# roysubhankar/dwt-domain-adaptation

Measured on NVIDIA H100. Metric: ResNet-50-DWT images/sec fwd+bwd, higher is better.
Workload: dtype f32

## Files before the change

### dwt-domain-adaptation_b200/dwt_b200/_native.py

```python
from __future__ import annotations

import ctypes
import os
import threading

import torch

_HERE = os.path.dirname(os.path.abspath(__file__))
LIB_PATH = os.environ.get("DWT_B200_LIB") or os.path.join(_HERE, "lib", "libdwt_b200.so")

ABI_VERSION = 6
MAX_DOMAINS = 4
MAX_GROUP_SIZE = 64
MODE_TRAIN, MODE_EVAL = 0, 1
EPI_NONE, EPI_AFFINE, EPI_RELU, EPI_RESIDUAL = 0, 1, 2, 4
LAYOUT_NHWC = 0x100
STATUS_NOT_PD, STATUS_BAD_LABEL = 1, 2
KIND_WHITEN, KIND_BN = 0, 1

_c_float_p = ctypes.c_void_p
_PtrArray = ctypes.c_void_p * MAX_DOMAINS


class TailSite(ctypes.Structure):
    _fields_ = [("x", ctypes.c_void_p), ("eps", ctypes.c_float), ("momentum", ctypes.c_float),
                ("update_running", ctypes.c_int), ("running_mean", ctypes.POINTER(ctypes.c_void_p)),
                ("running_cov", ctypes.POINTER(ctypes.c_void_p)), ("gamma", ctypes.c_void_p), ("beta", ctypes.c_void_p),
                ("save_mean", ctypes.c_void_p), ("save_w", ctypes.c_void_p), ("dx", ctypes.c_void_p),
                ("dgamma", ctypes.c_void_p), ("dbeta", ctypes.c_void_p)]

_SIGNATURES = {
    "dwt_abi_version": (ctypes.c_int, []),
    "dwt_last_error": (ctypes.c_char_p, []),
    "dwt_workspace_bytes": (ctypes.c_size_t, [ctypes.c_int64, ctypes.c_int64, ctypes.c_int64, ctypes.c_int, ctypes.c_int]),
    "dwt_whiten_fwd": (ctypes.c_int, [_c_float_p, _c_float_p, ctypes.c_int64, ctypes.c_int64, ctypes.c_int64,
                                      ctypes.c_int, ctypes.c_int, ctypes.c_int, ctypes.c_float, ctypes.c_float,
                                      ctypes.c_int, ctypes.POINTER(ctypes.c_void_p), ctypes.POINTER(ctypes.c_void_p),
                                      _c_float_p, _c_float_p, _c_float_p, ctypes.c_void_p, ctypes.c_int, _c_float_p,
                                      _c_float_p, ctypes.c_void_p, ctypes.c_size_t, ctypes.c_void_p]),
    "dwt_whiten_bwd": (ctypes.c_int, [_c_float_p, _c_float_p, _c_float_p, _c_float_p, ctypes.c_int64, ctypes.c_int64,
                                      ctypes.c_int64, ctypes.c_int, ctypes.c_int, ctypes.c_int, ctypes.c_float,
                                      _c_float_p, _c_float_p, _c_float_p, _c_float_p, ctypes.c_void_p, _c_float_p,
                                      ctypes.c_int, _c_float_p, _c_float_p, ctypes.c_void_p, ctypes.c_size_t,
                                      ctypes.c_void_p]),
    "dwt_bn_fwd": (ctypes.c_int, [_c_float_p, _c_float_p, ctypes.c_int64, ctypes.c_int64, ctypes.c_int64,
                                  ctypes.c_int, ctypes.c_int, ctypes.c_float, ctypes.c_float, ctypes.c_int,
                                  ctypes.POINTER(ctypes.c_void_p), ctypes.POINTER(ctypes.c_void_p), _c_float_p,
                                  _c_float_p, _c_float_p, ctypes.c_void_p, ctypes.c_int, _c_float_p, _c_float_p,
                                  ctypes.c_void_p, ctypes.c_size_t, ctypes.c_void_p]),
    "dwt_bn_bwd": (ctypes.c_int, [_c_float_p, _c_float_p, _c_float_p, _c_float_p, ctypes.c_int64, ctypes.c_int64, ctypes.c_int64,
                                  ctypes.c_int, ctypes.c_int, _c_float_p, _c_float_p, _c_float_p, _c_float_p,
                                  ctypes.c_void_p, _c_float_p, ctypes.c_int, _c_float_p, _c_float_p, ctypes.c_void_p,
                                  ctypes.c_size_t, ctypes.c_void_p]),
    "dwt_tail2_fwd": (ctypes.c_int, [ctypes.c_int, ctypes.POINTER(TailSite), _c_float_p, ctypes.c_void_p, ctypes.c_int64,
                                     ctypes.c_int64, ctypes.c_int64, ctypes.c_int, ctypes.c_int, ctypes.c_void_p,
                                     ctypes.c_size_t, ctypes.c_void_p]),
    "dwt_tail2_bwd": (ctypes.c_int, [ctypes.c_int, ctypes.POINTER(TailSite), _c_float_p, _c_float_p, ctypes.c_void_p,
                                     _c_float_p, ctypes.c_int64, ctypes.c_int64, ctypes.c_int64, ctypes.c_int, ctypes.c_int,
                                     ctypes.c_void_p, ctypes.c_size_t, ctypes.c_void_p]),
    "dwt_mec_fwd_bwd": (ctypes.c_int, [_c_float_p, _c_float_p, ctypes.c_int64, ctypes.c_int64, _c_float_p,
                                       _c_float_p, _c_float_p, ctypes.c_void_p]),
    "dwt_head_loss_fwd_bwd": (ctypes.c_int, [_c_float_p, ctypes.c_void_p, ctypes.c_int64, ctypes.c_int64, ctypes.c_float,
                                             _c_float_p, _c_float_p, ctypes.c_void_p, ctypes.c_void_p]),
    "dwt_augment_pair": (ctypes.c_int, [ctypes.c_void_p, ctypes.c_int64, ctypes.c_int, ctypes.c_int, ctypes.c_int,
                                        ctypes.c_void_p, ctypes.c_void_p, ctypes.c_void_p, _c_float_p,
                                        ctypes.POINTER(ctypes.c_float), ctypes.POINTER(ctypes.c_float), _c_float_p,
                                        _c_float_p, ctypes.c_int, ctypes.c_void_p]),
    "dwt_maxpool_fwd": (ctypes.c_int, [_c_float_p, _c_float_p, ctypes.c_void_p, ctypes.c_int64, ctypes.c_int64, ctypes.c_int64,
                                       ctypes.c_int64, ctypes.c_int, ctypes.c_int, ctypes.c_int, ctypes.c_void_p]),
    "dwt_maxpool_bwd": (ctypes.c_int, [_c_float_p, ctypes.c_void_p, _c_float_p, ctypes.c_int64, ctypes.c_int64, ctypes.c_int64,
                                       ctypes.c_int64, ctypes.c_int, ctypes.c_int, ctypes.c_int, ctypes.c_void_p]),
    "dwt_launch_count": (ctypes.c_int64, []),
    "dwt_profile_begin": (None, []),
    "dwt_profile_end": (ctypes.c_int, [ctypes.c_void_p, ctypes.c_int]),
}


class ProfileEntry(ctypes.Structure):
    _fields_ = [("name", ctypes.c_char * 48), ("launches", ctypes.c_int64), ("ms", ctypes.c_double),
                ("bytes", ctypes.c_double)]


def profile_begin():
    lib().dwt_profile_begin()


def profile_end():
    cap = 1024
    buf = (ProfileEntry * cap)()
    k = lib().dwt_profile_end(ctypes.cast(buf, ctypes.c_void_p), cap)
    return {buf[i].name.decode(): dict(launches=buf[i].launches, ms=buf[i].ms, bytes=buf[i].bytes) for i in range(k)}


def by_family(prof):
    out = {}
    for name, v in prof.items():
        f = out.setdefault(name.split("|")[0], dict(launches=0, ms=0.0, bytes=0.0))
        for k in f:
            f[k] += v[k]
    return out


def launch_count() -> int:
    return int(lib().dwt_launch_count())
EXPORTS = tuple(_SIGNATURES)

_lib = None
_lock = threading.Lock()


class NativeError(RuntimeError):
    pass


def lib() -> ctypes.CDLL:
    global _lib
    if _lib is None:
        with _lock:
            if _lib is None:
                if not os.path.exists(LIB_PATH):
                    raise NativeError(
                        f"{LIB_PATH} is missing: build it with `python {os.path.join(_HERE, 'build.py')}` "
                        "(dwt_b200 has no CPU or PyTorch fallback)")
                handle = ctypes.CDLL(LIB_PATH)
                for name, (res, args) in _SIGNATURES.items():
                    fn = getattr(handle, name)
                    fn.restype, fn.argtypes = res, args
                if handle.dwt_abi_version() != ABI_VERSION:
                    raise NativeError("libdwt_b200.so ABI version mismatch; rebuild it")
                _lib = handle
    return _lib


def channels_last_supported(channels: int, group_size: int) -> bool:
    if group_size not in (1, 2, 4) or channels % 4:
        return False
    c4 = channels // 4
    return c4 & (c4 - 1) == 0


def check(rc: int) -> None:
    if rc != 0:
        raise NativeError(f"libdwt_b200 error {rc}: {lib().dwt_last_error().decode()}")


def ptr(t):
    return None if t is None else ctypes.c_void_p(t.data_ptr())


def ptr_array(tensors):
    arr = _PtrArray()
    for i, t in enumerate(tensors):
        arr[i] = None if t is None else t.data_ptr()
    return ctypes.cast(arr, ctypes.POINTER(ctypes.c_void_p))


def require_cuda(*tensors, any_dtype=False) -> torch.device:
    dev = None
    for t in tensors:
        if t is None:
            continue
        if not t.is_cuda:
            raise NativeError("dwt_b200 runs on CUDA tensors only (no CPU fallback); got a tensor on " + str(t.device))
        if t.dtype != torch.float32 and not any_dtype:
            raise NativeError("dwt_b200 computes in float32; got " + str(t.dtype))
        if dev is None:
            dev = t.device
        elif t.device != dev:
            raise NativeError(f"tensors on different devices: {dev} vs {t.device}")
    return dev


def stream_ptr(device) -> ctypes.c_void_p:
    return ctypes.c_void_p(torch.cuda.current_stream(device).cuda_stream)


_workspaces: dict = {}


def workspace(device, n, c, hw, gs, nd):
    need = lib().dwt_workspace_bytes(n, c, hw, gs, nd)
    if need == 0:
        raise NativeError(f"invalid geometry for workspace: C={c} group_size={gs} domains={nd}")
    key = (device.index, torch.cuda.current_stream(device).cuda_stream)
    buf = _workspaces.get(key)
    if buf is None or buf.numel() < need:
        buf = torch.zeros(max(need, 8 << 20), dtype=torch.uint8, device=device)
        _workspaces[key] = buf
    return buf


def status(device=None) -> int:
    device = torch.device("cuda", torch.cuda.current_device()) if device is None else device
    buf = _workspaces.get((device.index, torch.cuda.current_stream(device).cuda_stream))
    return 0 if buf is None else int(buf[:4].view(torch.int32).item())


def status_all(device=None) -> int:
    device = torch.device("cuda", torch.cuda.current_device()) if device is None else device
    torch.cuda.synchronize(device)
    st = 0
    for (idx, _), buf in _workspaces.items():
        if idx == device.index:
            st |= int(buf[:4].view(torch.int32).item())
    return st


def status_ptr(device):
    return ctypes.c_void_p(workspace(device, 1, 4, 1, 1, 1).data_ptr())


def clear_status(device=None) -> None:
    device = torch.device("cuda", torch.cuda.current_device()) if device is None else device
    buf = _workspaces.get((device.index, torch.cuda.current_stream(device).cuda_stream))
    if buf is not None:
        buf[:4].zero_()


class NotPositiveDefiniteError(torch.linalg.LinAlgError):
    """What the reference's torch.cholesky raises at utils/whitening.py:53, raised late: the kernels never sync the
    host, so the failure is seen at the next poll (raise_on_status) or explicit check_status() call."""


_poll = {"every": 0, "count": 0}


def raise_on_status(every: int = 1) -> None:
    _poll["every"], _poll["count"] = max(0, int(every)), 0


def check_status(device=None) -> None:
    st = status(device)
    if st == 0:
        return
    clear_status(device)
    if st & STATUS_NOT_PD:
        raise NotPositiveDefiniteError(
            "cholesky: a whitening covariance was not positive definite (status word bit 0; the reference raises "
            "from torch.cholesky, utils/whitening.py:53); the affected group's output is NaN and its running-"
            "statistics update was skipped")
    if st & STATUS_BAD_LABEL:
        raise IndexError("head loss: a label was outside [0, num_classes) and is not ignore_index=-100 "
                         "(F.nll_loss asserts here); the row was dropped")
    raise NativeError(f"unknown status bits {st:#x}")


def poll_status(device) -> None:
    if _poll["every"]:
        _poll["count"] += 1
        if _poll["count"] >= _poll["every"]:
            _poll["count"] = 0
            check_status(device)
```

### dwt-domain-adaptation_b200/dwt_b200/csrc/api.cu

```cuda
#include <stdarg.h>
#include <stdio.h>
#include <stdlib.h>

#include <atomic>
#include <mutex>
#include <string>
#include <vector>
#include <string.h>

#include "norm_launch.h"

namespace {

thread_local char g_err[512] = "";

int fail(int code, const char* fmt, ...) {
  va_list ap;
  va_start(ap, fmt);
  vsnprintf(g_err, sizeof(g_err), fmt, ap);
  va_end(ap);
  return code;
}

int check_launch(const char* what) {
  cudaError_t e = cudaPeekAtLastError();
  if (e != cudaSuccess) {
    cudaGetLastError();
    return fail(DWT_E_LAUNCH, "%s: %s", what, cudaGetErrorString(e));
  }
  return DWT_OK;
}

int sm_count() {
  static int n = 0;
  if (n == 0) {
    int dev = 0;
    if (cudaGetDevice(&dev) != cudaSuccess ||
        cudaDeviceGetAttribute(&n, cudaDevAttrMultiProcessorCount, dev) != cudaSuccess || n <= 0)
      n = 132;
  }
  return n;
}

std::atomic<int64_t> g_launches{0};
std::mutex g_prof_mu;
bool g_prof_on = false;
struct ProfRec { char name[48]; cudaEvent_t a, b; double bytes; };
std::vector<ProfRec> g_prof;
std::vector<cudaEvent_t> g_event_pool;

cudaEvent_t take_event() {
  if (!g_event_pool.empty()) { cudaEvent_t e = g_event_pool.back(); g_event_pool.pop_back(); return e; }
  cudaEvent_t e = nullptr;
  cudaEventCreate(&e);
  return e;
}

struct Launch {
  cudaStream_t st; ProfRec rec; bool on;
  Launch(const char* family, const dwt::Geom* gm, double bytes, cudaStream_t s) : st(s), on(false) {
    rec.a = rec.b = nullptr; rec.bytes = bytes;
    if (gm) snprintf(rec.name, sizeof(rec.name), "%s|%d|%d|%d|%d|%d", family, gm->C, gm->HW, gm->GS, gm->D, gm->N);
    else snprintf(rec.name, sizeof(rec.name), "%s", family);
    g_launches.fetch_add(1, std::memory_order_relaxed);
    std::lock_guard<std::mutex> lk(g_prof_mu);
    if (g_prof_on && g_prof.size() < (1u << 18)) {
      on = true; rec.a = take_event(); rec.b = take_event();
      cudaEventRecord(rec.a, st);
    }
  }
  ~Launch() {
    if (!on) return;
    cudaEventRecord(rec.b, st);
    std::lock_guard<std::mutex> lk(g_prof_mu);
    g_prof.push_back(rec);
  }
};

std::once_flag g_tiled_once;
int g_tiled_rc = 0;
int ensure_tiled() {
  std::call_once(g_tiled_once, [] { g_tiled_rc = dwt::tiled_init(); });
  return g_tiled_rc;
}

std::once_flag g_tc_once;
int g_tc_rc = 0;
int ensure_tc() {
  std::call_once(g_tc_once, [] { g_tc_rc = dwt::tc_init(); });
  return g_tc_rc;
}

int tc_chunks(const dwt::Geom& g) {
  const int problems = dwt::tc_superblocks(g) * g.D;
  int n = 2 * sm_count() / problems;
  const int64_t tiles = (int64_t)g.N * ((g.HW + 31) / 32);
  if (n > tiles) n = (int)tiles;
  return n < 1 ? 1 : n;
}

int tc_apply_ctas(const dwt::Geom& g, int per_sm, int tile_px) {
  const int problems = dwt::tc_superblocks(g) * g.D;
  int n = per_sm * sm_count() / problems;
  const int64_t tiles = (int64_t)g.N * ((g.HW + tile_px - 1) / tile_px);
  if (n > tiles) n = (int)tiles;
  return n < 1 ? 1 : n;
}

int env_int(const char* name, int dflt) {
  const char* v = getenv(name);
  return (v && *v) ? atoi(v) : dflt;
}

struct ClPlan { int nred, new_, S, gridy, gz_red, gz_ew; };
ClPlan cl_plan(const dwt::Geom& g, int slots_red, int slots_ew, int unroll_red, int unroll_ew) {
  static const int seq_mb = env_int("DWT_CL_SEQ_MB", 1 << 30);
  const int C4 = g.C / 4, CW = C4 < 256 ? C4 : 256, rpi = 256 / CW, gridy = C4 / CW;
  const long long rows = (long long)g.N * g.HW;
  const double mbytes = 4.0 * (double)g.D * (double)rows * (double)g.C / 1048576.0;
  const bool seq = g.D > 1 && mbytes >= (double)seq_mb;
  ClPlan p;
  p.gridy = gridy;
  p.gz_red = p.gz_ew = seq ? 1 : g.D;
  auto shape = [&](int slots, int unroll, int gz) {
    long long by_work = rows / ((long long)rpi * unroll * 2);
    if (by_work < 1) by_work = 1;
    int cap = slots * sm_count() / (gridy * gz);
    if (cap < 1) cap = 1;
    return (int)(by_work < cap ? by_work : cap);
  };
  p.nred = shape(slots_red, unroll_red, p.gz_red);
  p.new_ = shape(slots_ew, unroll_ew, p.gz_ew);
  p.S = p.nred < 8 ? p.nred : 8;
  return p;
}

inline size_t align_up(size_t v, size_t a) { return (v + a - 1) / a * a; }

enum KernelKind { K_STATS, K_APPLY, K_BWD_REDUCE, K_BWD_APPLY };

int slots_per_sm(KernelKind k, int GS) {
  if (GS > 4) return 2;
  return ((k == K_STATS || k == K_APPLY) && GS < 4) ? 4 : 3;
}

int chunk_cap(int GS, int G, int D) {
  (void)GS;
  const int target = 16 * sm_count();
  int cap = (target + G * D - 1) / (G * D);
  return cap < 1 ? 1 : cap;
}

struct Workspace {
  int* status;
  int* counters;
  int* dom_counter;
  int* dom_counter2;
  float* partial;
  float* save_cov;
  float* coef;
  float* dgb_part;
  float* gram;
  float* shift;
  float* red;
  int* bad;
  size_t bytes;
};

constexpr size_t kMaxGroups = 65536;
constexpr size_t kOffCounters = 256;
constexpr size_t kOffDom1 = kOffCounters + sizeof(int) * DWT_MAX_DOMAINS * kMaxGroups;
constexpr size_t kOffDom2 = kOffDom1 + sizeof(int) * kMaxGroups;
constexpr size_t kOffScratch = kOffDom2 + sizeof(int) * kMaxGroups;

Workspace carve(void* base, int64_t C, int GS, int D, size_t start = kOffScratch) {
  const int G = (int)(C / GS);
  const int cap = chunk_cap(GS, G, D);
  size_t off = start;
  auto take = [&](size_t nbytes) { size_t o = off; off = align_up(off + nbytes, 256); return o; };
  char* b = static_cast<char*>(base);
  Workspace w;
  w.status = reinterpret_cast<int*>(b);
  w.counters = reinterpret_cast<int*>(b + kOffCounters);
  w.dom_counter = reinterpret_cast<int*>(b + kOffDom1);
  w.dom_counter2 = reinterpret_cast<int*>(b + kOffDom2);
  size_t partial_floats = (size_t)D * G * cap * (GS * GS + GS);
  if (GS >= 8 && 64 % GS == 0) {
    const size_t tc = ((size_t)2 * sm_count() + (size_t)((C + 63) / 64) * D) * (64 * 64 + 64);
    if (tc > partial_floats) partial_floats = tc;
  }
  size_t red_floats = 1;
  if (dwt::cl_supports((int)C, GS)) {
    const size_t W = (size_t)dwt::cl_bwd_width((int)C, GS);
    const int C4 = (int)C / 4, gridy = C4 <= 256 ? 1 : C4 / 256;
    const size_t cl = (size_t)D * (3 * sm_count() / gridy + 1) * W;
    if (cl > partial_floats) partial_floats = cl;
    red_floats = (size_t)D * 8 * W;
  }
  w.partial = reinterpret_cast<float*>(b + take(sizeof(float) * partial_floats));
  w.red = reinterpret_cast<float*>(b + take(sizeof(float) * red_floats));
  w.save_cov = reinterpret_cast<float*>(b + take(sizeof(float) * (size_t)D * G * GS * GS));
  w.coef = reinterpret_cast<float*>(b + take(sizeof(float) * (size_t)D * G * dwt::coef_stride(GS)));
  w.dgb_part = reinterpret_cast<float*>(b + take(sizeof(float) * (size_t)D * 2 * C));
  const size_t SBn = (size_t)((C + 63) / 64);
  w.gram = reinterpret_cast<float*>(b + take(sizeof(float) * (size_t)D * SBn * (64 * 64 + 64)));
  w.shift = reinterpret_cast<float*>(b + take(sizeof(float) * (size_t)D * SBn * 64));
  w.bad = reinterpret_cast<int*>(b + take(sizeof(int) * (size_t)D * G));
  w.bytes = off;
  return w;
}

struct Plan {
  dwt::Geom gm;
  dwt::Geom gm_ew;
  int vec;
  int chunks_ew;
  bool small;
};

void shape(dwt::Geom& g, int64_t work_units, KernelKind kind, bool small, int* chunks) {
  const bool reduce = (kind == K_STATS || kind == K_BWD_REDUCE);
  const int slots = slots_per_sm(kind, g.GS) * sm_count();
  const int target = reduce ? slots : 4 * slots;
  g.ppc = 1;
  if (small) {
    while (g.ppc < 8 && (int64_t)((g.G + g.ppc - 1) / g.ppc) * g.D > target) g.ppc <<= 1;
  }
  int n = 1;
  if (g.ppc == 1) {
    n = target / (g.G * g.D);
    const int cap = chunk_cap(g.GS, g.G, g.D);
    if (n > cap) n = cap;
    if (n > work_units) n = (int)work_units;
    if (n < 1) n = 1;
  }
  *chunks = n;
}

int make_plan(Plan& p, KernelKind reduce_kind, KernelKind ew_kind, const void* a0, const void* a1, const void* a2,
              int64_t N, int64_t C, int64_t HW, int GS, int D) {
  if (N <= 0 || C <= 0 || HW <= 0) return fail(DWT_E_INVALID, "empty tensor (N=%lld C=%lld HW=%lld)", (long long)N,
                                               (long long)C, (long long)HW);
  if (GS < 1 || GS > DWT_MAX_GROUP_SIZE) return fail(DWT_E_UNSUPPORTED, "group_size %d outside [1,%d]", GS,
                                                     DWT_MAX_GROUP_SIZE);
  if (C % GS != 0) return fail(DWT_E_INVALID, "channels %lld not divisible by group_size %d", (long long)C, GS);
  if (D < 1 || D > DWT_MAX_DOMAINS) return fail(DWT_E_INVALID, "n_domains %d outside [1,%d]", D, DWT_MAX_DOMAINS);
  if (N * C * HW >= (int64_t)1 << 31 || C / GS > 65535)
    return fail(DWT_E_UNSUPPORTED, "shape too large for 32-bit item indexing");
  dwt::Geom& g = p.gm;
  g.N = (int)N; g.C = (int)C; g.HW = (int)HW; g.GS = GS; g.G = (int)(C / GS); g.D = D;
  g.M = (float)((double)N * (double)HW);
  const uintptr_t bits = (uintptr_t)a0 | (uintptr_t)a1 | (uintptr_t)a2;
  p.vec = (HW % 4 == 0 && bits % 16 == 0) ? 4 : 1;
  p.small = dwt::small_supports(GS);
  int64_t work_units;
  if (p.small) work_units = (N * (HW / p.vec) + dwt::kThreads * 2 - 1) / (dwt::kThreads * 2);
  else work_units = (N * HW + 127) / 128;
  if (work_units < 1) work_units = 1;
  shape(g, work_units, reduce_kind, p.small, &g.nchunks);
  p.gm_ew = g;
  shape(p.gm_ew, work_units, ew_kind, p.small, &p.chunks_ew);
  p.gm_ew.nchunks = g.nchunks;
  return DWT_OK;
}

int check_running(bool need_running, float* const* rmean, float* const* rcov, int D) {
  if (!need_running) return DWT_OK;
  if (!rmean || !rcov) return fail(DWT_E_INVALID, "running buffers required");
  for (int d = 0; d < D; ++d)
    if (!rmean[d] || !rcov[d]) return fail(DWT_E_INVALID, "running buffer of domain %d is null", d);
  return DWT_OK;
}

dwt::FwdFin make_fwd_fin(float a, float b, float momentum, float unbias, int update_running, bool need_running,
                         float* const* rmean, float* const* rcov, float* save_mean, float* save_w, const Workspace& w, int D) {
  dwt::FwdFin fin{};
  fin.a = a; fin.b = b; fin.momentum = momentum; fin.unbias = unbias;
  fin.update_running = update_running;
  fin.save_mean = save_mean; fin.save_w = save_w; fin.save_cov = w.save_cov;
  for (int d = 0; d < D; ++d) { fin.rmean[d] = need_running ? rmean[d] : nullptr; fin.rcov[d] = need_running ? rcov[d] : nullptr; }
  fin.dom_counter = w.dom_counter; fin.status = w.status; fin.bad = w.bad;
  if (need_running && D > 1) {
    bool all_same = true, all_distinct = true;
    for (int d = 1; d < D; ++d) {
      if (rmean[d] != rmean[0] || rcov[d] != rcov[0]) all_same = false;
      for (int e = 0; e < d; ++e)
        if (rmean[d] == rmean[e] || rcov[d] == rcov[e]) all_distinct = false;
    }
    fin.aliased = all_same ? 1 : (all_distinct ? 0 : -1);
  }
  return fin;
}

dwt::BwdFin make_bwd_fin(float a, int mode, int epi, const float* save_mean, const float* save_w, const float* gamma,
                         float* dgamma, float* dbeta, const Workspace& w) {
  dwt::BwdFin fin{};
  fin.a = a; fin.mode = mode; fin.epi = epi;
  fin.save_mean = save_mean; fin.save_w = save_w; fin.gamma = gamma;
  fin.coef = w.coef; fin.dgb_part = w.dgb_part;
  fin.dgamma = (epi & DWT_EPI_AFFINE) ? dgamma : nullptr;
  fin.dbeta = (epi & DWT_EPI_AFFINE) ? dbeta : nullptr;
  fin.dom_counter = w.dom_counter2;
  return fin;
}

int whiten_like_fwd(const float* x, float* y, int64_t N, int64_t C, int64_t HW, int GS, int D, int mode, float a,
                    float b, float momentum, float unbias, int update_running, float* const* rmean,
                    float* const* rcov, const float* gamma, const float* beta, const float* residual,
                    uint8_t* relu_mask, int epi, float* save_mean, float* save_w, void* ws, size_t ws_bytes,
                    cudaStream_t st) {
  const bool nhwc = (mode & DWT_LAYOUT_NHWC) != 0;
  mode &= 0xFF;
  Plan p;
  if (int rc = make_plan(p, K_STATS, K_APPLY, x, y, nullptr, N, C, HW, GS, D)) return rc;
  if (!x || !y || !save_mean || !save_w || !ws) return fail(DWT_E_INVALID, "null pointer argument");
  if (nhwc && !dwt::cl_supports((int)C, GS))
    return fail(DWT_E_UNSUPPORTED, "channels-last layout is built for group_size 1, 2, 4 with C/4 a power of two (C=%lld gs=%d)", (long long)C, GS);
  if (nhwc && (((uintptr_t)x | (uintptr_t)y) % 16 != 0)) return fail(DWT_E_INVALID, "channels-last tensors must be 16-byte aligned");
  if (mode != DWT_MODE_TRAIN && mode != DWT_MODE_EVAL) return fail(DWT_E_INVALID, "bad mode %d", mode);
  if ((epi & DWT_EPI_RELU) && !(epi & DWT_EPI_AFFINE)) return fail(DWT_E_INVALID, "RELU epilogue needs AFFINE");
  if ((epi & DWT_EPI_AFFINE) && (!gamma || !beta)) return fail(DWT_E_INVALID, "AFFINE epilogue needs gamma and beta");
  if ((epi & DWT_EPI_RESIDUAL) && ((epi & 3) != 3 || !residual)) return fail(DWT_E_INVALID, "RESIDUAL epilogue needs AFFINE|RELU and a residual tensor");
  if ((epi & DWT_EPI_RESIDUAL) && (uintptr_t)residual % 16 != 0) return fail(DWT_E_INVALID, "residual must be 16-byte aligned");
  if (relu_mask && !((epi & DWT_EPI_RESIDUAL) && nhwc))
    return fail(DWT_E_UNSUPPORTED, "the ReLU byte map is written by the channels-last RESIDUAL epilogue only");
  if (epi != 0 && !p.small)
    return fail(DWT_E_UNSUPPORTED, "fused gamma/beta/ReLU epilogue is built for group_size 1, 2, 4 (got %d)", GS);
  const bool need_running = (mode == DWT_MODE_EVAL) || update_running;
  if (int rc = check_running(need_running, rmean, rcov, D)) return rc;
  Workspace w = carve(ws, C, GS, D);
  if (w.bytes > ws_bytes) return fail(DWT_E_WORKSPACE, "workspace too small: need %zu bytes, got %zu", w.bytes, ws_bytes);
  if ((uintptr_t)ws % 256 != 0) return fail(DWT_E_WORKSPACE, "workspace must be 256-byte aligned");
  if (!p.small && ensure_tiled() != 0) return fail(DWT_E_LAUNCH, "cudaFuncSetAttribute failed (%d)", g_tiled_rc);

  const dwt::FwdFin fin = make_fwd_fin(a, b, momentum, unbias, mode == DWT_MODE_TRAIN ? update_running : 0, need_running,
                                       rmean, rcov, save_mean, save_w, w, D);

  const double E = 4.0 * (double)D * (double)N * (double)C * (double)HW;
  if (nhwc) {
    const ClPlan cp = cl_plan(p.gm, 3, 3, 8, (epi & DWT_EPI_RESIDUAL) ? 4 : 8);
    if (mode == DWT_MODE_TRAIN) {
      {
        Launch l("cl_stats", &p.gm, E, st);
        dwt::cl_stats(x, p.gm, cp.nred, cp.gz_red, w.partial, w.shift, st);
      }
      if (int rc = check_launch("channels-last statistics kernel")) return rc;
      Launch l("cl_fwd_finalize", &p.gm, 0.0, st);
      dwt::cl_fwd_finalize(w.partial, cp.nred, w.shift, p.gm, fin, st);
    } else {
      Launch l("eval_prep", &p.gm, 0.0, st);
      dwt::small_eval_prep(p.gm, fin, st);
    }
    if (int rc = check_launch("channels-last finalize kernel")) return rc;
    {
      Launch l("cl_apply", &p.gm, ((epi & DWT_EPI_RESIDUAL) ? (relu_mask ? 3.0625 : 3.0) : 2.0) * E, st);
      dwt::cl_apply(x, y, p.gm, cp.new_, cp.gz_ew, epi, save_mean, save_w, gamma, beta, residual, relu_mask, st);
    }
    return check_launch("channels-last apply kernel");
  }
  const bool tc = !p.small && dwt::tc_supports(p.gm, p.vec) && ensure_tc() == 0;
  if (mode == DWT_MODE_TRAIN) {
    Launch l(p.small ? "small_stats" : (tc ? "tc_stats" : "tiled_stats"), &p.gm, E, st);
    if (p.small) dwt::small_stats(x, p.gm, p.vec, fin, w.partial, w.counters, st);
    else if (tc) {
      if (int cr = dwt::tc_stats(x, p.gm, tc_chunks(p.gm), w.shift, w.partial, st))
        return fail(DWT_E_LAUNCH, "cuTensorMapEncodeTiled failed (CUresult %d) x=%p N=%d C=%d HW=%d D=%d", cr, (const void*)x, p.gm.N, p.gm.C, p.gm.HW, p.gm.D);
    } else dwt::tiled_stats(x, p.gm, p.vec, fin, w.partial, w.counters, st);
  } else {
    Launch l("eval_prep", &p.gm, 0.0, st);
    if (p.small) dwt::small_eval_prep(p.gm, fin, st);
    else if (tc) dwt::dense_fwd_factor(nullptr, nullptr, p.gm, fin, st);
    else dwt::tiled_eval_prep(p.gm, fin, st);
  }
  if (tc && mode == DWT_MODE_TRAIN) {
    if (int rc = check_launch("tensor-core statistics kernel")) return rc;
    Launch l("dense_fwd_finalize", &p.gm, 0.0, st);
    dwt::dense_partial_reduce(w.partial, tc_chunks(p.gm), dwt::tc_superblocks(p.gm) * D, w.gram, st);
    dwt::dense_fwd_factor(w.gram, w.shift, p.gm, fin, st);
  }
  if (int rc = check_launch("whitening statistics kernel")) return rc;
  {
    Launch l(p.small ? "small_apply" : (tc ? "tc_apply" : "tiled_apply"), &p.gm, ((epi & DWT_EPI_RESIDUAL) ? 3 : 2) * E, st);
    if (p.small) dwt::small_apply(x, y, p.gm_ew, p.vec, p.chunks_ew, epi, save_mean, save_w, gamma, beta, residual, st);
    else if (tc) {
      if (int cr = dwt::tc_apply(x, y, p.gm, tc_apply_ctas(p.gm, 1, 64), save_mean, save_w, st))
        return fail(DWT_E_LAUNCH, "cuTensorMapEncodeTiled failed (CUresult %d)", cr);
    } else dwt::tiled_apply(x, y, p.gm_ew, p.vec, p.chunks_ew, save_mean, save_w, st);
  }
  return check_launch("whitening apply kernel");
}

int whiten_like_bwd(const float* x, const float* dout, const float* dout2, float* dx, int64_t N, int64_t C, int64_t HW, int GS, int D,
                    int mode, float a, const float* save_mean, const float* save_w, const float* gamma,
                    const float* beta, const uint8_t* relu_mask, float* dresidual, int epi, float* dgamma,
                    float* dbeta, void* ws, size_t ws_bytes, cudaStream_t st) {
  const bool nhwc = (mode & DWT_LAYOUT_NHWC) != 0;
  mode &= 0xFF;
  Plan p;
  if (int rc = make_plan(p, K_BWD_REDUCE, K_BWD_APPLY, x, dout, dx, N, C, HW, GS, D)) return rc;
  if (!x || !dout || !dx || !save_mean || !save_w || !ws) return fail(DWT_E_INVALID, "null pointer argument");
  if (dout2 && (!nhwc || (uintptr_t)dout2 % 16 != 0))
    return fail(nhwc ? DWT_E_INVALID : DWT_E_UNSUPPORTED, "a second gradient addend (dout2) is built for the channels-last "
                "kernels (16-byte aligned tensor); add it to dout otherwise");
  if (nhwc && !dwt::cl_supports((int)C, GS))
    return fail(DWT_E_UNSUPPORTED, "channels-last layout is built for group_size 1, 2, 4 with C/4 a power of two (C=%lld gs=%d)", (long long)C, GS);
  if (nhwc && (((uintptr_t)x | (uintptr_t)dout | (uintptr_t)dx) % 16 != 0)) return fail(DWT_E_INVALID, "channels-last tensors must be 16-byte aligned");
  if (mode != DWT_MODE_TRAIN && mode != DWT_MODE_EVAL) return fail(DWT_E_INVALID, "bad mode %d", mode);
  if ((epi & DWT_EPI_RELU) && !(epi & DWT_EPI_AFFINE)) return fail(DWT_E_INVALID, "RELU epilogue needs AFFINE");
  if ((epi & DWT_EPI_AFFINE) && (!gamma || !beta)) return fail(DWT_E_INVALID, "AFFINE epilogue needs gamma and beta");
  if (epi & DWT_EPI_RESIDUAL) {
    if (!nhwc || !relu_mask || (epi & 3) != 3 || !dresidual)
      return fail(DWT_E_INVALID, "backward of a RESIDUAL forward needs the channels-last layout, AFFINE|RELU, the forward's "
                                 "ReLU byte map and dresidual (or pass dout already masked by (out > 0) with epilogue AFFINE)");
    if ((uintptr_t)dresidual % 16 != 0) return fail(DWT_E_INVALID, "dresidual must be 16-byte aligned");
  } else if (relu_mask || dresidual) {
    return fail(DWT_E_INVALID, "relu_mask / dresidual belong to the RESIDUAL epilogue");
  }
  if ((dgamma == nullptr) != (dbeta == nullptr)) return fail(DWT_E_INVALID, "dgamma and dbeta go together");
  if (epi != 0 && !p.small)
    return fail(DWT_E_UNSUPPORTED, "fused gamma/beta/ReLU epilogue is built for group_size 1, 2, 4 (got %d)", GS);
  Workspace w = carve(ws, C, GS, D);
  if (w.bytes > ws_bytes) return fail(DWT_E_WORKSPACE, "workspace too small: need %zu bytes, got %zu", w.bytes, ws_bytes);
  if ((uintptr_t)ws % 256 != 0) return fail(DWT_E_WORKSPACE, "workspace must be 256-byte aligned");
  if (!p.small && ensure_tiled() != 0) return fail(DWT_E_LAUNCH, "cudaFuncSetAttribute failed (%d)", g_tiled_rc);

  const dwt::BwdFin fin = make_bwd_fin(a, mode, epi, save_mean, save_w, gamma, dgamma, dbeta, w);
  const bool masked = nhwc && (epi & DWT_EPI_RESIDUAL) != 0;

  const bool need_reduce = (mode == DWT_MODE_TRAIN) || (fin.dgamma != nullptr) || masked;
  const double E = 4.0 * (double)D * (double)N * (double)C * (double)HW;
  if (nhwc) {
    const ClPlan cp = cl_plan(p.gm, 2, 2, 4, 4);
    if (need_reduce) {
      {
        Launch l("cl_bwd_reduce", &p.gm, ((masked ? 3.0625 : 2.0) + (dout2 ? 1.0 : 0.0)) * E, st);
        dwt::cl_bwd_reduce(x, dout, dout2, p.gm, cp.nred, cp.gz_red, epi, save_mean, save_w, gamma, beta, relu_mask, dresidual, w.partial, st);
      }
      if (int rc = check_launch("channels-last backward reduction kernel")) return rc;
      Launch l("cl_bwd_finalize", &p.gm, 0.0, st);
      dwt::cl_bwd_finalize(w.partial, cp.nred, p.gm, fin, st);
    } else {
      Launch l("bwd_prep", &p.gm, 0.0, st);
      dwt::small_bwd_prep(p.gm, fin, st);
    }
    if (int rc = check_launch("channels-last backward finalize kernel")) return rc;
    {
      Launch l("cl_bwd_apply", &p.gm, (3.0 + (dout2 && !masked ? 1.0 : 0.0)) * E, st);
      if (masked) dwt::cl_bwd_apply(x, dresidual, nullptr, dx, p.gm, cp.new_, cp.gz_ew, DWT_EPI_AFFINE, w.coef, save_mean, save_w, gamma, beta, st);
      else dwt::cl_bwd_apply(x, dout, dout2, dx, p.gm, cp.new_, cp.gz_ew, epi, w.coef, save_mean, save_w, gamma, beta, st);
    }
    return check_launch("channels-last backward apply kernel");
  }
  const bool tc = !p.small && dwt::tc_supports(p.gm, p.vec) && ensure_tc() == 0;
  if (need_reduce) {
    Launch l(p.small ? "small_bwd_reduce" : (tc ? "tc_bwd_reduce" : "tiled_bwd_reduce"), &p.gm, 2 * E, st);
    if (p.small) dwt::small_bwd_reduce(x, dout, p.gm, p.vec, fin, beta, w.partial, w.counters, st);
    else if (tc) {
      if (int cr = dwt::tc_bwd_reduce(x, dout, p.gm, tc_chunks(p.gm), save_mean, w.partial, st))
        return fail(DWT_E_LAUNCH, "cuTensorMapEncodeTiled failed (CUresult %d) x=%p dout=%p N=%d C=%d HW=%d D=%d", cr, (const void*)x, (const void*)dout, p.gm.N, p.gm.C, p.gm.HW, p.gm.D);
    } else dwt::tiled_bwd_reduce(x, dout, p.gm, p.vec, fin, w.partial, w.counters, st);
  } else {
    Launch l("bwd_prep", &p.gm, 0.0, st);
    if (p.small) dwt::small_bwd_prep(p.gm, fin, st);
    else if (tc) dwt::dense_bwd_coef(nullptr, p.gm, fin, w.shift, st);
    else dwt::tiled_bwd_prep(p.gm, fin, st);
  }
  if (tc && need_reduce) {
    if (int rc = check_launch("tensor-core backward reduction kernel")) return rc;
    Launch l("dense_bwd_finalize", &p.gm, 0.0, st);
    dwt::dense_partial_reduce(w.partial, tc_chunks(p.gm), dwt::tc_superblocks(p.gm) * D, w.gram, st);
    dwt::dense_bwd_coef(w.gram, p.gm, fin, w.shift, st);
  }
  if (int rc = check_launch("whitening backward reduction kernel")) return rc;
  {
    Launch l(p.small ? "small_bwd_apply" : (tc ? "tc_bwd_apply" : "tiled_bwd_apply"), &p.gm, 3 * E, st);
    if (p.small) dwt::small_bwd_apply(x, dout, dx, p.gm_ew, p.vec, p.chunks_ew, epi, w.coef, save_mean, save_w, gamma, beta, st);
    else if (tc) {
      if (int cr = dwt::tc_bwd_apply(x, dout, dx, p.gm, tc_apply_ctas(p.gm, 1, 64), w.coef, save_mean, w.shift, st))
        return fail(DWT_E_LAUNCH, "cuTensorMapEncodeTiled failed (CUresult %d)", cr);
    } else dwt::tiled_bwd_apply(x, dout, dx, p.gm_ew, p.vec, p.chunks_ew, w.coef, st);
  }
  return check_launch("whitening backward apply kernel");
}

struct SiteConst { float a, b, unbias; };
SiteConst site_const(int kind, float eps, int64_t N, int64_t HW) {
  if (kind == DWT_KIND_BN) {
    const double M = (double)N * (double)HW;
    return {1.f, eps, M > 1.0 ? (float)(M / (M - 1.0)) : 1.f};
  }
  return {1.f - eps, eps, 1.f};
}

int tail2_plan(Plan& p, int kind, const dwt_tail_site* s, const void* out, int64_t N, int64_t C, int64_t HW, int GS, int D) {
  if (kind != DWT_KIND_WHITEN && kind != DWT_KIND_BN) return fail(DWT_E_INVALID, "bad kind %d", kind);
  if (kind == DWT_KIND_BN && GS != 1) return fail(DWT_E_INVALID, "batch norm has group_size 1 (got %d)", GS);
  if (!s) return fail(DWT_E_INVALID, "null pointer argument");
  if (int rc = make_plan(p, K_STATS, K_APPLY, s[0].x, s[1].x, out, N, C, HW, GS, D)) return rc;
  if (!dwt::cl_supports((int)C, GS))
    return fail(DWT_E_UNSUPPORTED, "the two-site tail runs on the channels-last kernels: group_size 1, 2, 4 with C/4 a power of two (C=%lld gs=%d)",
                (long long)C, GS);
  for (int k = 0; k < 2; ++k)
    if (!s[k].x || !s[k].gamma || !s[k].beta || !s[k].save_mean || !s[k].save_w || !out) return fail(DWT_E_INVALID, "null pointer argument");
  if ((((uintptr_t)s[0].x | (uintptr_t)s[1].x | (uintptr_t)out) % 16) != 0) return fail(DWT_E_INVALID, "channels-last tensors must be 16-byte aligned");
  return DWT_OK;
}

int tail2_workspace(Workspace (&w)[2], void* ws, size_t ws_bytes, int64_t C, int GS, int D) {
  if (!ws) return fail(DWT_E_INVALID, "null pointer argument");
  w[0] = carve(ws, C, GS, D);
  w[1] = carve(ws, C, GS, D, w[0].bytes);
  if (w[1].bytes > ws_bytes) return fail(DWT_E_WORKSPACE, "workspace too small: need %zu bytes, got %zu", w[1].bytes, ws_bytes);
  if ((uintptr_t)ws % 256 != 0) return fail(DWT_E_WORKSPACE, "workspace must be 256-byte aligned");
  return DWT_OK;
}

int tail2_fwd(int kind, const dwt_tail_site* s, float* y, uint8_t* relu_mask, int64_t N, int64_t C, int64_t HW, int GS, int D,
              void* ws, size_t ws_bytes, cudaStream_t st) {
  Plan p;
  if (int rc = tail2_plan(p, kind, s, y, N, C, HW, GS, D)) return rc;
  if (!relu_mask) return fail(DWT_E_INVALID, "the two-site tail writes the ReLU byte map its backward reads");
  for (int k = 0; k < 2; ++k)
    if (int rc = check_running(s[k].update_running != 0, s[k].running_mean, s[k].running_cov, D)) return rc;
  Workspace w[2];
  if (int rc = tail2_workspace(w, ws, ws_bytes, C, GS, D)) return rc;
  dwt::FwdFin fin[2];
  for (int k = 0; k < 2; ++k) {
    const SiteConst sc = site_const(kind, s[k].eps, N, HW);
    fin[k] = make_fwd_fin(sc.a, sc.b, s[k].momentum, sc.unbias, s[k].update_running, s[k].update_running != 0, s[k].running_mean,
                          s[k].running_cov, s[k].save_mean, s[k].save_w, w[k], D);
  }
  const double E = 4.0 * (double)D * (double)N * (double)C * (double)HW;
  const ClPlan cp = cl_plan(p.gm, 3, 3, 8, 4);
  for (int k = 0; k < 2; ++k) {
    Launch l("cl_stats", &p.gm, E, st);
    dwt::cl_stats(s[k].x, p.gm, cp.nred, cp.gz_red, w[k].partial, w[k].shift, st);
  }
  if (int rc = check_launch("channels-last statistics kernel")) return rc;
  {
    Launch l("cl_tail2_fwd_finalize", &p.gm, 0.0, st);
    dwt::cl_fwd_finalize(w[0].partial, cp.nred, w[0].shift, p.gm, fin[0], st, &fin[1], (size_t)(w[1].partial - w[0].partial),
                         (size_t)(w[1].shift - w[0].shift));
  }
  if (int rc = check_launch("channels-last finalize kernel")) return rc;
  {
    Launch l("cl_tail2_apply", &p.gm, 3.0625 * E, st);
    dwt::cl_tail2_apply(s[0].x, s[1].x, y, p.gm, cp.new_, cp.gz_ew, s[0].save_mean, s[0].save_w, s[0].gamma, s[0].beta,
                        s[1].save_mean, s[1].save_w, s[1].gamma, s[1].beta, relu_mask, st);
  }
  return check_launch("channels-last two-site apply kernel");
}

int tail2_bwd(int kind, const dwt_tail_site* s, const float* dout, const float* dout2, const uint8_t* relu_mask, float* dz,
              int64_t N, int64_t C, int64_t HW, int GS, int D, void* ws, size_t ws_bytes, cudaStream_t st) {
  Plan p;
  if (int rc = tail2_plan(p, kind, s, dz, N, C, HW, GS, D)) return rc;
  if (!dout || !relu_mask || !s[0].dx || !s[1].dx) return fail(DWT_E_INVALID, "null pointer argument");
  if ((((uintptr_t)dout | (uintptr_t)dout2 | (uintptr_t)s[0].dx | (uintptr_t)s[1].dx) % 16) != 0)
    return fail(DWT_E_INVALID, "channels-last tensors must be 16-byte aligned");
  for (int k = 0; k < 2; ++k)
    if ((s[k].dgamma == nullptr) != (s[k].dbeta == nullptr)) return fail(DWT_E_INVALID, "dgamma and dbeta go together");
  Workspace w[2];
  if (int rc = tail2_workspace(w, ws, ws_bytes, C, GS, D)) return rc;
  dwt::BwdFin fin[2];
  for (int k = 0; k < 2; ++k)
    fin[k] = make_bwd_fin(site_const(kind, s[k].eps, N, HW).a, DWT_MODE_TRAIN, k ? DWT_EPI_AFFINE : (DWT_EPI_AFFINE | DWT_EPI_RELU | DWT_EPI_RESIDUAL),
                          s[k].save_mean, s[k].save_w, s[k].gamma, s[k].dgamma, s[k].dbeta, w[k]);
  const double E = 4.0 * (double)D * (double)N * (double)C * (double)HW;
  const ClPlan cp = cl_plan(p.gm, 2, 2, 4, 4);
  {
    Launch l("cl_tail2_bwd_reduce", &p.gm, (4.0625 + (dout2 ? 1.0 : 0.0)) * E, st);
    dwt::cl_tail2_bwd_reduce(s[0].x, s[1].x, dout, dout2, p.gm, cp.nred, cp.gz_red, s[0].save_mean, s[1].save_mean, relu_mask, dz,
                             w[0].partial, (size_t)(w[1].partial - w[0].partial), st);
  }
  if (int rc = check_launch("channels-last two-site backward reduction kernel")) return rc;
  {
    Launch l("cl_tail2_bwd_finalize", &p.gm, 0.0, st);
    dwt::cl_bwd_finalize(w[0].partial, cp.nred, p.gm, fin[0], st, &fin[1], (size_t)(w[1].partial - w[0].partial));
  }
  if (int rc = check_launch("channels-last backward finalize kernel")) return rc;
  {
    Launch l("cl_tail2_bwd_apply", &p.gm, 5.0 * E, st);
    dwt::cl_tail2_bwd_apply(s[0].x, s[1].x, dz, s[0].dx, s[1].dx, p.gm, cp.new_, cp.gz_ew, w[0].coef, w[1].coef, st);
  }
  return check_launch("channels-last two-site backward apply kernel");
}

}

extern "C" {

int dwt_abi_version(void) { return DWT_B200_ABI_VERSION; }

const char* dwt_last_error(void) { return g_err; }

size_t dwt_workspace_bytes(int64_t N, int64_t C, int64_t HW, int group_size, int n_domains) {
  (void)N; (void)HW;
  if (C <= 0 || group_size < 1 || group_size > DWT_MAX_GROUP_SIZE || C % group_size != 0 || n_domains < 1 ||
      n_domains > DWT_MAX_DOMAINS)
    return 0;
  return carve(nullptr, C, group_size, n_domains, carve(nullptr, C, group_size, n_domains).bytes).bytes;
}

int dwt_whiten_fwd(const float* x, float* y, int64_t N, int64_t C, int64_t HW, int group_size, int n_domains,
                   int mode, float eps, float momentum, int update_running, float* const* running_mean,
                   float* const* running_cov, const float* gamma, const float* beta, const float* residual,
                   uint8_t* relu_mask, int epilogue, float* save_mean, float* save_w, void* workspace,
                   size_t workspace_bytes, dwt_stream_t stream) {
  return whiten_like_fwd(x, y, N, C, HW, group_size, n_domains, mode, 1.f - eps, eps, momentum, 1.f, update_running,
                         running_mean, running_cov, gamma, beta, residual, relu_mask, epilogue, save_mean, save_w,
                         workspace, workspace_bytes, (cudaStream_t)stream);
}

int dwt_whiten_bwd(const float* x, const float* dout, const float* dout2, float* dx, int64_t N, int64_t C, int64_t HW, int group_size,
                   int n_domains, int mode, float eps, const float* save_mean, const float* save_w,
                   const float* gamma, const float* beta, const uint8_t* relu_mask, float* dresidual, int epilogue,
                   float* dgamma, float* dbeta, void* workspace, size_t workspace_bytes, dwt_stream_t stream) {
  return whiten_like_bwd(x, dout, dout2, dx, N, C, HW, group_size, n_domains, mode, 1.f - eps, save_mean, save_w, gamma,
                         beta, relu_mask, dresidual, epilogue, dgamma, dbeta, workspace, workspace_bytes,
                         (cudaStream_t)stream);
}

int dwt_bn_fwd(const float* x, float* y, int64_t N, int64_t C, int64_t HW, int n_domains, int mode, float eps,
               float factor, int update_running, float* const* running_mean, float* const* running_var,
               const float* weight, const float* bias, const float* residual, uint8_t* relu_mask, int epilogue,
               float* save_mean, float* save_invstd, void* workspace, size_t workspace_bytes, dwt_stream_t stream) {
  const double M = (double)N * (double)HW;
  const float unbias = M > 1.0 ? (float)(M / (M - 1.0)) : 1.f;
  return whiten_like_fwd(x, y, N, C, HW, 1, n_domains, mode, 1.f, eps, factor, unbias, update_running, running_mean,
                         running_var, weight, bias, residual, relu_mask, epilogue, save_mean, save_invstd, workspace,
                         workspace_bytes, (cudaStream_t)stream);
}

int dwt_bn_bwd(const float* x, const float* dout, const float* dout2, float* dx, int64_t N, int64_t C, int64_t HW, int n_domains,
               int mode, const float* save_mean, const float* save_invstd, const float* weight, const float* bias,
               const uint8_t* relu_mask, float* dresidual, int epilogue, float* dweight, float* dbias, void* workspace,
               size_t workspace_bytes, dwt_stream_t stream) {
  return whiten_like_bwd(x, dout, dout2, dx, N, C, HW, 1, n_domains, mode, 1.f, save_mean, save_invstd, weight, bias,
                         relu_mask, dresidual, epilogue, dweight, dbias, workspace, workspace_bytes,
                         (cudaStream_t)stream);
}

int dwt_tail2_fwd(int kind, const dwt_tail_site* sites, float* y, uint8_t* relu_mask, int64_t N, int64_t C, int64_t HW,
                  int group_size, int n_domains, void* workspace, size_t workspace_bytes, dwt_stream_t stream) {
  return tail2_fwd(kind, sites, y, relu_mask, N, C, HW, group_size, n_domains, workspace, workspace_bytes, (cudaStream_t)stream);
}

int dwt_tail2_bwd(int kind, const dwt_tail_site* sites, const float* dout, const float* dout2, const uint8_t* relu_mask, float* dz,
                  int64_t N, int64_t C, int64_t HW, int group_size, int n_domains, void* workspace, size_t workspace_bytes,
                  dwt_stream_t stream) {
  return tail2_bwd(kind, sites, dout, dout2, relu_mask, dz, N, C, HW, group_size, n_domains, workspace, workspace_bytes,
                   (cudaStream_t)stream);
}

int dwt_mec_fwd_bwd(const float* x, const float* y, int64_t N, int64_t K, float* loss, float* gx, float* gy,
                    dwt_stream_t stream) {
  if (!x || !y || !loss || !gx || !gy) return fail(DWT_E_INVALID, "null pointer argument");
  if (N <= 0 || K <= 0 || N >= (1 << 24) || K >= (1 << 24)) return fail(DWT_E_INVALID, "bad logits shape [%lld,%lld]", (long long)N, (long long)K);
  {
    Launch l("mec", nullptr, 16.0 * (double)N * (double)K, (cudaStream_t)stream);
    dwt::mec_launch(x, y, (int)N, (int)K, loss, gx, gy, (cudaStream_t)stream);
  }
  return check_launch("MEC kernel");
}

int dwt_head_loss_fwd_bwd(const float* logits, const int64_t* labels, int64_t B, int64_t K, float lambda, float* losses,
                          float* grad, int* status, dwt_stream_t stream) {
  if (!logits || !labels || !losses || !grad) return fail(DWT_E_INVALID, "null pointer argument");
  if (B <= 0 || K <= 0 || B >= (1 << 22) || K >= (1 << 24)) return fail(DWT_E_INVALID, "bad logits shape [3*%lld,%lld]", (long long)B, (long long)K);
  {
    Launch l("head_loss", nullptr, 4.0 * 3 * (double)B * (double)K * 2, (cudaStream_t)stream);
    dwt::head_loss_launch(logits, reinterpret_cast<const long long*>(labels), (int)B, (int)K, lambda, losses, grad, status,
                          (cudaStream_t)stream);
  }
  return check_launch("head loss kernel");
}

int dwt_augment_pair(const uint8_t* images, int64_t B, int src_h, int src_w, int crop, const int32_t* crop_plain,
                     const int32_t* crop_aug, const uint8_t* flip, const float* affine, const float* mean,
                     const float* stdv, float* out_plain, float* out_aug, int layout, dwt_stream_t stream) {
  if (!images || !mean || !stdv) return fail(DWT_E_INVALID, "null pointer argument");
  if (!out_plain && !out_aug) return fail(DWT_E_INVALID, "at least one of out_plain / out_aug is needed");
  if (out_plain && !crop_plain) return fail(DWT_E_INVALID, "out_plain needs crop_plain");
  if (out_aug && (!crop_aug || !flip || !affine)) return fail(DWT_E_INVALID, "out_aug needs crop_aug, flip and affine");
  if (B <= 0 || B > 65535 || src_h <= 0 || src_w <= 0 || src_h > 16384 || src_w > 16384)
    return fail(DWT_E_INVALID, "bad image batch [%lld,%d,%d,3]", (long long)B, src_h, src_w);
  if (crop <= 0 || crop > src_h || crop > src_w) return fail(DWT_E_INVALID, "crop %d does not fit %dx%d", crop, src_h, src_w);
  if (layout != 0 && layout != DWT_LAYOUT_NHWC) return fail(DWT_E_INVALID, "layout must be 0 (NCHW) or DWT_LAYOUT_NHWC");
  for (int c = 0; c < 3; ++c)
    if (!(stdv[c] != 0.f)) return fail(DWT_E_INVALID, "std[%d] must be non-zero", c);
  {
    const double px = (double)B * crop * crop;
    Launch l("augment_pair", nullptr, px * 3 * ((out_plain ? 5.0 : 0.0) + (out_aug ? 5.0 : 0.0)), (cudaStream_t)stream);
    dwt::augment_pair_launch(images, (int)B, src_h, src_w, crop, crop_plain, crop_aug, flip, affine, mean, stdv, out_plain,
                             out_aug, layout != 0, (cudaStream_t)stream);
  }
  return check_launch("augmentation kernel");
}

namespace {
int pool_check(int64_t N, int64_t H, int64_t W, int64_t C, int k, int s, int p, int* OH, int* OW) {
  if (N <= 0 || H <= 0 || W <= 0 || C <= 0 || C % 4 != 0) return fail(DWT_E_INVALID, "bad pooling input [%lld,%lld,%lld,%lld] (C must be a multiple of 4)", (long long)N, (long long)H, (long long)W, (long long)C);
  if (k < 1 || k > 15 || s < 1 || p < 0 || 2 * p > k) return fail(DWT_E_INVALID, "bad pooling window k=%d s=%d p=%d (k <= 15, pad <= k/2)", k, s, p);
  if (H + 2 * p < k || W + 2 * p < k) return fail(DWT_E_INVALID, "pooling window larger than the padded image");
  *OH = (int)((H + 2 * p - k) / s + 1);
  *OW = (int)((W + 2 * p - k) / s + 1);
  if (N * H * W * C >= ((int64_t)1 << 40)) return fail(DWT_E_UNSUPPORTED, "tensor too large");
  return DWT_OK;
}
}

int dwt_maxpool_fwd(const float* x, float* y, uint8_t* argmax, int64_t N, int64_t H, int64_t W, int64_t C, int kernel,
                    int stride, int padding, dwt_stream_t stream) {
  int OH = 0, OW = 0;
  if (int rc = pool_check(N, H, W, C, kernel, stride, padding, &OH, &OW)) return rc;
  if (!x || !y || !argmax) return fail(DWT_E_INVALID, "null pointer argument");
  if ((((uintptr_t)x | (uintptr_t)y) % 16) != 0 || (uintptr_t)argmax % 4 != 0) return fail(DWT_E_INVALID, "pooling tensors must be 16-byte aligned");
  {
    const double in = (double)N * H * W * C, out = (double)N * OH * OW * C;
    Launch l("maxpool_fwd", nullptr, 4.0 * (in + out) + out, (cudaStream_t)stream);
    dwt::maxpool_fwd_launch(x, y, argmax, (int)N, (int)H, (int)W, (int)C, OH, OW, kernel, stride, padding, (cudaStream_t)stream);
  }
  return check_launch("max-pool forward kernel");
}

int dwt_maxpool_bwd(const float* dy, const uint8_t* argmax, float* dx, int64_t N, int64_t H, int64_t W, int64_t C, int kernel,
                    int stride, int padding, dwt_stream_t stream) {
  int OH = 0, OW = 0;
  if (int rc = pool_check(N, H, W, C, kernel, stride, padding, &OH, &OW)) return rc;
  if (!dy || !dx || !argmax) return fail(DWT_E_INVALID, "null pointer argument");
  if ((((uintptr_t)dy | (uintptr_t)dx) % 16) != 0 || (uintptr_t)argmax % 4 != 0) return fail(DWT_E_INVALID, "pooling tensors must be 16-byte aligned");
  {
    const double in = (double)N * H * W * C, out = (double)N * OH * OW * C;
    Launch l("maxpool_bwd", nullptr, 4.0 * (in + out) + out, (cudaStream_t)stream);
    dwt::maxpool_bwd_launch(dy, argmax, dx, (int)N, (int)H, (int)W, (int)C, OH, OW, kernel, stride, padding, (cudaStream_t)stream);
  }
  return check_launch("max-pool backward kernel");
}

int64_t dwt_launch_count(void) { return g_launches.load(); }

void dwt_profile_begin(void) {
  std::lock_guard<std::mutex> lk(g_prof_mu);
  for (auto& r : g_prof) { g_event_pool.push_back(r.a); g_event_pool.push_back(r.b); }
  g_prof.clear();
  g_prof_on = true;
}

int dwt_profile_end(dwt_profile_entry* out, int max_entries) {
  std::vector<ProfRec> recs;
  {
    std::lock_guard<std::mutex> lk(g_prof_mu);
    g_prof_on = false;
    recs.swap(g_prof);
  }
  int n = 0;
  for (auto& r : recs) {
    float ms = 0.f;
    if (cudaEventSynchronize(r.b) == cudaSuccess && cudaEventElapsedTime(&ms, r.a, r.b) == cudaSuccess) {
      int k = 0;
      for (; k < n; ++k)
        if (strcmp(out[k].name, r.name) == 0) break;
      if (k == n && n < max_entries) {
        memset(&out[n], 0, sizeof(out[n]));
        strncpy(out[n].name, r.name, sizeof(out[n].name) - 1);
        ++n;
      }
      if (k < n) { out[k].launches += 1; out[k].ms += ms; out[k].bytes += r.bytes; }
    }
    std::lock_guard<std::mutex> lk(g_prof_mu);
    g_event_pool.push_back(r.a); g_event_pool.push_back(r.b);
  }
  return n;
}

}
```

### dwt-domain-adaptation_b200/dwt_b200/csrc/norm_cl.cu

```cuda
#include <stdlib.h>

#include "dwt_common.cuh"
#include "norm_launch.h"
#include "small_algebra.cuh"

namespace dwt {
namespace {

constexpr int kT = 256;

__device__ __forceinline__ void pdl_wait() { asm volatile("griddepcontrol.wait;" ::: "memory"); }
__device__ __forceinline__ void pdl_launch_dependents() { asm volatile("griddepcontrol.launch_dependents;" ::: "memory"); }

template <int GS> struct ClShape {
  static constexpr int NSUB = 4 / GS;
  static constexpr int NM = GS * (GS + 1) / 2;
  static constexpr int FWD1 = GS + NM;
  static constexpr int BWD1 = GS * GS + GS;
  static constexpr int FWD = NSUB * FWD1;
  static constexpr int BWD = NSUB * BWD1;
};

struct ClThread {
  int C4, CW, rpi, col, rsub, q;
  __device__ __forceinline__ ClThread(const Geom& gm) {
    C4 = gm.C >> 2;
    CW = C4 < kT ? C4 : kT;
    rpi = kT / CW;
    col = threadIdx.x % CW;
    rsub = threadIdx.x / CW;
    q = blockIdx.y * CW + col;
  }
};

template <int UNROLL, bool DESC, class F>
__device__ __forceinline__ void sweep_rows(const ClThread& t, unsigned rows, F&& body) {
  const unsigned krows = (unsigned)t.rpi * UNROLL, nch = (rows + krows - 1) / krows;
  for (unsigned i = blockIdx.x; i < nch; i += gridDim.x) body((DESC ? nch - 1 - i : i) * krows + t.rsub);
}
#define CL_FOR_DOMAINS(d, gm, DESC) \
  for (int di_ = blockIdx.z, d = (DESC) ? (gm).D - 1 - di_ : di_; di_ < (gm).D; di_ += gridDim.z, d = (DESC) ? (gm).D - 1 - di_ : di_)

__device__ __forceinline__ float4 ldg4(const float* p) { return __ldg(reinterpret_cast<const float4*>(p)); }

template <int NACC>
__device__ __forceinline__ void column_reduce(const ClThread& t, float (&acc)[NACC], float* sRed) {
  if (t.rpi == 1) return;
#pragma unroll
  for (int i = 0; i < NACC; ++i) sRed[i * kT + threadIdx.x] = acc[i];
  __syncthreads();
  if (t.rsub == 0) {
#pragma unroll
    for (int i = 0; i < NACC; ++i) {
      float s = acc[i];
      for (int r = 1; r < t.rpi; ++r) s += sRed[i * kT + r * t.CW + t.col];
      acc[i] = s;
    }
  }
}

template <int GS>
__global__ void __launch_bounds__(kT, 3) cl_stats_kernel(const float* __restrict__ x, const Geom gm,
                                                         float* __restrict__ partial, float* __restrict__ shift) {
  using S = ClShape<GS>;
  constexpr int UNROLL = 8;
  __shared__ float sRed[kT * S::FWD];
  const ClThread t(gm);
  const unsigned rows = (unsigned)gm.N * gm.HW;
  pdl_launch_dependents();
  CL_FOR_DOMAINS(d, gm, true) {
    const float* xd = x + (size_t)d * rows * gm.C + 4 * t.q;
    float K[4] = {0.f, 0.f, 0.f, 0.f};
    {
      const unsigned np = rows < 8 ? rows : 8;
      for (unsigned r = 0; r < np; ++r) {
        const float4 v = ldg4(xd + (size_t)r * gm.C);
        K[0] += v.x; K[1] += v.y; K[2] += v.z; K[3] += v.w;
      }
#pragma unroll
      for (int c = 0; c < 4; ++c) K[c] /= (float)np;
      if (blockIdx.x == 0 && t.rsub == 0) *reinterpret_cast<float4*>(shift + (size_t)d * gm.C + 4 * t.q) = make_float4(K[0], K[1], K[2], K[3]);
    }
    float acc[S::FWD];
#pragma unroll
    for (int i = 0; i < S::FWD; ++i) acc[i] = 0.f;
    sweep_rows<UNROLL, true>(t, rows, [&](unsigned r) {
      float4 v[UNROLL];
#pragma unroll
      for (int u = 0; u < UNROLL; ++u) {
        const unsigned rr = r + u * t.rpi;
        v[u] = rr < rows ? ldg4(xd + (size_t)rr * gm.C) : make_float4(K[0], K[1], K[2], K[3]);
      }
#pragma unroll
      for (int u = 0; u < UNROLL; ++u) {
        const float e[4] = {v[u].x - K[0], v[u].y - K[1], v[u].z - K[2], v[u].w - K[3]};
#pragma unroll
        for (int s = 0; s < S::NSUB; ++s) {
#pragma unroll
          for (int c = 0; c < GS; ++c) {
            acc[s * S::FWD1 + c] += e[s * GS + c];
#pragma unroll
            for (int j = 0; j <= c; ++j)
              acc[s * S::FWD1 + GS + c * (c + 1) / 2 + j] = fmaf(e[s * GS + c], e[s * GS + j], acc[s * S::FWD1 + GS + c * (c + 1) / 2 + j]);
          }
        }
      }
    });
    column_reduce<S::FWD>(t, acc, sRed);
    if (t.rsub == 0) {
      float* dst = partial + (((size_t)d * gridDim.x + blockIdx.x) * t.C4 + t.q) * S::FWD;
#pragma unroll
      for (int i = 0; i < S::FWD; ++i) dst[i] = acc[i];
    }
    if (gridDim.z == 1) __syncthreads();
  }
}

template <int GS, int PER>
__device__ __forceinline__ int acc_index(int g, int a) {
  constexpr int NSUB = 4 / GS;
  return (g / NSUB) * (NSUB * PER) + (g % NSUB) * PER + a;
}

constexpr int kFinQ = 2;

template <int NACC>
__device__ __forceinline__ void column_row_sum(const float* __restrict__ col, int nrows, int W, float (&a)[NACC]) {
  static_assert(NACC % 2 == 0, "accumulators are read as float2");
#pragma unroll
  for (int i = 0; i < NACC; ++i) a[i] = 0.f;
#pragma unroll 4
  for (int r = threadIdx.x; r < nrows; r += 32) {
    const float2* p = reinterpret_cast<const float2*>(col + (size_t)r * W);
#pragma unroll
    for (int i = 0; i < NACC / 2; ++i) {
      const float2 v = __ldcg(p + i);
      a[2 * i] += v.x; a[2 * i + 1] += v.y;
    }
  }
#pragma unroll
  for (int o = 1; o < 32; o <<= 1)
#pragma unroll
    for (int i = 0; i < NACC; ++i) a[i] += __shfl_xor_sync(0xffffffffu, a[i], o);
}

template <int NSUB, int PER>
__device__ __forceinline__ void take_group(const float (&a)[NSUB * PER], int s, float (&v)[PER]) {
#pragma unroll
  for (int i = 0; i < PER; ++i) {
    v[i] = a[i];
#pragma unroll
    for (int k = 1; k < NSUB; ++k)
      if (s == k) v[i] = a[k * PER + i];
  }
}

template <int GS>
__device__ __forceinline__ void cl_fwd_finalize_site(const float* __restrict__ partial, int nrows, const float* __restrict__ shift,
                                                     const Geom& gm, const FwdFin& fin) {
  using SH = ClShape<GS>;
  constexpr int NST = GS + GS * GS;
  __shared__ float sStat[DWT_MAX_DOMAINS][kFinQ][SH::NSUB][NST + 1];
  __shared__ unsigned char sBad[DWT_MAX_DOMAINS][kFinQ][SH::NSUB];
  const int s = threadIdx.x, ql = threadIdx.y, d = threadIdx.z, q = blockIdx.x * blockDim.y + ql;
  const int W = (gm.C >> 2) * SH::FWD;
  const float invM = 1.f / gm.M;
  const bool lead = s < SH::NSUB;
  const int g = q * SH::NSUB + (lead ? s : 0);
  const bool direct = gm.D == 1 || fin.aliased == 0;
  const int dbuf = direct ? d : 0;
  const bool upd = fin.update_running && lead && (direct || (fin.aliased == 1 && d == 0));
  float rc_old[GS * GS], rm_old[GS];
  if (upd) {
#pragma unroll
    for (int e = 0; e < GS * GS; ++e) rc_old[e] = fin.rcov[dbuf][(size_t)g * GS * GS + e];
#pragma unroll
    for (int e = 0; e < GS; ++e) rm_old[e] = fin.rmean[dbuf][g * GS + e];
  }
  pdl_launch_dependents();
  pdl_wait();
  float a[SH::FWD];
  column_row_sum<SH::FWD>(partial + (size_t)d * nrows * W + (size_t)q * SH::FWD, nrows, W, a);
  if (lead) {
    float v[SH::FWD1];
    take_group<SH::NSUB, SH::FWD1>(a, s, v);
    float mean[GS], cov[GS][GS];
#pragma unroll
    for (int i = 0; i < GS; ++i) mean[i] = shift[(size_t)d * gm.C + g * GS + i] + v[i] * invM;
#pragma unroll
    for (int i = 0; i < GS; ++i)
#pragma unroll
      for (int j = 0; j <= i; ++j) {
        const float c = v[GS + i * (i + 1) / 2 + j] * invM - (v[i] * invM) * (v[j] * invM);
        cov[i][j] = c; cov[j][i] = c;
      }
    const bool bad = factor_thread<GS>(gm, fin, d, g, mean, cov, false);
    if (fin.update_running) {
      if (direct) {
        if (!bad) {
          const float m = fin.momentum, kk = 1.f - fin.momentum;
#pragma unroll
          for (int i = 0; i < GS; ++i) {
            fin.rmean[d][g * GS + i] = m * mean[i] + kk * rm_old[i];
#pragma unroll
            for (int j = 0; j < GS; ++j)
              fin.rcov[d][(size_t)g * GS * GS + i * GS + j] = m * (cov[i][j] * fin.unbias) + kk * rc_old[i * GS + j];
          }
        }
      } else {
        sBad[d][ql][s] = bad ? 1 : 0;
#pragma unroll
        for (int i = 0; i < GS; ++i) {
          sStat[d][ql][s][i] = mean[i];
#pragma unroll
          for (int j = 0; j < GS; ++j) sStat[d][ql][s][GS + i * GS + j] = cov[i][j];
        }
      }
    }
  }
  if (!fin.update_running || direct) return;
  __syncthreads();
  if (!(lead && d == 0)) return;
  if (fin.aliased == 1) {
    const float m = fin.momentum, kk = 1.f - fin.momentum;
    float* rc = fin.rcov[0] + (size_t)g * GS * GS;
    float* rm = fin.rmean[0] + g * GS;
    for (int dd = 0; dd < gm.D; ++dd) {
      if (sBad[dd][ql][s]) continue;
#pragma unroll
      for (int e = 0; e < GS * GS; ++e) rc_old[e] = m * (sStat[dd][ql][s][GS + e] * fin.unbias) + kk * rc_old[e];
#pragma unroll
      for (int e = 0; e < GS; ++e) rm_old[e] = m * sStat[dd][ql][s][e] + kk * rm_old[e];
    }
#pragma unroll
    for (int e = 0; e < GS * GS; ++e) rc[e] = rc_old[e];
#pragma unroll
    for (int e = 0; e < GS; ++e) rm[e] = rm_old[e];
  } else {
    for (int dd = 0; dd < gm.D; ++dd)
      if (!sBad[dd][ql][s]) ema_direct<GS>(gm, fin, dd, g, &sStat[dd][ql][s][0], &sStat[dd][ql][s][GS]);
  }
}

template <int GS>
__global__ void __launch_bounds__(32 * kFinQ * DWT_MAX_DOMAINS) cl_fwd_finalize_kernel(const float* __restrict__ partial, size_t pstride, int nrows,
                                                                                      const float* __restrict__ shift, size_t sstride, const Geom gm,
                                                                                      const __grid_constant__ FwdFin fin, const __grid_constant__ FwdFin fin2) {
  const bool second = blockIdx.y != 0;
  cl_fwd_finalize_site<GS>(partial + (second ? pstride : 0), nrows, shift + (second ? sstride : 0), gm, second ? fin2 : fin);
}

template <int GS, int EPI, bool DS>
__global__ void __launch_bounds__(kT, 3) cl_apply_kernel(const float* __restrict__ x, float* __restrict__ y, const Geom gm,
                                                         const float* __restrict__ save_mean, const float* __restrict__ save_w,
                                                         const float* __restrict__ gamma, const float* __restrict__ beta,
                                                         const float* __restrict__ res, uint8_t* __restrict__ mask,
                                                         const float* __restrict__ save_mean_d, const float* __restrict__ save_w_d,
                                                         const float* __restrict__ gamma_d, const float* __restrict__ beta_d) {
  using S = ClShape<GS>;
  constexpr bool RES = (EPI & DWT_EPI_RESIDUAL) != 0;
  static_assert(!DS || RES, "the two-site tail is a residual epilogue");
  constexpr int UNROLL = DS ? 2 : (RES ? 4 : 8);
  const ClThread t(gm);
  const unsigned rows = (unsigned)gm.N * gm.HW;
  pdl_wait();
  CL_FOR_DOMAINS(d, gm, false) {
    float Wp[S::NSUB][S::NM], bp[S::NSUB][GS], Wd[DS ? S::NSUB : 1][S::NM], bd[DS ? S::NSUB : 1][GS];
#pragma unroll
    for (int s = 0; s < S::NSUB; ++s) {
      const int g = t.q * S::NSUB + s;
      load_forward_map<GS, EPI>(save_w + ((size_t)d * gm.G + g) * GS * GS, save_mean + (size_t)d * gm.C + g * GS,
                                gamma + g * GS, beta + g * GS, Wp[s], bp[s]);
      if constexpr (DS)
        load_forward_map<GS, DWT_EPI_AFFINE>(save_w_d + ((size_t)d * gm.G + g) * GS * GS, save_mean_d + (size_t)d * gm.C + g * GS,
                                             gamma_d + g * GS, beta_d + g * GS, Wd[s], bd[s]);
    }
    const size_t base = (size_t)d * rows * gm.C + 4 * t.q;
    const float* xd = x + base;
    const float* rd = res + base;
    float* yd = y + base;
    uint8_t* md = mask + (size_t)d * rows * t.C4 + t.q;
    sweep_rows<UNROLL, false>(t, rows, [&](unsigned r) {
      float4 v[UNROLL], rs[UNROLL];
#pragma unroll
      for (int u = 0; u < UNROLL; ++u) {
        const unsigned rr = r + u * t.rpi;
        if (rr < rows) {
          v[u] = ldg4(xd + (size_t)rr * gm.C);
          if constexpr (RES) rs[u] = ldg4(rd + (size_t)rr * gm.C);
        }
      }
#pragma unroll
      for (int u = 0; u < UNROLL; ++u) {
        const unsigned rr = r + u * t.rpi;
        if (rr < rows) {
          const float e[4] = {v[u].x, v[u].y, v[u].z, v[u].w};
          float o[4], ra[4] = {0.f, 0.f, 0.f, 0.f};
          if constexpr (RES) { ra[0] = rs[u].x; ra[1] = rs[u].y; ra[2] = rs[u].z; ra[3] = rs[u].w; }
          unsigned bits = 0;
#pragma unroll
          for (int s = 0; s < S::NSUB; ++s) {
            float xi[GS], oi[GS];
            if constexpr (DS) {
              float xdi[GS], odi[GS];
#pragma unroll
              for (int c = 0; c < GS; ++c) xdi[c] = ra[s * GS + c];
              apply_group<GS>(Wd[s], bd[s], xdi, odi);
#pragma unroll
              for (int c = 0; c < GS; ++c) ra[s * GS + c] = odi[c];
            }
#pragma unroll
            for (int c = 0; c < GS; ++c) xi[c] = e[s * GS + c];
            apply_group<GS>(Wp[s], bp[s], xi, oi);
#pragma unroll
            for (int c = 0; c < GS; ++c) {
              const float z = RES ? oi[c] + ra[s * GS + c] : oi[c];
              if constexpr (RES) bits |= (z > 0.f ? 1u : 0u) << (s * GS + c);
              o[s * GS + c] = (EPI & DWT_EPI_RELU) ? fmaxf(z, 0.f) : z;
            }
          }
          *reinterpret_cast<float4*>(yd + (size_t)rr * gm.C) = make_float4(o[0], o[1], o[2], o[3]);
          if constexpr (RES) { if (mask != nullptr) md[(size_t)rr * t.C4] = (uint8_t)bits; }
        }
      }
    });
  }
}

template <int GS>
__device__ __forceinline__ void bwd_accumulate(float* acc, const float (&dz)[GS], const float (&xi)[GS], const float* mu) {
#pragma unroll
  for (int i = 0; i < GS; ++i) {
    acc[GS * GS + i] += dz[i];
#pragma unroll
    for (int j = 0; j < GS; ++j) acc[i * GS + j] = fmaf(dz[i], xi[j] - mu[j], acc[i * GS + j]);
  }
}

template <int GS, int EPI, bool D2, bool DS>
__global__ void __launch_bounds__(kT, 2) cl_bwd_reduce_kernel(const float* __restrict__ x, const float* __restrict__ dout, const float* __restrict__ dout2,
                                                              const Geom gm, const float* __restrict__ save_mean,
                                                              const float* __restrict__ save_w, const float* __restrict__ gamma,
                                                              const float* __restrict__ beta, const uint8_t* __restrict__ mask,
                                                              float* __restrict__ dzout, float* __restrict__ partial,
                                                              const float* __restrict__ xds, const float* __restrict__ save_mean_d,
                                                              size_t pstride) {
  using S = ClShape<GS>;
  constexpr int UNROLL = 4;
  constexpr bool MASK = (EPI & DWT_EPI_RESIDUAL) != 0;
  constexpr bool RELU = (EPI & DWT_EPI_RELU) != 0 && !MASK;
  static_assert(!DS || MASK, "the two-site tail is a residual epilogue");
  constexpr int NS = DS ? 2 : 1;
  __shared__ float sRed[kT * S::BWD];
  const ClThread t(gm);
  const unsigned rows = (unsigned)gm.N * gm.HW;
  pdl_launch_dependents();
  CL_FOR_DOMAINS(d, gm, true) {
    float Wp[S::NSUB][S::NM], bp[S::NSUB][GS], mu[NS][4];
#pragma unroll
    for (int s = 0; s < S::NSUB; ++s) {
      const int g = t.q * S::NSUB + s;
      if constexpr (RELU)
        load_forward_map<GS, EPI>(save_w + ((size_t)d * gm.G + g) * GS * GS, save_mean + (size_t)d * gm.C + g * GS,
                                  gamma + g * GS, beta + g * GS, Wp[s], bp[s]);
    }
#pragma unroll
    for (int k = 0; k < NS; ++k) {
      const float4 m4 = ldg4((k ? save_mean_d : save_mean) + (size_t)d * gm.C + 4 * t.q);
      mu[k][0] = m4.x; mu[k][1] = m4.y; mu[k][2] = m4.z; mu[k][3] = m4.w;
    }
    float acc[NS][S::BWD];
#pragma unroll
    for (int k = 0; k < NS; ++k)
#pragma unroll
      for (int i = 0; i < S::BWD; ++i) acc[k][i] = 0.f;
    const size_t base = (size_t)d * rows * gm.C + 4 * t.q;
    const float* xp[NS];
    xp[0] = x + base;
    if constexpr (DS) xp[NS - 1] = xds + base;
    const float* gd = dout + base;
    const float* gd2 = D2 ? dout2 + base : nullptr;
    float* zd = MASK ? dzout + base : nullptr;
    const uint8_t* md = mask + (size_t)d * rows * t.C4 + t.q;
    constexpr int H = DS ? UNROLL / 2 : UNROLL;
    sweep_rows<UNROLL, true>(t, rows, [&](unsigned r0) {
#pragma unroll
     for (int h = 0; h < UNROLL; h += H) {
      const unsigned r = r0 + h * t.rpi;
      float4 v[NS][H], q[H], q2[D2 ? H : 1];
      unsigned mb[H];
#pragma unroll
      for (int u = 0; u < H; ++u) {
        const unsigned rr = r + u * t.rpi;
        if (rr < rows) {
#pragma unroll
          for (int k = 0; k < NS; ++k) v[k][u] = ldg4(xp[k] + (size_t)rr * gm.C);
          q[u] = ldg4(gd + (size_t)rr * gm.C);
          if constexpr (MASK) mb[u] = __ldg(md + (size_t)rr * t.C4);
          if constexpr (D2) q2[u] = ldg4(gd2 + (size_t)rr * gm.C);
        } else {
#pragma unroll
          for (int k = 0; k < NS; ++k) v[k][u] = make_float4(mu[k][0], mu[k][1], mu[k][2], mu[k][3]);
          q[u] = make_float4(0.f, 0.f, 0.f, 0.f);
          if constexpr (MASK) mb[u] = 0u;
          if constexpr (D2) q2[u] = make_float4(0.f, 0.f, 0.f, 0.f);
        }
      }
      if constexpr (D2) {
#pragma unroll
        for (int u = 0; u < H; ++u) { q[u].x += q2[u].x; q[u].y += q2[u].y; q[u].z += q2[u].z; q[u].w += q2[u].w; }
      }
#pragma unroll
      for (int u = 0; u < H; ++u) {
        const float ge[4] = {q[u].x, q[u].y, q[u].z, q[u].w};
        const float e[4] = {v[0][u].x, v[0][u].y, v[0][u].z, v[0][u].w};
        const float ed[4] = {v[NS - 1][u].x, v[NS - 1][u].y, v[NS - 1][u].z, v[NS - 1][u].w};
        float zm[4];
#pragma unroll
        for (int s = 0; s < S::NSUB; ++s) {
          float xi[GS], dz[GS];
#pragma unroll
          for (int c = 0; c < GS; ++c) { xi[c] = e[s * GS + c]; dz[c] = ge[s * GS + c]; }
          if constexpr (RELU) {
            float oi[GS];
            apply_group<GS>(Wp[s], bp[s], xi, oi);
#pragma unroll
            for (int c = 0; c < GS; ++c) dz[c] = oi[c] > 0.f ? dz[c] : 0.f;
          }
          if constexpr (MASK) {
#pragma unroll
            for (int c = 0; c < GS; ++c) { dz[c] = ((mb[u] >> (s * GS + c)) & 1u) ? dz[c] : 0.f; zm[s * GS + c] = dz[c]; }
          }
          bwd_accumulate<GS>(acc[0] + s * S::BWD1, dz, xi, &mu[0][s * GS]);
          if constexpr (DS) {
#pragma unroll
            for (int c = 0; c < GS; ++c) xi[c] = ed[s * GS + c];
            bwd_accumulate<GS>(acc[NS - 1] + s * S::BWD1, dz, xi, &mu[NS - 1][s * GS]);
          }
        }
        if constexpr (MASK) {
          const unsigned rr = r + u * t.rpi;
          if (rr < rows) *reinterpret_cast<float4*>(zd + (size_t)rr * gm.C) = make_float4(zm[0], zm[1], zm[2], zm[3]);
        }
      }
     }
    });
#pragma unroll
    for (int k = 0; k < NS; ++k) {
      if (k) __syncthreads();
      column_reduce<S::BWD>(t, acc[k], sRed);
      if (t.rsub == 0) {
        float* dst = partial + k * pstride + (((size_t)d * gridDim.x + blockIdx.x) * t.C4 + t.q) * S::BWD;
#pragma unroll
        for (int i = 0; i < S::BWD; ++i) dst[i] = acc[k][i];
      }
    }
    if (gridDim.z == 1) __syncthreads();
  }
}

template <int GS>
__device__ __forceinline__ void cl_bwd_finalize_site(const float* __restrict__ partial, int nrows, const Geom& gm, const BwdFin& fin) {
  using SH = ClShape<GS>;
  const int s = threadIdx.x, d = threadIdx.z, q = blockIdx.x * blockDim.y + threadIdx.y;
  const int W = (gm.C >> 2) * SH::BWD;
  pdl_launch_dependents();
  pdl_wait();
  float a[SH::BWD];
  column_row_sum<SH::BWD>(partial + (size_t)d * nrows * W + (size_t)q * SH::BWD, nrows, W, a);
  if (s < SH::NSUB) {
    float v[SH::BWD1], R[GS][GS], sdz[GS];
    take_group<SH::NSUB, SH::BWD1>(a, s, v);
#pragma unroll
    for (int i = 0; i < SH::BWD1; ++i) {
      if (i < GS * GS) R[i / GS][i % GS] = v[i]; else sdz[i - GS * GS] = v[i];
    }
    bwd_finalize_thread<GS>(gm, fin, d, q * SH::NSUB + s, R, sdz, false);
  }
  if (!((fin.epi & DWT_EPI_AFFINE) && fin.dgamma != nullptr)) return;
  __syncthreads();
  if (d == 0 && s < 4) {
    const int ch = 4 * q + s;
    float sg = 0.f, sb = 0.f;
    for (int dd = 0; dd < gm.D; ++dd) {
      sg += fin.dgb_part[((size_t)dd * 2 + 0) * gm.C + ch];
      sb += fin.dgb_part[((size_t)dd * 2 + 1) * gm.C + ch];
    }
    fin.dgamma[ch] = sg;
    fin.dbeta[ch] = sb;
  }
}

template <int GS>
__global__ void __launch_bounds__(32 * kFinQ * DWT_MAX_DOMAINS) cl_bwd_finalize_kernel(const float* __restrict__ partial, size_t pstride, int nrows,
                                                                                      const Geom gm, const __grid_constant__ BwdFin fin,
                                                                                      const __grid_constant__ BwdFin fin2) {
  const bool second = blockIdx.y != 0;
  cl_bwd_finalize_site<GS>(partial + (second ? pstride : 0), nrows, gm, second ? fin2 : fin);
}

template <int GS>
struct BwdCoef {
  float A1[GS * (GS + 1) / 2], Bm[GS * (GS + 1) / 2], cv[GS];
  __device__ __forceinline__ void load(const float* cf) {
#pragma unroll
    for (int i = 0; i < GS; ++i) {
      cv[i] = __ldg(cf + 2 * GS * GS + i);
#pragma unroll
      for (int j = 0; j <= i; ++j) {
        A1[i * (i + 1) / 2 + j] = __ldg(cf + j * GS + i);
        Bm[i * (i + 1) / 2 + j] = __ldg(cf + GS * GS + i * GS + j);
      }
    }
  }
  __device__ __forceinline__ void apply(const float (&dz)[GS], const float (&xi)[GS], float* o) const {
#pragma unroll
    for (int i = 0; i < GS; ++i) {
      float a = cv[i];
#pragma unroll
      for (int j = i; j < GS; ++j) a = fmaf(A1[j * (j + 1) / 2 + i], dz[j], a);
#pragma unroll
      for (int j = 0; j < GS; ++j) {
        const int hi = i > j ? i : j, lo = i > j ? j : i;
        a = fmaf(Bm[hi * (hi + 1) / 2 + lo], xi[j], a);
      }
      o[i] = a;
    }
  }
};

template <int GS, int EPI, bool D2, bool DS>
__global__ void __launch_bounds__(kT, 2) cl_bwd_apply_kernel(const float* __restrict__ x, const float* __restrict__ dout, const float* __restrict__ dout2,
                                                             float* __restrict__ dx, const Geom gm, const float* __restrict__ coef,
                                                             const float* __restrict__ save_mean, const float* __restrict__ save_w,
                                                             const float* __restrict__ gamma, const float* __restrict__ beta,
                                                             const float* __restrict__ xds, float* __restrict__ dxds,
                                                             const float* __restrict__ coef_d) {
  using S = ClShape<GS>;
  constexpr int UNROLL = 4;
  constexpr bool RELU = (EPI & DWT_EPI_RELU) != 0;
  static_assert((EPI & DWT_EPI_RESIDUAL) == 0, "the residual tail's apply runs with EPI = AFFINE on dz");
  static_assert(!DS || (!D2 && !RELU), "the two-site tail's apply reads dz");
  constexpr int NS = DS ? 2 : 1;
  const ClThread t(gm);
  const unsigned rows = (unsigned)gm.N * gm.HW;
  pdl_wait();
  CL_FOR_DOMAINS(d, gm, false) {
    float Wp[S::NSUB][S::NM], bp[S::NSUB][GS];
    BwdCoef<GS> cf[NS][S::NSUB];
#pragma unroll
    for (int s = 0; s < S::NSUB; ++s) {
      const int g = t.q * S::NSUB + s;
      if constexpr (RELU)
        load_forward_map<GS, EPI>(save_w + ((size_t)d * gm.G + g) * GS * GS, save_mean + (size_t)d * gm.C + g * GS,
                                  gamma + g * GS, beta + g * GS, Wp[s], bp[s]);
#pragma unroll
      for (int k = 0; k < NS; ++k) cf[k][s].load((k ? coef_d : coef) + ((size_t)d * gm.G + g) * coef_stride(GS));
    }
    const size_t base = (size_t)d * rows * gm.C + 4 * t.q;
    const float* xp[NS];
    float* op[NS];
    xp[0] = x + base; op[0] = dx + base;
    if constexpr (DS) { xp[NS - 1] = xds + base; op[NS - 1] = dxds + base; }
    const float* gd = dout + base;
    const float* gd2 = D2 ? dout2 + base : nullptr;
    sweep_rows<UNROLL, false>(t, rows, [&](unsigned r) {
      float4 v[NS][UNROLL], q[UNROLL], q2[D2 ? UNROLL : 1];
#pragma unroll
      for (int u = 0; u < UNROLL; ++u) {
        const unsigned rr = r + u * t.rpi;
        if (rr < rows) {
#pragma unroll
          for (int k = 0; k < NS; ++k) v[k][u] = ldg4(xp[k] + (size_t)rr * gm.C);
          q[u] = ldg4(gd + (size_t)rr * gm.C);
          if constexpr (D2) q2[u] = ldg4(gd2 + (size_t)rr * gm.C);
        }
      }
      if constexpr (D2) {
#pragma unroll
        for (int u = 0; u < UNROLL; ++u)
          if (r + u * t.rpi < rows) { q[u].x += q2[u].x; q[u].y += q2[u].y; q[u].z += q2[u].z; q[u].w += q2[u].w; }
      }
#pragma unroll
      for (int u = 0; u < UNROLL; ++u) {
        const unsigned rr = r + u * t.rpi;
        if (rr < rows) {
          const float ge[4] = {q[u].x, q[u].y, q[u].z, q[u].w};
#pragma unroll
          for (int k = 0; k < NS; ++k) {
            const float e[4] = {v[k][u].x, v[k][u].y, v[k][u].z, v[k][u].w};
            float o[4];
#pragma unroll
            for (int s = 0; s < S::NSUB; ++s) {
              float xi[GS], dz[GS];
#pragma unroll
              for (int c = 0; c < GS; ++c) { xi[c] = e[s * GS + c]; dz[c] = ge[s * GS + c]; }
              if constexpr (RELU) {
                float oi[GS];
                apply_group<GS>(Wp[s], bp[s], xi, oi);
#pragma unroll
                for (int c = 0; c < GS; ++c) dz[c] = oi[c] > 0.f ? dz[c] : 0.f;
              }
              cf[k][s].apply(dz, xi, o + s * GS);
            }
            *reinterpret_cast<float4*>(op[k] + (size_t)rr * gm.C) = make_float4(o[0], o[1], o[2], o[3]);
          }
        }
      }
    });
  }
}

#define CL_GS(GS_, ...)                                  \
  switch (GS_) {                                         \
    case 1: { constexpr int kGS = 1; __VA_ARGS__; break; } \
    case 2: { constexpr int kGS = 2; __VA_ARGS__; break; } \
    case 4: { constexpr int kGS = 4; __VA_ARGS__; break; } \
    default: break;                                      \
  }
#define CL_EPI(E_, ...)                                                   \
  if ((E_) == 3) { constexpr int kEPI = 3; __VA_ARGS__; }                 \
  else if ((E_) == 1) { constexpr int kEPI = 1; __VA_ARGS__; }            \
  else { constexpr int kEPI = 0; __VA_ARGS__; }
#define CL_EPI_BWD(E_, ...)                                               \
  if ((E_) == 7) { constexpr int kEPI = 7; __VA_ARGS__; }                 \
  else CL_EPI(E_, __VA_ARGS__)
#define CL_D2(P_, ...)                                                    \
  if (P_) { constexpr bool kD2 = true; __VA_ARGS__; }                     \
  else { constexpr bool kD2 = false; __VA_ARGS__; }

inline bool use_pdl() {
  static const bool on = [] { const char* v = getenv("DWT_PDL"); return v != nullptr && v[0] == '1'; }();
  return on;
}

template <class... KArgs, class... Args>
inline void launch_k(void (*kernel)(KArgs...), dim3 grid, dim3 block, cudaStream_t st, bool pdl, Args... args) {
  cudaLaunchConfig_t cfg = {};
  cfg.gridDim = grid; cfg.blockDim = block; cfg.dynamicSmemBytes = 0; cfg.stream = st;
  cudaLaunchAttribute attr[1];
  attr[0].id = cudaLaunchAttributeProgrammaticStreamSerialization;
  attr[0].val.programmaticStreamSerializationAllowed = 1;
  cfg.attrs = attr; cfg.numAttrs = pdl ? 1 : 0;
  cudaLaunchKernelEx(&cfg, kernel, KArgs(args)...);
}

inline dim3 cl_grid(const Geom& gm, int nctas, int gz) {
  const int C4 = gm.C / 4, CW = C4 < kT ? C4 : kT;
  return dim3(nctas, C4 / CW, gz);
}

}

bool cl_supports(int C, int GS) {
  if (!(GS == 1 || GS == 2 || GS == 4) || C % 4 != 0) return false;
  const int c4 = C / 4;
  return (c4 & (c4 - 1)) == 0 && c4 <= 16384;
}
int cl_fwd_width(int C, int GS) { return (C / 4) * (4 / GS) * (GS + GS * (GS + 1) / 2); }
int cl_bwd_width(int C, int GS) { return (C / 4) * (4 / GS) * (GS * GS + GS); }


void cl_stats(const float* x, const Geom& gm, int nctas, int gz, float* partial, float* shift, cudaStream_t st) {
  CL_GS(gm.GS, (cl_stats_kernel<kGS><<<cl_grid(gm, nctas, gz), kT, 0, st>>>(x, gm, partial, shift)));
}
inline dim3 fin_block(const Geom& gm) { const int c4 = gm.C / 4; return dim3(32, c4 < kFinQ ? c4 : kFinQ, gm.D); }
void cl_fwd_finalize(const float* partial, int nrows, const float* shift, const Geom& gm, const FwdFin& fin, cudaStream_t st,
                     const FwdFin* fin2, size_t pstride, size_t sstride) {
  const dim3 b = fin_block(gm), g((gm.C / 4) / b.y, fin2 ? 2 : 1);
  CL_GS(gm.GS, (launch_k(cl_fwd_finalize_kernel<kGS>, g, b, st, use_pdl(), partial, pstride, nrows, shift, sstride, gm, fin, fin2 ? *fin2 : fin)));
}
void cl_apply(const float* x, float* y, const Geom& gm, int nctas, int gz, int epi, const float* mean, const float* w,
              const float* gamma, const float* beta, const float* residual, uint8_t* mask, cudaStream_t st) {
  const float* nul = nullptr;
  if (epi == 7) {
    CL_GS(gm.GS, (launch_k(cl_apply_kernel<kGS, 7, false>, cl_grid(gm, nctas, gz), dim3(kT), st, use_pdl(), x, y, gm, mean, w, gamma, beta, residual, mask,
                           nul, nul, nul, nul)));
    return;
  }
  CL_GS(gm.GS, CL_EPI(epi, (launch_k(cl_apply_kernel<kGS, kEPI, false>, cl_grid(gm, nctas, gz), dim3(kT), st, use_pdl(), x, y, gm, mean, w, gamma, beta,
                                     nul, (uint8_t*)nullptr, nul, nul, nul, nul))));
}
void cl_tail2_apply(const float* x, const float* xd, float* y, const Geom& gm, int nctas, int gz, const float* mean, const float* w,
                    const float* gamma, const float* beta, const float* mean_d, const float* w_d, const float* gamma_d,
                    const float* beta_d, uint8_t* mask, cudaStream_t st) {
  CL_GS(gm.GS, (launch_k(cl_apply_kernel<kGS, 7, true>, cl_grid(gm, nctas, gz), dim3(kT), st, use_pdl(), x, y, gm, mean, w, gamma, beta, xd, mask,
                         mean_d, w_d, gamma_d, beta_d)));
}
void cl_bwd_reduce(const float* x, const float* dout, const float* dout2, const Geom& gm, int nctas, int gz, int epi, const float* mean, const float* w,
                   const float* gamma, const float* beta, const uint8_t* mask, float* dz, float* partial, cudaStream_t st) {
  const float* nul = nullptr;
  CL_GS(gm.GS, CL_D2(dout2, CL_EPI_BWD(epi, (cl_bwd_reduce_kernel<kGS, kEPI, kD2, false><<<cl_grid(gm, nctas, gz), kT, 0, st>>>(
                                                x, dout, dout2, gm, mean, w, gamma, beta, mask, dz, partial, nul, nul, 0)))));
}
void cl_tail2_bwd_reduce(const float* x, const float* xd, const float* dout, const float* dout2, const Geom& gm, int nctas, int gz,
                         const float* mean, const float* mean_d, const uint8_t* mask, float* dz, float* partial, size_t pstride,
                         cudaStream_t st) {
  const float* nul = nullptr;
  CL_GS(gm.GS, CL_D2(dout2, (cl_bwd_reduce_kernel<kGS, 7, kD2, true><<<cl_grid(gm, nctas, gz), kT, 0, st>>>(
                                x, dout, dout2, gm, mean, nul, nul, nul, mask, dz, partial, xd, mean_d, pstride))));
}
void cl_bwd_finalize(const float* partial, int nrows, const Geom& gm, const BwdFin& fin, cudaStream_t st, const BwdFin* fin2, size_t pstride) {
  const dim3 b = fin_block(gm), g((gm.C / 4) / b.y, fin2 ? 2 : 1);
  CL_GS(gm.GS, (launch_k(cl_bwd_finalize_kernel<kGS>, g, b, st, use_pdl(), partial, pstride, nrows, gm, fin, fin2 ? *fin2 : fin)));
}
void cl_bwd_apply(const float* x, const float* dout, const float* dout2, float* dx, const Geom& gm, int nctas, int gz, int epi, const float* coef,
                  const float* mean, const float* w, const float* gamma, const float* beta, cudaStream_t st) {
  const float* nul = nullptr;
  CL_GS(gm.GS, CL_D2(dout2, CL_EPI(epi, (launch_k(cl_bwd_apply_kernel<kGS, kEPI, kD2, false>, cl_grid(gm, nctas, gz), dim3(kT), st, use_pdl(), x, dout,
                                                  dout2, dx, gm, coef, mean, w, gamma, beta, nul, (float*)nullptr, nul)))));
}
void cl_tail2_bwd_apply(const float* x, const float* xd, const float* dz, float* dx, float* dxd, const Geom& gm, int nctas, int gz,
                        const float* coef, const float* coef_d, cudaStream_t st) {
  const float* nul = nullptr;
  CL_GS(gm.GS, (launch_k(cl_bwd_apply_kernel<kGS, 1, false, true>, cl_grid(gm, nctas, gz), dim3(kT), st, use_pdl(), x, dz, nul, dx, gm, coef,
                         nul, nul, nul, nul, xd, dxd, coef_d)));
}

}
```

### dwt-domain-adaptation_b200/dwt_b200/csrc/norm_launch.h

```cpp
#pragma once
#include <stdint.h>

#include "dwt_common.cuh"

namespace dwt {

inline void bind_context() {
  thread_local bool bound = false;
  if (!bound) { cudaFree(nullptr); bound = true; }
}

bool small_supports(int GS);
void small_stats(const float* x, const Geom& gm, int vec, const FwdFin& fin, float* partial, int* counters,
                 cudaStream_t st);
void small_eval_prep(const Geom& gm, const FwdFin& fin, cudaStream_t st);
void small_apply(const float* x, float* y, const Geom& gm, int vec, int chunks, int epi, const float* mean,
                 const float* w, const float* gamma, const float* beta, const float* residual, cudaStream_t st);
void small_bwd_reduce(const float* x, const float* dout, const Geom& gm, int vec, const BwdFin& fin,
                      const float* beta, float* partial, int* counters, cudaStream_t st);
void small_bwd_prep(const Geom& gm, const BwdFin& fin, cudaStream_t st);
void small_bwd_apply(const float* x, const float* dout, float* dx, const Geom& gm, int vec, int chunks, int epi,
                     const float* coef, const float* mean, const float* w, const float* gamma, const float* beta,
                     cudaStream_t st);

int tiled_smem_bytes(int GS);
int tiled_init();
void tiled_stats(const float* x, const Geom& gm, int vec, const FwdFin& fin, float* partial, int* counters,
                 cudaStream_t st);
void tiled_eval_prep(const Geom& gm, const FwdFin& fin, cudaStream_t st);
void tiled_apply(const float* x, float* y, const Geom& gm, int vec, int chunks, const float* mean, const float* w,
                 cudaStream_t st);
void tiled_bwd_reduce(const float* x, const float* dout, const Geom& gm, int vec, const BwdFin& fin, float* partial,
                      int* counters, cudaStream_t st);
void tiled_bwd_prep(const Geom& gm, const BwdFin& fin, cudaStream_t st);
void tiled_bwd_apply(const float* x, const float* dout, float* dx, const Geom& gm, int vec, int chunks,
                     const float* coef, cudaStream_t st);

int tc_init();
bool tc_supports(const Geom& gm, int vec);
int tc_superblocks(const Geom& gm);
int tc_stats(const float* x, const Geom& gm, int nchunks, float* shift, float* partial, cudaStream_t st);
int tc_bwd_reduce(const float* x, const float* dout, const Geom& gm, int nchunks, const float* save_mean,
                  float* partial, cudaStream_t st);

int dense_init();
void dense_partial_reduce(const float* partial, int nchunks, int problems, float* gram, cudaStream_t st);
void dense_fwd_factor(const float* gram, const float* shift, const Geom& gm, const FwdFin& fin, cudaStream_t st);
void dense_bwd_coef(const float* rgram, const Geom& gm, const BwdFin& fin, float* dybar, cudaStream_t st);

int tc_apply_init();
int tc_apply(const float* x, float* y, const Geom& gm, int nctas, const float* save_mean, const float* save_w,
             cudaStream_t st);
int tc_bwd_apply(const float* x, const float* dout, float* dx, const Geom& gm, int nctas, const float* coef,
                 const float* save_mean, const float* dybar, cudaStream_t st);

bool cl_supports(int C, int GS);
int cl_fwd_width(int C, int GS);
int cl_bwd_width(int C, int GS);
void cl_stats(const float* x, const Geom& gm, int nctas, int gz, float* partial, float* shift, cudaStream_t st);
void cl_fwd_finalize(const float* partial, int nrows, const float* shift, const Geom& gm, const FwdFin& fin, cudaStream_t st,
                     const FwdFin* fin2 = nullptr, size_t pstride = 0, size_t sstride = 0);
void cl_apply(const float* x, float* y, const Geom& gm, int nctas, int gz, int epi, const float* mean, const float* w,
              const float* gamma, const float* beta, const float* residual, uint8_t* mask, cudaStream_t st);
void cl_bwd_reduce(const float* x, const float* dout, const float* dout2, const Geom& gm, int nctas, int gz, int epi, const float* mean, const float* w,
                   const float* gamma, const float* beta, const uint8_t* mask, float* dz, float* partial, cudaStream_t st);
void cl_bwd_finalize(const float* partial, int nrows, const Geom& gm, const BwdFin& fin, cudaStream_t st,
                     const BwdFin* fin2 = nullptr, size_t pstride = 0);
void cl_bwd_apply(const float* x, const float* dout, const float* dout2, float* dx, const Geom& gm, int nctas, int gz, int epi, const float* coef,
                  const float* mean, const float* w, const float* gamma, const float* beta, cudaStream_t st);
void cl_tail2_apply(const float* x, const float* xd, float* y, const Geom& gm, int nctas, int gz, const float* mean, const float* w,
                    const float* gamma, const float* beta, const float* mean_d, const float* w_d, const float* gamma_d,
                    const float* beta_d, uint8_t* mask, cudaStream_t st);
void cl_tail2_bwd_reduce(const float* x, const float* xd, const float* dout, const float* dout2, const Geom& gm, int nctas, int gz,
                         const float* mean, const float* mean_d, const uint8_t* mask, float* dz, float* partial, size_t pstride,
                         cudaStream_t st);
void cl_tail2_bwd_apply(const float* x, const float* xd, const float* dz, float* dx, float* dxd, const Geom& gm, int nctas, int gz,
                        const float* coef, const float* coef_d, cudaStream_t st);

void maxpool_fwd_launch(const float* x, float* y, uint8_t* idx, int N, int H, int W, int C, int OH, int OW, int k, int s, int p,
                        cudaStream_t st);
void maxpool_bwd_launch(const float* dy, const uint8_t* idx, float* dx, int N, int H, int W, int C, int OH, int OW, int k, int s,
                        int p, cudaStream_t st);

void augment_pair_launch(const uint8_t* images, int B, int SH, int SW, int CR, const int* crop_plain, const int* crop_aug,
                         const uint8_t* flip, const float* affine, const float* mean, const float* stdv,
                         float* out_plain, float* out_aug, int nhwc, cudaStream_t st);
void head_loss_launch(const float* logits, const long long* labels, int B, int K, float lambda, float* losses,
                      float* grad, int* status, cudaStream_t st);
void mec_launch(const float* x, const float* y, int N, int K, float* loss, float* gx, float* gy, cudaStream_t st);

}
```

### dwt-domain-adaptation_b200/dwt_b200/csrc/pool.cu

```cuda
#include "dwt_common.cuh"
#include "norm_launch.h"

namespace dwt {
namespace {

struct PoolGeom {
  int N, H, W, C4, OH, OW, k, s, p, c4shift;
};

template <int K, int S, int P>
__device__ __forceinline__ PoolGeom fixed(PoolGeom g) {
  if constexpr (K > 0) { g.k = K; g.s = S; g.p = P; }
  return g;
}

__device__ __forceinline__ bool takes(float v, float best) { return (v > best) || (v != v); }

template <int K, int S, int P, bool POW2>
__global__ void __launch_bounds__(256) maxpool_fwd_kernel(const float* __restrict__ x, float* __restrict__ y,
                                                          uint8_t* __restrict__ idx, const PoolGeom g0) {
  const PoolGeom g = fixed<K, S, P>(g0);
  const int n = blockIdx.x / g.OH, oh = blockIdx.x - n * g.OH;
  const int h0 = oh * g.s - g.p;
  const float4* xn = reinterpret_cast<const float4*>(x) + (size_t)n * g.H * g.W * g.C4;
  const size_t obase = ((size_t)n * g.OH + oh) * g.OW * g.C4;
  for (int t = threadIdx.x; t < g.OW * g.C4; t += blockDim.x) {
    const int ow = POW2 ? (t >> g.c4shift) : t / g.C4, c4 = t - ow * g.C4;
    const int w0 = ow * g.s - g.p;
    float best[4] = {-INFINITY, -INFINITY, -INFINITY, -INFINITY};
    unsigned bi[4] = {0u, 0u, 0u, 0u};
#pragma unroll
    for (int kh = 0; kh < g.k; ++kh) {
      const int h = h0 + kh;
      if (h < 0 || h >= g.H) continue;
      const float4* xr = xn + (size_t)h * g.W * g.C4 + c4;
#pragma unroll
      for (int kw = 0; kw < g.k; ++kw) {
        const int w = w0 + kw;
        if (w < 0 || w >= g.W) continue;
        const float4 v = __ldg(xr + (size_t)w * g.C4);
        const float e[4] = {v.x, v.y, v.z, v.w};
        const unsigned code = (unsigned)(kh * g.k + kw);
#pragma unroll
        for (int c = 0; c < 4; ++c)
          if (takes(e[c], best[c])) { best[c] = e[c]; bi[c] = code; }
      }
    }
    reinterpret_cast<float4*>(y)[obase + t] = make_float4(best[0], best[1], best[2], best[3]);
    reinterpret_cast<uint32_t*>(idx)[obase + t] = bi[0] | (bi[1] << 8) | (bi[2] << 16) | (bi[3] << 24);
  }
}

template <int K, int S, int P, bool POW2>
__global__ void __launch_bounds__(256) maxpool_bwd_kernel(const float* __restrict__ dy, const uint8_t* __restrict__ idx,
                                                          float* __restrict__ dx, const PoolGeom g0) {
  const PoolGeom g = fixed<K, S, P>(g0);
  const int n = blockIdx.x / g.H, h = blockIdx.x - n * g.H;
  int oh0 = h + g.p - g.k + 1;
  oh0 = oh0 <= 0 ? 0 : (oh0 + g.s - 1) / g.s;
  int oh1 = (h + g.p) / g.s;
  if (oh1 > g.OH - 1) oh1 = g.OH - 1;
  const float4* dyn = reinterpret_cast<const float4*>(dy) + (size_t)n * g.OH * g.OW * g.C4;
  const uint32_t* ixn = reinterpret_cast<const uint32_t*>(idx) + (size_t)n * g.OH * g.OW * g.C4;
  float4* dxr = reinterpret_cast<float4*>(dx) + ((size_t)n * g.H + h) * g.W * g.C4;
  for (int t = threadIdx.x; t < g.W * g.C4; t += blockDim.x) {
    const int w = POW2 ? (t >> g.c4shift) : t / g.C4, c4 = t - w * g.C4;
    int ow0 = w + g.p - g.k + 1;
    ow0 = ow0 <= 0 ? 0 : (ow0 + g.s - 1) / g.s;
    int ow1 = (w + g.p) / g.s;
    if (ow1 > g.OW - 1) ow1 = g.OW - 1;
    float acc[4] = {0.f, 0.f, 0.f, 0.f};
    for (int oh = oh0; oh <= oh1; ++oh) {
      const unsigned kh = (unsigned)(h - (oh * g.s - g.p));
      for (int ow = ow0; ow <= ow1; ++ow) {
        const unsigned code = kh * g.k + (unsigned)(w - (ow * g.s - g.p));
        const size_t o = ((size_t)oh * g.OW + ow) * g.C4 + c4;
        const uint32_t m = __ldg(ixn + o);
        const bool h0 = (m & 0xFFu) == code, h1 = ((m >> 8) & 0xFFu) == code, h2 = ((m >> 16) & 0xFFu) == code, h3 = (m >> 24) == code;
        if (h0 || h1 || h2 || h3) {
          const float4 gq = __ldg(dyn + o);
          if (h0) acc[0] += gq.x;
          if (h1) acc[1] += gq.y;
          if (h2) acc[2] += gq.z;
          if (h3) acc[3] += gq.w;
        }
      }
    }
    dxr[t] = make_float4(acc[0], acc[1], acc[2], acc[3]);
  }
}

__global__ void __launch_bounds__(256) maxpool_fwd_3s2_kernel(const float* __restrict__ x, float* __restrict__ y,
                                                              uint8_t* __restrict__ idx, const PoolGeom g) {
  const int OH2 = g.OH >> 1, OW2 = g.OW >> 1;
  const int n = blockIdx.y / OH2, a = blockIdx.y - n * OH2;
  const int i = blockIdx.x * blockDim.x + threadIdx.x;
  if (i >= OW2 * g.C4) return;
  const int b = i >> g.c4shift, c4 = i & (g.C4 - 1);
  const float4* xn = reinterpret_cast<const float4*>(x) + (size_t)n * g.H * g.W * g.C4 + c4;
  float best[2][2][4];
  unsigned bi[2][2][4];
#pragma unroll
  for (int oa = 0; oa < 2; ++oa)
#pragma unroll
    for (int ob = 0; ob < 2; ++ob)
#pragma unroll
      for (int c = 0; c < 4; ++c) { best[oa][ob][c] = -INFINITY; bi[oa][ob][c] = 0u; }
  const int h0 = 4 * a - 1, w0 = 4 * b - 1;
#pragma unroll
  for (int r = 0; r < 5; ++r) {
    const int h = h0 + r;
    if (h < 0 || h >= g.H) continue;
    float4 row[5];
    bool in[5];
#pragma unroll
    for (int cc = 0; cc < 5; ++cc) {
      const int w = w0 + cc;
      in[cc] = w >= 0 && w < g.W;
      row[cc] = in[cc] ? __ldg(xn + ((size_t)h * g.W + w) * g.C4) : make_float4(0.f, 0.f, 0.f, 0.f);
    }
#pragma unroll
    for (int oa = 0; oa < 2; ++oa) {
      const int kh = r - 2 * oa;
      if (kh < 0 || kh > 2) continue;
#pragma unroll
      for (int ob = 0; ob < 2; ++ob)
#pragma unroll
        for (int kw = 0; kw < 3; ++kw) {
          const int cc = 2 * ob + kw;
          if (!in[cc]) continue;
          const float e[4] = {row[cc].x, row[cc].y, row[cc].z, row[cc].w};
          const unsigned code = (unsigned)(kh * 3 + kw);
#pragma unroll
          for (int c = 0; c < 4; ++c)
            if (takes(e[c], best[oa][ob][c])) { best[oa][ob][c] = e[c]; bi[oa][ob][c] = code; }
        }
    }
  }
#pragma unroll
  for (int oa = 0; oa < 2; ++oa)
#pragma unroll
    for (int ob = 0; ob < 2; ++ob) {
      const size_t o = (((size_t)n * g.OH + 2 * a + oa) * g.OW + 2 * b + ob) * g.C4 + c4;
      reinterpret_cast<float4*>(y)[o] = make_float4(best[oa][ob][0], best[oa][ob][1], best[oa][ob][2], best[oa][ob][3]);
      reinterpret_cast<uint32_t*>(idx)[o] = bi[oa][ob][0] | (bi[oa][ob][1] << 8) | (bi[oa][ob][2] << 16) | (bi[oa][ob][3] << 24);
    }
}

__device__ __forceinline__ void take(float4& acc, const float4& gq, uint32_t m, unsigned code) {
  if ((m & 0xFFu) == code) acc.x += gq.x;
  if (((m >> 8) & 0xFFu) == code) acc.y += gq.y;
  if (((m >> 16) & 0xFFu) == code) acc.z += gq.z;
  if ((m >> 24) == code) acc.w += gq.w;
}

__global__ void __launch_bounds__(256) maxpool_bwd_3s2_kernel(const float* __restrict__ dy, const uint8_t* __restrict__ idx,
                                                              float* __restrict__ dx, const PoolGeom g) {
  const int H2 = g.H >> 1, W2 = g.W >> 1;
  const int n = blockIdx.y / H2, k = blockIdx.y - n * H2;
  const int i = blockIdx.x * blockDim.x + threadIdx.x;
  if (i >= W2 * g.C4) return;
  const int j = i >> g.c4shift, c4 = i & (g.C4 - 1);
  const float4* dyn = reinterpret_cast<const float4*>(dy) + (size_t)n * g.OH * g.OW * g.C4;
  const uint32_t* ixn = reinterpret_cast<const uint32_t*>(idx) + (size_t)n * g.OH * g.OW * g.C4;
  uint32_t m[2][2];
  float4 gq[2][2];
#pragma unroll
  for (int a = 0; a < 2; ++a)
#pragma unroll
    for (int b = 0; b < 2; ++b) {
      const bool ok = (k + a < g.OH) && (j + b < g.OW);
      const size_t o = ((size_t)(k + a) * g.OW + (j + b)) * g.C4 + c4;
      m[a][b] = ok ? __ldg(ixn + o) : 0xFFFFFFFFu;
      gq[a][b] = ok ? __ldg(dyn + o) : make_float4(0.f, 0.f, 0.f, 0.f);
    }
  float4 o00 = make_float4(0.f, 0.f, 0.f, 0.f), o01 = o00, o10 = o00, o11 = o00;
  take(o00, gq[0][0], m[0][0], 4u);
  take(o01, gq[0][0], m[0][0], 5u); take(o01, gq[0][1], m[0][1], 3u);
  take(o10, gq[0][0], m[0][0], 7u); take(o10, gq[1][0], m[1][0], 1u);
  take(o11, gq[0][0], m[0][0], 8u); take(o11, gq[0][1], m[0][1], 6u); take(o11, gq[1][0], m[1][0], 2u); take(o11, gq[1][1], m[1][1], 0u);
  float4* r0 = reinterpret_cast<float4*>(dx) + (((size_t)n * g.H + 2 * k) * g.W + 2 * j) * g.C4 + c4;
  float4* r1 = r0 + (size_t)g.W * g.C4;
  r0[0] = o00; r0[g.C4] = o01;
  r1[0] = o10; r1[g.C4] = o11;
}

}

namespace {
int pow2_shift(int v) {
  int sh = 0;
  while ((1 << sh) < v) ++sh;
  return (1 << sh) == v ? sh : -1;
}
}

void maxpool_fwd_launch(const float* x, float* y, uint8_t* idx, int N, int H, int W, int C, int OH, int OW, int k, int s, int p,
                        cudaStream_t st) {
  const int sh = pow2_shift(C / 4);
  const PoolGeom g{N, H, W, C / 4, OH, OW, k, s, p, sh < 0 ? 0 : sh};
  if (k == 3 && s == 2 && p == 1 && sh >= 0 && H % 4 == 0 && W % 4 == 0 && (long long)N * (OH / 2) <= 65535) {
    const int items = (OW / 2) * (C / 4), threads = items >= 256 ? 256 : ((items + 31) / 32) * 32;
    maxpool_fwd_3s2_kernel<<<dim3((items + threads - 1) / threads, N * (OH / 2)), threads, 0, st>>>(x, y, idx, g);
  } else if (k == 3 && s == 2 && p == 1 && sh >= 0) maxpool_fwd_kernel<3, 2, 1, true><<<N * OH, 256, 0, st>>>(x, y, idx, g);
  else maxpool_fwd_kernel<0, 0, 0, false><<<N * OH, 256, 0, st>>>(x, y, idx, g);
}

void maxpool_bwd_launch(const float* dy, const uint8_t* idx, float* dx, int N, int H, int W, int C, int OH, int OW, int k, int s,
                        int p, cudaStream_t st) {
  const int sh = pow2_shift(C / 4);
  const PoolGeom g{N, H, W, C / 4, OH, OW, k, s, p, sh < 0 ? 0 : sh};
  if (k == 3 && s == 2 && p == 1 && sh >= 0 && H % 2 == 0 && W % 2 == 0 && (long long)N * (H / 2) <= 65535) {
    const int items = (W / 2) * (C / 4), threads = items >= 256 ? 256 : ((items + 31) / 32) * 32;
    maxpool_bwd_3s2_kernel<<<dim3((items + threads - 1) / threads, N * (H / 2)), threads, 0, st>>>(dy, idx, dx, g);
  } else if (k == 3 && s == 2 && p == 1 && sh >= 0) maxpool_bwd_kernel<3, 2, 1, true><<<N * H, 256, 0, st>>>(dy, idx, dx, g);
  else maxpool_bwd_kernel<0, 0, 0, false><<<N * H, 256, 0, st>>>(dy, idx, dx, g);
}

}
```

### dwt-domain-adaptation_b200/dwt_b200/functional.py

```python
from __future__ import annotations

import torch

from . import _native as nv


def _dense(x: torch.Tensor, group_size: int):
    n, c = x.shape[0], x.shape[1]
    hw = 1
    for s in x.shape[2:]:
        hw *= s
    nhwc = (x.dim() == 4 and not x.is_contiguous() and x.is_contiguous(memory_format=torch.channels_last)
            and nv.channels_last_supported(c, group_size))
    if not nhwc and not x.is_contiguous():
        x = x.contiguous()
    return x, n, c, hw, nhwc


def _check_param(name, t, numel):
    if t is None:
        return
    if t.numel() != numel:
        raise ValueError(f"{name} has {t.numel()} elements, expected {numel}")
    if not t.is_contiguous():
        raise ValueError(f"{name} must be contiguous (it is written / read through a raw pointer)")


class _NormFunction(torch.autograd.Function):

    @staticmethod
    def forward(ctx, x, gamma, beta, residual, kind, group_size, n_domains, mode, eps, momentum, update_running,
                running, relu):
        lib = nv.lib()
        gs = group_size if kind == "whiten" else 1
        x, n_all, c, hw, nhwc = _dense(x, gs)
        layout = nv.LAYOUT_NHWC if nhwc else 0
        if n_all % n_domains != 0:
            raise ValueError(f"batch of {n_all} does not split into {n_domains} domains")
        n = n_all // n_domains
        dev = nv.require_cuda(x, gamma, beta, residual, *[t for pair in running for t in pair])
        for d, (rm_t, rv_t) in enumerate(running):
            _check_param(f"running mean of domain {d}", rm_t, c)
            _check_param(f"running second moment of domain {d}", rv_t, c * gs)
        _check_param("gamma / weight", gamma, c)
        _check_param("beta / bias", beta, c)
        epi = nv.EPI_NONE
        if residual is not None:
            if gamma is None or not relu or residual.shape != x.shape:
                raise ValueError("a fused residual needs gamma/beta, relu=True and a tensor shaped like x")
            residual = residual.contiguous(memory_format=torch.channels_last) if nhwc else residual.contiguous()
        if gamma is not None:
            epi = nv.EPI_AFFINE | (nv.EPI_RELU if relu else 0) | (nv.EPI_RESIDUAL if residual is not None else 0)
            gamma_c, beta_c = gamma.detach().reshape(-1).contiguous(), beta.detach().reshape(-1).contiguous()
        else:
            gamma_c = beta_c = None
        y = torch.empty_like(x)
        mask = torch.empty(x.numel() // 4, dtype=torch.uint8, device=dev) if (residual is not None and nhwc) else None
        save_mean = torch.empty(n_domains, c, dtype=torch.float32, device=dev)
        save_w = torch.empty(n_domains, c // gs, gs, gs, dtype=torch.float32, device=dev)
        ws = nv.workspace(dev, n, c, hw, gs, n_domains)
        need_running = (mode == nv.MODE_EVAL) or update_running
        rm = nv.ptr_array([p[0] for p in running]) if need_running else None
        rv = nv.ptr_array([p[1] for p in running]) if need_running else None
        with torch.cuda.device(dev):
            if kind == "whiten":
                rc = lib.dwt_whiten_fwd(nv.ptr(x), nv.ptr(y), n, c, hw, gs, n_domains, mode | layout, eps, momentum,
                                        int(update_running), rm, rv, nv.ptr(gamma_c), nv.ptr(beta_c), nv.ptr(residual),
                                        nv.ptr(mask), epi, nv.ptr(save_mean), nv.ptr(save_w), nv.ptr(ws), ws.numel(),
                                        nv.stream_ptr(dev))
            else:
                rc = lib.dwt_bn_fwd(nv.ptr(x), nv.ptr(y), n, c, hw, n_domains, mode | layout, eps, momentum,
                                    int(update_running), rm, rv, nv.ptr(gamma_c), nv.ptr(beta_c), nv.ptr(residual),
                                    nv.ptr(mask), epi, nv.ptr(save_mean), nv.ptr(save_w), nv.ptr(ws), ws.numel(),
                                    nv.stream_ptr(dev))
        nv.check(rc)
        nv.poll_status(dev)
        if update_running and mode == nv.MODE_TRAIN:
            seen = set()
            for pair in running:
                for buf in pair:
                    if buf is not None and id(buf) not in seen:
                        seen.add(id(buf))
                        torch.autograd.graph.increment_version(buf)
        ctx.residual_mode = None
        if mask is not None:
            ctx.save_for_backward(x, save_mean, save_w, gamma_c, beta_c, mask)
            ctx.residual_mode = "mask"
        elif residual is not None:
            ctx.save_for_backward(x, save_mean, save_w, gamma_c, beta_c, y)
            epi = nv.EPI_AFFINE
            ctx.residual_mode = "aten"
        else:
            ctx.save_for_backward(x, save_mean, save_w, gamma_c, beta_c)
        ctx.cfg = (kind, gs, n_domains, mode | layout, eps, epi, n, c, hw, None if gamma is None else gamma.shape)
        return y

    @staticmethod
    def backward(ctx, dout):
        lib = nv.lib()
        mask = None
        if ctx.residual_mode == "mask":
            x, save_mean, save_w, gamma_c, beta_c, mask = ctx.saved_tensors
        elif ctx.residual_mode == "aten":
            x, save_mean, save_w, gamma_c, beta_c, out = ctx.saved_tensors
            extra = ctx.__dict__.pop("_dwt_extra_grad", None)
            if extra is not None:
                dout = dout + extra
            dout = torch.ops.aten.threshold_backward(dout, out, 0)
        else:
            x, save_mean, save_w, gamma_c, beta_c = ctx.saved_tensors
        kind, gs, n_domains, mode, eps, epi, n, c, hw, gshape = ctx.cfg
        dout2 = ctx.__dict__.pop("_dwt_extra_grad", None)
        if dout2 is not None and not ((mode & nv.LAYOUT_NHWC) and dout2.shape == dout.shape and dout2.dtype == torch.float32
                                      and dout2.is_contiguous(memory_format=torch.channels_last)):
            dout, dout2 = dout + dout2, None
        dout = dout.contiguous(memory_format=torch.channels_last) if (mode & nv.LAYOUT_NHWC) else dout.contiguous()
        dev = nv.require_cuda(dout)
        dx = torch.empty_like(x)
        want_affine = gamma_c is not None and (ctx.needs_input_grad[1] or ctx.needs_input_grad[2])
        d_res = None
        if ctx.residual_mode == "mask":
            d_res = torch.empty_like(x)
        elif ctx.residual_mode == "aten" and ctx.needs_input_grad[3]:
            d_res = dout
        dgamma = torch.empty(c, dtype=torch.float32, device=dev) if want_affine else None
        dbeta = torch.empty(c, dtype=torch.float32, device=dev) if want_affine else None
        ws = nv.workspace(dev, n, c, hw, gs, n_domains)
        with torch.cuda.device(dev):
            if kind == "whiten":
                rc = lib.dwt_whiten_bwd(nv.ptr(x), nv.ptr(dout), nv.ptr(dout2), nv.ptr(dx), n, c, hw, gs, n_domains, mode, eps,
                                        nv.ptr(save_mean), nv.ptr(save_w), nv.ptr(gamma_c), nv.ptr(beta_c), nv.ptr(mask),
                                        nv.ptr(d_res) if mask is not None else None, epi,
                                        nv.ptr(dgamma), nv.ptr(dbeta), nv.ptr(ws), ws.numel(), nv.stream_ptr(dev))
            else:
                rc = lib.dwt_bn_bwd(nv.ptr(x), nv.ptr(dout), nv.ptr(dout2), nv.ptr(dx), n, c, hw, n_domains, mode,
                                    nv.ptr(save_mean), nv.ptr(save_w), nv.ptr(gamma_c), nv.ptr(beta_c), nv.ptr(mask),
                                    nv.ptr(d_res) if mask is not None else None, epi,
                                    nv.ptr(dgamma), nv.ptr(dbeta), nv.ptr(ws), ws.numel(), nv.stream_ptr(dev))
        nv.check(rc)
        if want_affine:
            dgamma, dbeta = dgamma.view(gshape), dbeta.view(gshape)
        return (dx, dgamma, dbeta, d_res if ctx.needs_input_grad[3] else None) + (None,) * 9


class _TailPairFunction(torch.autograd.Function):

    @staticmethod
    def forward(ctx, x, xd, gamma, beta, gamma_d, beta_d, kind, group_size, n_domains, sites):
        lib = nv.lib()
        gs = group_size if kind == "whiten" else 1
        if not (x.dim() == 4 and x.shape == xd.shape and _dense(x, gs)[4] and _dense(xd, gs)[4]):
            raise ValueError("the two-site tail takes two channels-last tensors of one shape with a channels-last build")
        if x.shape[0] % n_domains != 0:
            raise ValueError(f"batch of {x.shape[0]} does not split into {n_domains} domains")
        n_all, c = x.shape[0], x.shape[1]
        hw = x.shape[2] * x.shape[3]
        n = n_all // n_domains
        dev = nv.require_cuda(x, xd, gamma, beta, gamma_d, beta_d, *[t for run, *_ in sites for pair in run for t in pair])
        params = [(gamma, beta), (gamma_d, beta_d)]
        c_sites = (nv.TailSite * 2)()
        keep = []
        saved = []
        for k, (inp, (g, b), (running, eps, momentum, update)) in enumerate(zip((x, xd), params, sites)):
            for d, (rm_t, rv_t) in enumerate(running):
                _check_param(f"running mean of domain {d}", rm_t, c)
                _check_param(f"running second moment of domain {d}", rv_t, c * gs)
            _check_param("gamma / weight", g, c)
            _check_param("beta / bias", b, c)
            g_c, b_c = g.detach().reshape(-1).contiguous(), b.detach().reshape(-1).contiguous()
            save_mean = torch.empty(n_domains, c, dtype=torch.float32, device=dev)
            save_w = torch.empty(n_domains, c // gs, gs, gs, dtype=torch.float32, device=dev)
            rm = nv.ptr_array([pr[0] for pr in running]) if update else None
            rv = nv.ptr_array([pr[1] for pr in running]) if update else None
            c_sites[k] = nv.TailSite(inp.data_ptr(), eps, momentum, int(update), rm, rv, g_c.data_ptr(), b_c.data_ptr(),
                                     save_mean.data_ptr(), save_w.data_ptr(), None, None, None)
            keep += [g_c, b_c, rm, rv]
            saved += [save_mean, save_w, g_c]
        y = torch.empty_like(x)
        mask = torch.empty(x.numel() // 4, dtype=torch.uint8, device=dev)
        ws = nv.workspace(dev, n, c, hw, gs, n_domains)
        nv_kind = nv.KIND_WHITEN if kind == "whiten" else nv.KIND_BN
        with torch.cuda.device(dev):
            rc = lib.dwt_tail2_fwd(nv_kind, c_sites, nv.ptr(y), nv.ptr(mask), n, c, hw, gs, n_domains, nv.ptr(ws), ws.numel(),
                                   nv.stream_ptr(dev))
        nv.check(rc)
        nv.poll_status(dev)
        seen = set()
        for running, _, _, update in sites:
            for buf in (t for pair in running for t in pair) if update else ():
                if id(buf) not in seen:
                    seen.add(id(buf))
                    torch.autograd.graph.increment_version(buf)
        ctx.save_for_backward(x, xd, mask, *saved)
        ctx.cfg = (nv_kind, gs, n_domains, n, c, hw, [s[1] for s in sites], gamma.shape, gamma_d.shape)
        return y

    @staticmethod
    def backward(ctx, dout):
        lib = nv.lib()
        x, xd, mask, mean0, w0, g0, mean1, w1, g1 = ctx.saved_tensors
        nv_kind, gs, n_domains, n, c, hw, eps, gshape, gshape_d = ctx.cfg
        dout2 = ctx.__dict__.pop("_dwt_extra_grad", None)
        if dout2 is not None and not (dout2.shape == dout.shape and dout2.dtype == torch.float32
                                      and dout2.is_contiguous(memory_format=torch.channels_last)):
            dout, dout2 = dout + dout2, None
        dout = dout.contiguous(memory_format=torch.channels_last)
        dev = nv.require_cuda(dout)
        dz = torch.empty_like(x)
        dx, dxd = torch.empty_like(x), torch.empty_like(xd)
        grads = [torch.empty(2, c, dtype=torch.float32, device=dev) for _ in range(2)]
        c_sites = (nv.TailSite * 2)()
        for k, (inp, mean, w, g, d_in, gr) in enumerate(zip((x, xd), (mean0, mean1), (w0, w1), (g0, g1), (dx, dxd), grads)):
            c_sites[k] = nv.TailSite(inp.data_ptr(), eps[k], 0.0, 0, None, None, g.data_ptr(), g.data_ptr(), mean.data_ptr(),
                                     w.data_ptr(), d_in.data_ptr(), gr[0].data_ptr(), gr[1].data_ptr())
        ws = nv.workspace(dev, n, c, hw, gs, n_domains)
        with torch.cuda.device(dev):
            rc = lib.dwt_tail2_bwd(nv_kind, c_sites, nv.ptr(dout), nv.ptr(dout2), nv.ptr(mask), nv.ptr(dz), n, c, hw, gs, n_domains,
                                   nv.ptr(ws), ws.numel(), nv.stream_ptr(dev))
        nv.check(rc)
        return (dx, dxd, grads[0][0].view(gshape), grads[0][1].view(gshape), grads[1][0].view(gshape_d),
                grads[1][1].view(gshape_d)) + (None,) * 4


def tail_pair(x, xd, gamma, beta, gamma_d, beta_d, *, kind, group_size, n_domains, sites):
    return _TailPairFunction.apply(x, xd, gamma, beta, gamma_d, beta_d, kind, group_size, n_domains,
                                   [(r, float(e), float(m), bool(u)) for r, e, m, u in sites])


class _ForkForSum(torch.autograd.Function):

    @staticmethod
    def forward(ctx, y):
        ctx.producer = y.grad_fn
        return y.view_as(y), y.view_as(y)

    @staticmethod
    def backward(ctx, ga, gb):
        producer, ctx.producer = ctx.producer, None
        if ga is None or gb is None:
            return ga if gb is None else gb
        if producer is None or "_dwt_extra_grad" in producer.__dict__:
            return ga + gb
        producer.__dict__["_dwt_extra_grad"] = gb
        return ga


def fork_for_sum(y):
    fn = getattr(y, "grad_fn", None)
    if not torch.is_grad_enabled() or fn is None or not isinstance(fn, (_NormFunction._backward_cls, _TailPairFunction._backward_cls)):
        return y, y
    return _ForkForSum.apply(y)


def norm(x, gamma, beta, *, kind, group_size, n_domains, training_stats, eps, momentum, update_running,
         running, relu=False, residual=None):
    mode = nv.MODE_TRAIN if training_stats else nv.MODE_EVAL
    return _NormFunction.apply(x, gamma, beta, residual, kind, group_size, n_domains, mode, float(eps),
                               float(momentum), bool(update_running), running, bool(relu))


class _MecFunction(torch.autograd.Function):
    @staticmethod
    def forward(ctx, x, y):
        lib = nv.lib()
        if x.dim() != 2 or x.shape != y.shape:
            raise ValueError(f"expected two [N, K] logit tensors, got {tuple(x.shape)} and {tuple(y.shape)}")
        x, y = x.contiguous(), y.contiguous()
        dev = nv.require_cuda(x, y)
        loss = torch.empty((), dtype=torch.float32, device=dev)
        gx, gy = torch.empty_like(x), torch.empty_like(y)
        with torch.cuda.device(dev):
            rc = lib.dwt_mec_fwd_bwd(nv.ptr(x), nv.ptr(y), x.shape[0], x.shape[1], nv.ptr(loss), nv.ptr(gx),
                                     nv.ptr(gy), nv.stream_ptr(dev))
        nv.check(rc)
        ctx.save_for_backward(gx, gy)
        return loss

    @staticmethod
    def backward(ctx, g):
        gx, gy = ctx.saved_tensors
        return g * gx, g * gy


def mec_loss(x, y):
    return _MecFunction.apply(x, y)


class _HeadLossFunction(torch.autograd.Function):
    @staticmethod
    def forward(ctx, logits, labels, lam):
        lib = nv.lib()
        if logits.dim() != 2 or logits.shape[0] % 3 != 0 or labels.dim() != 1 or labels.shape[0] * 3 != logits.shape[0]:
            raise ValueError(f"expected logits [3B, K] and labels [B], got {tuple(logits.shape)} and {tuple(labels.shape)}")
        logits = logits.contiguous()
        dev = nv.require_cuda(logits)
        if not labels.is_cuda or labels.dtype != torch.int64:
            raise nv.NativeError("labels must be an int64 CUDA tensor")
        labels = labels.contiguous()
        losses = torch.empty(3, dtype=torch.float32, device=dev)
        grad = torch.empty_like(logits)
        with torch.cuda.device(dev):
            rc = lib.dwt_head_loss_fwd_bwd(nv.ptr(logits), nv.ptr(labels), labels.shape[0], logits.shape[1], float(lam),
                                           nv.ptr(losses), nv.ptr(grad), nv.status_ptr(dev), nv.stream_ptr(dev))
        nv.check(rc)
        nv.poll_status(dev)
        ctx.save_for_backward(grad)
        ctx.mark_non_differentiable(losses)
        return losses[0], losses

    @staticmethod
    def backward(ctx, g, _unused):
        (grad,) = ctx.saved_tensors
        return g * grad, None, None


def head_loss(logits, labels, lambda_mec):
    return _HeadLossFunction.apply(logits, labels, lambda_mec)
```

### dwt-domain-adaptation_b200/dwt_b200/fused.py

```python
from __future__ import annotations

import torch
import torch.nn as nn

from . import _native as nv
from . import functional as F


class DomainTripleNorm(nn.Module):
    def __init__(self, kind, num_features, group_size=4, n_domains=3):
        super().__init__()
        if kind not in ("whiten", "bn"):
            raise ValueError("kind must be 'whiten' or 'bn'")
        self.kind, self.num_features, self.n_domains = kind, num_features, n_domains
        self.group_size = min(num_features, group_size) if kind == "whiten" else 1
        self.kernel_epilogue = self.group_size in (1, 2, 4)

    def forward(self, x, domain_modules, gamma, beta, relu=False, residual=None, replicated=False, count_batches=True):
        mods = list(domain_modules)
        if len(mods) != self.n_domains:
            raise ValueError(f"expected {self.n_domains} domain modules")
        if x.dim() != 4:
            raise ValueError('expected 4D input (got {}D input)'.format(x.dim()))
        if replicated:
            return self._forward_replicated(x, mods, gamma, beta, relu, residual, count_batches)
        running, eps, momentum, update = self._running_args(mods, count_batches)
        if not self.kernel_epilogue:
            y = F.norm(x, None, None, kind=self.kind, group_size=self.group_size, n_domains=self.n_domains,
                       training_stats=True, eps=eps, momentum=momentum, update_running=update, running=running)
            return self._tensor_epilogue(y, gamma, beta, relu, residual)
        return F.norm(x, gamma, beta, kind=self.kind, group_size=self.group_size, n_domains=self.n_domains,
                      training_stats=True, eps=eps, momentum=momentum, update_running=update,
                      running=running, relu=relu, residual=residual)

    def _running_args(self, mods, count_batches):
        m0 = mods[0]
        if self.kind == "whiten":
            running = [(m.running_mean, m.running_variance) for m in mods]
            eps, momentum = m0.eps, m0.momentum
        else:
            if count_batches:
                counters = [m.num_batches_tracked for m in mods if m.training and m.track_running_stats]
                if counters:
                    torch._foreach_add_(counters, 1)
            running = [(m.running_mean, m.running_var) for m in mods]
            eps = m0.eps
            momentum = m0.momentum if m0.momentum is not None else 1.0 / m0.num_batches_tracked.item()
        return running, eps, momentum, m0.training and m0.track_running_stats

    def forward_with_downsample(self, x, domain_modules, gamma, beta, xd, down, down_modules, down_gamma, down_beta,
                                count_batches=True):
        mods, down_mods = list(domain_modules), list(down_modules)
        pair = (self.kernel_epilogue and down.kernel_epilogue and self.kind == down.kind
                and self.group_size == down.group_size and self.n_domains == down.n_domains
                and len(mods) == len(down_mods) == self.n_domains and x.dim() == 4 and x.shape == xd.shape
                and all(t.is_contiguous(memory_format=torch.channels_last) and not t.is_contiguous() for t in (x, xd))
                and nv.channels_last_supported(x.shape[1], self.group_size))
        if not pair:
            identity = down(xd, down_mods, down_gamma, down_beta, relu=False, count_batches=count_batches)
            return self(x, mods, gamma, beta, True, residual=identity, count_batches=count_batches)
        down_args = down._running_args(down_mods, count_batches)
        site_args = self._running_args(mods, count_batches)
        return F.tail_pair(x, xd, gamma, beta, down_gamma, down_beta, kind=self.kind, group_size=self.group_size,
                           n_domains=self.n_domains, sites=(site_args, down_args))

    @staticmethod
    def _tensor_epilogue(y, gamma, beta, relu, residual):
        if residual is not None and not relu:
            raise ValueError("a fused residual needs relu=True")
        if gamma is not None:
            y = y * gamma + beta
        if residual is not None:
            y = y + residual
        return torch.relu(y) if relu else y

    def _forward_replicated(self, x, mods, gamma, beta, relu, residual, count_batches=True):
        second = "running_variance" if self.kind == "whiten" else "running_var"
        keep = {}
        for m in mods:
            if not (m.training and m.track_running_stats):
                continue
            if self.kind == "bn":
                if count_batches:
                    m.num_batches_tracked += 1
                f = m.momentum if m.momentum is not None else 1.0 / m.num_batches_tracked.item()
            else:
                f = m.momentum
            rm, rv = m.running_mean, getattr(m, second)
            key = (rm.data_ptr(), rv.data_ptr())
            prod, _ = keep.get(key, (1.0, None))
            keep[key] = (prod * (1.0 - f), (rm, rv))
        means = {k[0] for k in keep}
        seconds = {k[1] for k in keep}
        if len(means) != len(keep) or len(seconds) != len(keep):
            raise ValueError("replicated statistics need each running_mean paired with one second-moment buffer")
        m0 = mods[0]
        common = dict(kind=self.kind, group_size=self.group_size, n_domains=1, training_stats=True, eps=m0.eps)
        if self.kernel_epilogue:
            common.update(relu=relu, residual=residual)
            g_arg, b_arg = gamma, beta
        else:
            g_arg = b_arg = None
        if not keep:
            out = F.norm(x, g_arg, b_arg, momentum=0.0, update_running=False,
                         running=[(m0.running_mean, getattr(m0, second))], **common)
        else:
            out = None
            for prod, pair in keep.values():
                y = F.norm(x, g_arg, b_arg, momentum=1.0 - prod, update_running=True, running=[pair], **common)
                out = y if out is None else out
        return out if self.kernel_epilogue else self._tensor_epilogue(out, gamma, beta, relu, residual)
```

### harness/resnet50_dwt.py

```python
from __future__ import annotations

import torch
import torch.nn as nn

_STAGES = ((64, 3, 1), (128, 4, 2), (256, 6, 2), (512, 3, 2))
_DOMAINS = ("s", "t", "t_aug")
EXPANSION = 4


_REPLICATED = [False]
_BATCHED_COUNTERS = [False]


class WhitenScaleShift(nn.Module):

    def __init__(self, layers, planes, group_size, running_mean, running_variance,
                 track_running_stats=True, affine=True):
        super().__init__()
        self.planes, self.group_size, self.affine = planes, group_size, affine
        self.wh = layers.WTransform2d(planes, group_size, running_m=running_mean,
                                      running_var=running_variance,
                                      track_running_stats=track_running_stats)
        if affine:
            self.gamma = nn.Parameter(torch.ones(planes, 1, 1))
            self.beta = nn.Parameter(torch.zeros(planes, 1, 1))

    def forward(self, x):
        y = self.wh(x)
        return y * self.gamma + self.beta if self.affine else y


class _SiteOwner(nn.Module):

    def _add_site(self, layers, tag, key, planes, whiten, group_size, stats, site_mode):
        pre, post = ("downsample_", "") if tag == "downsample" else ("", tag)
        names = [f"{pre}bn{d}{post}" if d != "t_aug" else f"{pre}bnt{post}_aug" for d in _DOMAINS]
        if whiten:
            rm, rv = stats[key + ".wh.running_mean"], stats[key + ".wh.running_variance"]
            gamma, beta = stats[key + ".gamma"], stats[key + ".beta"]
            mods = [WhitenScaleShift(layers, planes, group_size, rm, rv, affine=False) for _ in names]
        else:
            rm, rv = stats[key + ".running_mean"], stats[key + ".running_var"]
            gamma, beta = stats[key + ".weight"].view(-1, 1, 1), stats[key + ".bias"].view(-1, 1, 1)
            mods = [layers.BatchNorm2d(num_features=planes, running_m=rm, running_v=rv, affine=False)
                    for _ in names]
        for n, m in zip(names, mods):
            setattr(self, n, m)
        gname = f"{pre}gamma{post}" if pre == "" else "downsample_gamma"
        bname = f"{pre}beta{post}" if pre == "" else "downsample_beta"
        setattr(self, gname, nn.Parameter(gamma))
        setattr(self, bname, nn.Parameter(beta))
        if not hasattr(self, "_sites"):
            self._sites = {}
        self._sites[tag] = (names, gname, bname, whiten)
        if site_mode == "fused":
            object.__setattr__(self, f"_fused_{tag}", layers.DomainTripleNorm(
                kind="whiten" if whiten else "bn", num_features=planes,
                group_size=group_size if whiten else 1))

    def _site(self, tag, x, relu, residual=None):
        names, gname, bname, whiten = self._sites[tag]
        gamma, beta = getattr(self, gname), getattr(self, bname)
        if residual is not None:
            fused = getattr(self, f"_fused_{tag}", None) if self.training else None
            if fused is not None:
                mods = [getattr(self, n) for n in names]
                return fused(x, [m.wh if whiten else m for m in mods], gamma, beta, True, residual=residual,
                             replicated=_REPLICATED[0], count_batches=not _BATCHED_COUNTERS[0])
            return torch.relu_(self._site(tag, x, relu=False) + residual)
        if self.training:
            fused = getattr(self, f"_fused_{tag}", None)
            mods = [getattr(self, n) for n in names]
            if fused is not None:
                return fused(x, [m.wh if whiten else m for m in mods], gamma, beta, relu, replicated=_REPLICATED[0],
                             count_batches=not _BATCHED_COUNTERS[0])
            if _REPLICATED[0]:
                raise RuntimeError("replicated statistics collection needs site_mode='fused'")
            parts = torch.split(x, x.shape[0] // 3, dim=0)
            s, t, a = (m(p) for m, p in zip(mods, parts))
            out = torch.cat((s, torch.cat((t, a), dim=0)), dim=0) * gamma + beta
        else:
            out = getattr(self, names[1])(x) * gamma + beta
        return torch.relu_(out) if relu else out


class Bottleneck(_SiteOwner):
    def __init__(self, layers, inplanes, planes, layer, sub_layer, stats, group_size, stride,
                 downsample, site_mode):
        super().__init__()
        whiten = layer == 1
        key = f"layer{layer}.{sub_layer}"
        self.conv1 = nn.Conv2d(inplanes, planes, 1, bias=False)
        self._add_site(layers, "1", key + ".bn1", planes, whiten, group_size, stats, site_mode)
        self.conv2 = nn.Conv2d(planes, planes, 3, stride=stride, padding=1, bias=False)
        self._add_site(layers, "2", key + ".bn2", planes, whiten, group_size, stats, site_mode)
        self.conv3 = nn.Conv2d(planes, planes * EXPANSION, 1, bias=False)
        self._add_site(layers, "3", key + ".bn3", planes * EXPANSION, whiten, group_size, stats, site_mode)
        self.downsample = downsample
        if downsample is not None:
            self._add_site(layers, "downsample", f"layer{layer}.0.downsample_bn", planes * EXPANSION,
                           whiten, group_size, stats, site_mode)
        object.__setattr__(self, "_fork", getattr(layers, "fork_for_sum", None) if site_mode == "fused" else None)

    def forward(self, x):
        xa, xb = self._fork(x) if (self._fork is not None and self.training) else (x, x)
        out = self._site("1", self.conv1(xa), relu=True)
        out = self._site("2", self.conv2(out), relu=True)
        if self.downsample is None:
            return self._site("3", self.conv3(out), relu=True, residual=xb)
        tail = getattr(self, "_fused_3", None) if (self.training and not _REPLICATED[0]) else None
        if tail is None:
            identity = self._site("downsample", self.downsample(xb), relu=False)
            return self._site("3", self.conv3(out), relu=True, residual=identity)
        xd = self.downsample(xb)
        names, gname, bname, whiten = self._sites["3"]
        dnames, dgname, dbname, _ = self._sites["downsample"]
        unwrap = (lambda m: m.wh) if whiten else (lambda m: m)
        return tail.forward_with_downsample(
            self.conv3(out), [unwrap(getattr(self, n)) for n in names], getattr(self, gname), getattr(self, bname),
            xd, self._fused_downsample, [unwrap(getattr(self, n)) for n in dnames], getattr(self, dgname),
            getattr(self, dbname), count_batches=not _BATCHED_COUNTERS[0])


class ResNet50DWT(_SiteOwner):
    def __init__(self, layers, state_dict, num_classes=65, group_size=4, site_mode="modules", stem_pad=0, stem_nchw=False,
                 stem_s2d=False):
        super().__init__()
        self.stem_s2d = stem_s2d
        self.stem_nchw = stem_nchw
        self.stem_pad = stem_pad
        if site_mode not in ("modules", "fused"):
            raise ValueError("site_mode must be 'modules' or 'fused'")
        stats = {k: v for k, v in state_dict.items() if "bn" in k or "downsample" in k}
        self.site_mode = site_mode
        self.conv1 = nn.Conv2d(3, 64, 7, stride=2, padding=3, bias=False)
        self._add_site(layers, "1", "bn1", 64, True, group_size, stats, site_mode)
        self.maxpool = nn.MaxPool2d(3, stride=2, padding=1)
        inplanes = 64
        for li, (planes, blocks, stride) in enumerate(_STAGES, start=1):
            seq = []
            for b in range(blocks):
                down = None
                if b == 0 and (stride != 1 or inplanes != planes * EXPANSION):
                    down = nn.Sequential(nn.Conv2d(inplanes, planes * EXPANSION, 1, stride=stride, bias=False))
                seq.append(Bottleneck(layers, inplanes, planes, li, b, stats, 4, stride if b == 0 else 1,
                                      down, site_mode))
                inplanes = planes * EXPANSION
            setattr(self, f"layer{li}", nn.Sequential(*seq))
        self.avgpool = nn.AdaptiveAvgPool2d((1, 1))
        self.fc_out = nn.Linear(512 * EXPANSION, num_classes)
        for m in self.modules():
            if isinstance(m, nn.Conv2d):
                nn.init.kaiming_normal_(m.weight, mode="fan_out", nonlinearity="relu")

    def _stem_s2d(self, x):
        n, c, h, w = x.shape
        if h % 2 or w % 2:
            return self.conv1(x)
        cl = x.is_contiguous(memory_format=torch.channels_last) and not x.is_contiguous()
        xp = torch.nn.functional.pad(x, (3, 3, 3, 3))
        hp, wp = (h + 6) // 2, (w + 6) // 2
        wt = torch.nn.functional.pad(self.conv1.weight, (0, 1, 0, 1))
        o = wt.shape[0]
        if cl:
            xs = xp.view(n, c, hp, 2, wp, 2).permute(0, 2, 4, 1, 3, 5).reshape(n, hp, wp, 4 * c).permute(0, 3, 1, 2)
            w4 = wt.view(o, c, 4, 2, 4, 2).permute(0, 2, 4, 1, 3, 5).reshape(o, 4, 4, 4 * c).permute(0, 3, 1, 2)
        else:
            xs = xp.view(n, c, hp, 2, wp, 2).permute(0, 1, 3, 5, 2, 4).reshape(n, 4 * c, hp, wp)
            w4 = wt.view(o, c, 4, 2, 4, 2).permute(0, 1, 3, 5, 2, 4).reshape(o, 4 * c, 4, 4)
        return torch.nn.functional.conv2d(xs, w4)

    def _stem(self, x):
        if self.stem_s2d:
            return self._stem_s2d(x)
        if self.stem_nchw:
            return self.conv1(x.contiguous()).contiguous(memory_format=torch.channels_last)
        if not self.stem_pad or x.shape[1] >= self.stem_pad:
            return self.conv1(x)
        extra = self.stem_pad - x.shape[1]
        fmt = torch.channels_last if (x.is_contiguous(memory_format=torch.channels_last) and not x.is_contiguous()) \
            else torch.contiguous_format
        xp = torch.zeros((x.shape[0], self.stem_pad) + tuple(x.shape[2:]), dtype=x.dtype, device=x.device).contiguous(memory_format=fmt)
        xp[:, :x.shape[1]] = x
        w = torch.nn.functional.pad(self.conv1.weight, (0, 0, 0, 0, 0, extra))
        if fmt == torch.channels_last:
            w = w.contiguous(memory_format=torch.channels_last)
        c = self.conv1
        return torch.nn.functional.conv2d(xp, w, None, c.stride, c.padding, c.dilation, c.groups)

    def _bump_counters(self):
        cs = getattr(self, "_bn_counters", None)
        if cs is None:
            cs = [m.num_batches_tracked for m in self.modules()
                  if hasattr(m, "num_batches_tracked") and m.num_batches_tracked is not None and getattr(m, "track_running_stats", False)]
            object.__setattr__(self, "_bn_counters", cs)
        if cs:
            torch._foreach_add_(cs, 1)

    def forward(self, x):
        batched = self.training and self.site_mode == "fused"
        if batched:
            self._bump_counters()
        _BATCHED_COUNTERS[0] = batched
        try:
            x = self.maxpool(self._site("1", self._stem(x), relu=True))
            x = self.layer4(self.layer3(self.layer2(self.layer1(x))))
        finally:
            _BATCHED_COUNTERS[0] = False
        return self.fc_out(torch.flatten(self.avgpool(x), 1))


def build_resnet50_dwt(state_dict, layers, site_mode="modules", num_classes=65, channels_last=False, stem_pad=0,
                       stem_nchw=False, stem_s2d=False):
    model = ResNet50DWT(layers, state_dict, num_classes=num_classes, site_mode=site_mode, stem_pad=stem_pad,
                        stem_nchw=stem_nchw and channels_last, stem_s2d=stem_s2d)
    model.load_state_dict(state_dict, strict=False)
    if channels_last and hasattr(layers, "MaxPool2d"):
        model.maxpool = layers.MaxPool2d(3, stride=2, padding=1)
    if channels_last:
        for m in model.modules():
            if isinstance(m, nn.Conv2d) and not (model.stem_nchw and m is model.conv1):
                m.weight.data = m.weight.data.contiguous(memory_format=torch.channels_last)
    return model


def collect_stats(model, batches, passes=1, replicated=True):
    was_training = model.training
    model.train(True)
    out = None
    try:
        with torch.no_grad():
            for _ in range(passes):
                for data in batches:
                    if replicated:
                        _REPLICATED[0] = True
                        out = model(data)
                    else:
                        out = model(torch.cat((data, data, data), dim=0))
    finally:
        _REPLICATED[0] = False
        model.train(was_training)
    return out
```

### include/dwt_b200.h

```cpp
#ifndef DWT_B200_H_
#define DWT_B200_H_

#include <stddef.h>
#include <stdint.h>

#ifdef __cplusplus
extern "C" {
#endif

#define DWT_B200_ABI_VERSION 6
#define DWT_MAX_DOMAINS 4
#define DWT_MAX_GROUP_SIZE 64

#define DWT_OK 0
#define DWT_E_INVALID (-1)
#define DWT_E_WORKSPACE (-2)
#define DWT_E_LAUNCH (-3)
#define DWT_E_UNSUPPORTED (-4)

#define DWT_MODE_TRAIN 0
#define DWT_MODE_EVAL 1

#define DWT_LAYOUT_NHWC 0x100

#define DWT_EPI_NONE 0
#define DWT_EPI_AFFINE 1
#define DWT_EPI_RELU 2
#define DWT_EPI_RESIDUAL 4

typedef struct CUstream_st *dwt_stream_t;

#if defined(__GNUC__)
#define DWT_API __attribute__((visibility("default")))
#else
#define DWT_API
#endif

DWT_API int dwt_abi_version(void);
DWT_API const char *dwt_last_error(void);

DWT_API size_t dwt_workspace_bytes(int64_t N, int64_t C, int64_t HW, int group_size, int n_domains);

#define DWT_STATUS_NOT_PD 1
#define DWT_STATUS_BAD_LABEL 2

DWT_API int dwt_whiten_fwd(const float *x, float *y, int64_t N, int64_t C, int64_t HW, int group_size,
                   int n_domains, int mode, float eps, float momentum, int update_running,
                   float *const *running_mean, float *const *running_cov, const float *gamma,
                   const float *beta, const float *residual, uint8_t *relu_mask, int epilogue, float *save_mean,
                   float *save_w, void *workspace, size_t workspace_bytes, dwt_stream_t stream);

DWT_API int dwt_whiten_bwd(const float *x, const float *dout, const float *dout2, float *dx, int64_t N, int64_t C, int64_t HW,
                   int group_size, int n_domains, int mode, float eps, const float *save_mean,
                   const float *save_w, const float *gamma, const float *beta, const uint8_t *relu_mask,
                   float *dresidual, int epilogue, float *dgamma, float *dbeta, void *workspace,
                   size_t workspace_bytes, dwt_stream_t stream);

DWT_API int dwt_bn_fwd(const float *x, float *y, int64_t N, int64_t C, int64_t HW, int n_domains, int mode,
               float eps, float factor, int update_running, float *const *running_mean,
               float *const *running_var, const float *weight, const float *bias, const float *residual,
               uint8_t *relu_mask, int epilogue, float *save_mean, float *save_invstd, void *workspace,
               size_t workspace_bytes, dwt_stream_t stream);

DWT_API int dwt_bn_bwd(const float *x, const float *dout, const float *dout2, float *dx, int64_t N, int64_t C, int64_t HW,
               int n_domains, int mode, const float *save_mean, const float *save_invstd,
               const float *weight, const float *bias, const uint8_t *relu_mask, float *dresidual, int epilogue,
               float *dweight, float *dbias, void *workspace, size_t workspace_bytes, dwt_stream_t stream);

#define DWT_KIND_WHITEN 0
#define DWT_KIND_BN 1
typedef struct {
  const float *x;
  float eps, momentum;
  int update_running;
  float *const *running_mean;
  float *const *running_cov;
  const float *gamma, *beta;
  float *save_mean, *save_w;
  float *dx;
  float *dgamma, *dbeta;
} dwt_tail_site;

DWT_API int dwt_tail2_fwd(int kind, const dwt_tail_site *sites, float *y, uint8_t *relu_mask, int64_t N, int64_t C,
                  int64_t HW, int group_size, int n_domains, void *workspace, size_t workspace_bytes,
                  dwt_stream_t stream);
DWT_API int dwt_tail2_bwd(int kind, const dwt_tail_site *sites, const float *dout, const float *dout2,
                  const uint8_t *relu_mask, float *dz, int64_t N, int64_t C, int64_t HW, int group_size,
                  int n_domains, void *workspace, size_t workspace_bytes, dwt_stream_t stream);

DWT_API int dwt_mec_fwd_bwd(const float *x, const float *y, int64_t N, int64_t K, float *loss, float *gx,
                    float *gy, dwt_stream_t stream);

DWT_API int dwt_head_loss_fwd_bwd(const float *logits, const int64_t *labels, int64_t B, int64_t K, float lambda,
                          float *losses, float *grad, int *status, dwt_stream_t stream);

DWT_API int dwt_augment_pair(const uint8_t *images, int64_t B, int src_h, int src_w, int crop, const int32_t *crop_plain,
                     const int32_t *crop_aug, const uint8_t *flip, const float *affine, const float *mean,
                     const float *stdv, float *out_plain, float *out_aug, int layout, dwt_stream_t stream);

DWT_API int dwt_maxpool_fwd(const float *x, float *y, uint8_t *argmax, int64_t N, int64_t H, int64_t W, int64_t C,
                    int kernel, int stride, int padding, dwt_stream_t stream);
DWT_API int dwt_maxpool_bwd(const float *dy, const uint8_t *argmax, float *dx, int64_t N, int64_t H, int64_t W, int64_t C,
                    int kernel, int stride, int padding, dwt_stream_t stream);

typedef struct {
  char name[48];
  int64_t launches;
  double ms;
  double bytes;
} dwt_profile_entry;

DWT_API int64_t dwt_launch_count(void);
DWT_API void dwt_profile_begin(void);
DWT_API int dwt_profile_end(dwt_profile_entry *out, int max_entries);

#ifdef __cplusplus
}
#endif
#endif
```

Before: 2895.

## Fuse stem whitening/BN apply with 3x3 stride-2 max-pool in forward and backward

Adds a fused stem-site + max-pool path. The forward apply kernel normalizes, applies ReLU and max-pools in one pass, writing only the pooled output and argmax. The backward reduce and apply kernels scatter the pooled gradient back through argmax on the fly, so the full-resolution activation and its gradient are never materialized. This cuts memory traffic and launches at the largest-resolution site, at the cost of more index arithmetic and new kernels that only cover the supported shapes.

After: 2919, median of 6. No clear change (+0.8%).

```diff
diff --git a/dwt-domain-adaptation_b200/dwt_b200/_native.py b/dwt-domain-adaptation_b200/dwt_b200/_native.py
--- a/dwt-domain-adaptation_b200/dwt_b200/_native.py
+++ b/dwt-domain-adaptation_b200/dwt_b200/_native.py
@@ -9,7 +9,7 @@
 _HERE = os.path.dirname(os.path.abspath(__file__))
 LIB_PATH = os.environ.get("DWT_B200_LIB") or os.path.join(_HERE, "lib", "libdwt_b200.so")
 
-ABI_VERSION = 6
+ABI_VERSION = 7
 MAX_DOMAINS = 4
 MAX_GROUP_SIZE = 64
 MODE_TRAIN, MODE_EVAL = 0, 1
@@ -58,6 +58,13 @@
     "dwt_tail2_bwd": (ctypes.c_int, [ctypes.c_int, ctypes.POINTER(TailSite), _c_float_p, _c_float_p, ctypes.c_void_p,
                                      _c_float_p, ctypes.c_int64, ctypes.c_int64, ctypes.c_int64, ctypes.c_int, ctypes.c_int,
                                      ctypes.c_void_p, ctypes.c_size_t, ctypes.c_void_p]),
+    "dwt_site_maxpool_fwd": (ctypes.c_int, [ctypes.c_int, ctypes.POINTER(TailSite), _c_float_p, ctypes.c_void_p, ctypes.c_int64,
+                                            ctypes.c_int64, ctypes.c_int64, ctypes.c_int64, ctypes.c_int, ctypes.c_int, ctypes.c_int,
+                                            ctypes.c_int, ctypes.c_int, ctypes.c_void_p, ctypes.c_size_t, ctypes.c_void_p]),
+    "dwt_site_maxpool_bwd": (ctypes.c_int, [ctypes.c_int, ctypes.POINTER(TailSite), _c_float_p, _c_float_p, ctypes.c_void_p,
+                                            ctypes.c_int64, ctypes.c_int64, ctypes.c_int64, ctypes.c_int64, ctypes.c_int, ctypes.c_int,
+                                            ctypes.c_int, ctypes.c_int, ctypes.c_int, ctypes.c_void_p, ctypes.c_size_t,
+                                            ctypes.c_void_p]),
     "dwt_mec_fwd_bwd": (ctypes.c_int, [_c_float_p, _c_float_p, ctypes.c_int64, ctypes.c_int64, _c_float_p,
                                        _c_float_p, _c_float_p, ctypes.c_void_p]),
     "dwt_head_loss_fwd_bwd": (ctypes.c_int, [_c_float_p, ctypes.c_void_p, ctypes.c_int64, ctypes.c_int64, ctypes.c_float,
diff --git a/dwt-domain-adaptation_b200/dwt_b200/csrc/api.cu b/dwt-domain-adaptation_b200/dwt_b200/csrc/api.cu
--- a/dwt-domain-adaptation_b200/dwt_b200/csrc/api.cu
+++ b/dwt-domain-adaptation_b200/dwt_b200/csrc/api.cu
@@ -586,6 +586,92 @@
   return check_launch("channels-last two-site backward apply kernel");
 }
 
+int site_pool_plan(Plan& p, int kind, const dwt_tail_site* s, const void* out, const uint8_t* argmax, int64_t N, int64_t C, int64_t H,
+                   int64_t W, int GS, int D, int k, int stride, int pad) {
+  if (kind != DWT_KIND_WHITEN && kind != DWT_KIND_BN) return fail(DWT_E_INVALID, "bad kind %d", kind);
+  if (kind == DWT_KIND_BN && GS != 1) return fail(DWT_E_INVALID, "batch norm has group_size 1 (got %d)", GS);
+  if (!s) return fail(DWT_E_INVALID, "null pointer argument");
+  if (k != 3 || stride != 2 || pad != 1)
+    return fail(DWT_E_UNSUPPORTED, "the fused site + max-pool is built for kernel 3, stride 2, padding 1 (got %d/%d/%d)", k, stride, pad);
+  if (H <= 0 || W <= 0 || H % 4 != 0 || W % 4 != 0)
+    return fail(DWT_E_UNSUPPORTED, "the fused site + max-pool needs H and W multiples of 4 (got %lldx%lld)", (long long)H, (long long)W);
+  if (int rc = make_plan(p, K_STATS, K_APPLY, s->x, out, nullptr, N, C, H * W, GS, D)) return rc;
+  if (!dwt::cl_supports((int)C, GS))
+    return fail(DWT_E_UNSUPPORTED, "the fused site + max-pool runs on the channels-last kernels: group_size 1, 2, 4 with C/4 a power of two "
+                "(C=%lld gs=%d)", (long long)C, GS);
+  if ((int64_t)D * N * (H / 2) > 65535) return fail(DWT_E_UNSUPPORTED, "too many image rows for the pooled kernels' grids");
+  if (!s->x || !s->gamma || !s->beta || !s->save_mean || !s->save_w || !out || !argmax) return fail(DWT_E_INVALID, "null pointer argument");
+  if ((((uintptr_t)s->x | (uintptr_t)out) % 16) != 0 || (uintptr_t)argmax % 4 != 0)
+    return fail(DWT_E_INVALID, "channels-last tensors must be 16-byte aligned");
+  return DWT_OK;
+}
+
+int site_pool_fwd(int kind, const dwt_tail_site* s, float* y, uint8_t* argmax, int64_t N, int64_t C, int64_t H, int64_t W, int GS, int D,
+                  int k, int stride, int pad, void* ws, size_t ws_bytes, cudaStream_t st) {
+  Plan p;
+  if (int rc = site_pool_plan(p, kind, s, y, argmax, N, C, H, W, GS, D, k, stride, pad)) return rc;
+  if (int rc = check_running(s->update_running != 0, s->running_mean, s->running_cov, D)) return rc;
+  if (!ws) return fail(DWT_E_INVALID, "null pointer argument");
+  const Workspace w = carve(ws, C, GS, D);
+  if (w.bytes > ws_bytes) return fail(DWT_E_WORKSPACE, "workspace too small: need %zu bytes, got %zu", w.bytes, ws_bytes);
+  if ((uintptr_t)ws % 256 != 0) return fail(DWT_E_WORKSPACE, "workspace must be 256-byte aligned");
+  const SiteConst sc = site_const(kind, s->eps, N, H * W);
+  const dwt::FwdFin fin = make_fwd_fin(sc.a, sc.b, s->momentum, sc.unbias, s->update_running, s->update_running != 0, s->running_mean,
+                                       s->running_cov, s->save_mean, s->save_w, w, D);
+  const double E = 4.0 * (double)D * (double)N * (double)C * (double)(H * W);
+  const ClPlan cp = cl_plan(p.gm, 3, 3, 8, 8);
+  {
+    Launch l("cl_stats", &p.gm, E, st);
+    dwt::cl_stats(s->x, p.gm, cp.nred, cp.gz_red, w.partial, w.shift, st);
+  }
+  if (int rc = check_launch("channels-last statistics kernel")) return rc;
+  {
+    Launch l("cl_fwd_finalize", &p.gm, 0.0, st);
+    dwt::cl_fwd_finalize(w.partial, cp.nred, w.shift, p.gm, fin, st);
+  }
+  if (int rc = check_launch("channels-last finalize kernel")) return rc;
+  {
+    Launch l("cl_apply_pool", &p.gm, 1.3125 * E, st);
+    dwt::cl_apply_pool(s->x, y, argmax, p.gm, (int)H, (int)W, s->save_mean, s->save_w, s->gamma, s->beta, st);
+  }
+  return check_launch("channels-last apply + max-pool kernel");
+}
+
+int site_pool_bwd(int kind, const dwt_tail_site* s, const float* dout, const float* dout2, const uint8_t* argmax, int64_t N, int64_t C,
+                  int64_t H, int64_t W, int GS, int D, int k, int stride, int pad, void* ws, size_t ws_bytes, cudaStream_t st) {
+  Plan p;
+  if (int rc = site_pool_plan(p, kind, s, dout, argmax, N, C, H, W, GS, D, k, stride, pad)) return rc;
+  if (!s->dx) return fail(DWT_E_INVALID, "null pointer argument");
+  if ((((uintptr_t)dout2 | (uintptr_t)s->dx) % 16) != 0) return fail(DWT_E_INVALID, "channels-last tensors must be 16-byte aligned");
+  if ((s->dgamma == nullptr) != (s->dbeta == nullptr)) return fail(DWT_E_INVALID, "dgamma and dbeta go together");
+  if (!ws) return fail(DWT_E_INVALID, "null pointer argument");
+  const Workspace w = carve(ws, C, GS, D);
+  if (w.bytes > ws_bytes) return fail(DWT_E_WORKSPACE, "workspace too small: need %zu bytes, got %zu", w.bytes, ws_bytes);
+  if ((uintptr_t)ws % 256 != 0) return fail(DWT_E_WORKSPACE, "workspace must be 256-byte aligned");
+  const int epi = DWT_EPI_AFFINE | DWT_EPI_RELU;
+  const dwt::BwdFin fin = make_bwd_fin(site_const(kind, s->eps, N, H * W).a, DWT_MODE_TRAIN, epi, s->save_mean, s->save_w, s->gamma,
+                                       s->dgamma, s->dbeta, w);
+  const double E = 4.0 * (double)D * (double)N * (double)C * (double)(H * W);
+  const double pooled = (dout2 ? 0.5 : 0.25) + 0.0625;
+  const ClPlan cp = cl_plan(p.gm, 2, 2, 4, 4);
+  {
+    Launch l("cl_pool_bwd_reduce", &p.gm, (1.0 + pooled) * E, st);
+    dwt::cl_pool_bwd_reduce(s->x, dout, dout2, argmax, p.gm, (int)H, (int)W, cp.nred, cp.gz_red, s->save_mean, s->save_w, s->gamma,
+                            s->beta, w.partial, st);
+  }
+  if (int rc = check_launch("channels-last pooled backward reduction kernel")) return rc;
+  {
+    Launch l("cl_bwd_finalize", &p.gm, 0.0, st);
+    dwt::cl_bwd_finalize(w.partial, cp.nred, p.gm, fin, st);
+  }
+  if (int rc = check_launch("channels-last backward finalize kernel")) return rc;
+  {
+    Launch l("cl_pool_bwd_apply", &p.gm, (2.0 + pooled) * E, st);
+    dwt::cl_pool_bwd_apply(s->x, dout, dout2, argmax, s->dx, p.gm, (int)H, (int)W, w.coef, s->save_mean, s->save_w, s->gamma, s->beta, st);
+  }
+  return check_launch("channels-last pooled backward apply kernel");
+}
+
 }
 
 extern "C" {
@@ -651,6 +737,20 @@
                   dwt_stream_t stream) {
   return tail2_bwd(kind, sites, dout, dout2, relu_mask, dz, N, C, HW, group_size, n_domains, workspace, workspace_bytes,
                    (cudaStream_t)stream);
+}
+
+int dwt_site_maxpool_fwd(int kind, const dwt_tail_site* site, float* y, uint8_t* argmax, int64_t N, int64_t C, int64_t H, int64_t W,
+                         int group_size, int n_domains, int kernel, int stride, int padding, void* workspace, size_t workspace_bytes,
+                         dwt_stream_t stream) {
+  return site_pool_fwd(kind, site, y, argmax, N, C, H, W, group_size, n_domains, kernel, stride, padding, workspace, workspace_bytes,
+                       (cudaStream_t)stream);
+}
+
+int dwt_site_maxpool_bwd(int kind, const dwt_tail_site* site, const float* dout, const float* dout2, const uint8_t* argmax, int64_t N,
+                         int64_t C, int64_t H, int64_t W, int group_size, int n_domains, int kernel, int stride, int padding,
+                         void* workspace, size_t workspace_bytes, dwt_stream_t stream) {
+  return site_pool_bwd(kind, site, dout, dout2, argmax, N, C, H, W, group_size, n_domains, kernel, stride, padding, workspace,
+                       workspace_bytes, (cudaStream_t)stream);
 }
 
 int dwt_mec_fwd_bwd(const float* x, const float* y, int64_t N, int64_t K, float* loss, float* gx, float* gy,
diff --git a/dwt-domain-adaptation_b200/dwt_b200/csrc/norm_cl.cu b/dwt-domain-adaptation_b200/dwt_b200/csrc/norm_cl.cu
--- a/dwt-domain-adaptation_b200/dwt_b200/csrc/norm_cl.cu
+++ b/dwt-domain-adaptation_b200/dwt_b200/csrc/norm_cl.cu
@@ -2,6 +2,7 @@
 
 #include "dwt_common.cuh"
 #include "norm_launch.h"
+#include "pool_3s2.cuh"
 #include "small_algebra.cuh"
 
 namespace dwt {
@@ -42,6 +43,36 @@
   for (int di_ = blockIdx.z, d = (DESC) ? (gm).D - 1 - di_ : di_; di_ < (gm).D; di_ += gridDim.z, d = (DESC) ? (gm).D - 1 - di_ : di_)
 
 __device__ __forceinline__ float4 ldg4(const float* p) { return __ldg(reinterpret_cast<const float4*>(p)); }
+
+struct ClPool {
+  const uint8_t* idx;
+  int H, W, OH, OW, c4shift;
+};
+
+struct PoolPos {
+  unsigned i = 0, h = 0, w = 0;
+  PoolPos() = default;
+  __device__ __forceinline__ PoolPos(const ClPool& pl, const Geom& gm, unsigned rr) {
+    i = rr / (unsigned)gm.HW;
+    const unsigned p = rr - i * (unsigned)gm.HW;
+    h = p / (unsigned)pl.W;
+    w = p - h * (unsigned)pl.W;
+  }
+  __device__ __forceinline__ void advance(const ClPool& pl, unsigned by) {
+    w += by;
+    while (w >= (unsigned)pl.W) {
+      w -= (unsigned)pl.W;
+      if (++h == (unsigned)pl.H) { h = 0; ++i; }
+    }
+  }
+};
+
+template <bool D2>
+__device__ __forceinline__ float4 pooled_grad(const float* __restrict__ dp, const float* __restrict__ dp2, const ClPool& pl,
+                                              const Geom& gm, int d, const PoolPos& pp, int q) {
+  const unsigned o = ((((unsigned)d * gm.N + pp.i) * pl.OH + (pp.h >> 1)) * pl.OW + (pp.w >> 1)) * (unsigned)(gm.C >> 2) + q;
+  return pool3s2_pixel_grad<D2>(dp, dp2, pl.idx, o, (int)pp.h, (int)pp.w, pl.OH, pl.OW, gm.C >> 2);
+}
 
 template <int NACC>
 __device__ __forceinline__ void column_reduce(const ClThread& t, float (&acc)[NACC], float* sRed) {
@@ -328,6 +359,47 @@
 }
 
 template <int GS>
+__global__ void __launch_bounds__(256) cl_apply_pool_kernel(const float* __restrict__ x, float* __restrict__ y, uint8_t* __restrict__ idx,
+                                                            const Geom gm, const ClPool pl, const float* __restrict__ save_mean,
+                                                            const float* __restrict__ save_w, const float* __restrict__ gamma,
+                                                            const float* __restrict__ beta) {
+  using S = ClShape<GS>;
+  constexpr int EPI = DWT_EPI_AFFINE | DWT_EPI_RELU;
+  const int C4 = gm.C >> 2, OH2 = pl.OH >> 1;
+  const int n = blockIdx.y / OH2, a = blockIdx.y - n * OH2, d = n / gm.N;
+  const int i = blockIdx.x * blockDim.x + threadIdx.x;
+  pdl_wait();
+  if (i >= (pl.OW >> 1) * C4) return;
+  const int b = i >> pl.c4shift, q = i & (C4 - 1);
+  float Wp[S::NSUB][S::NM], bp[S::NSUB][GS];
+#pragma unroll
+  for (int s = 0; s < S::NSUB; ++s) {
+    const int g = q * S::NSUB + s;
+    load_forward_map<GS, EPI>(save_w + ((size_t)d * gm.G + g) * GS * GS, save_mean + (size_t)d * gm.C + g * GS,
+                              gamma + g * GS, beta + g * GS, Wp[s], bp[s]);
+  }
+  const float* xn = x + (size_t)n * gm.HW * gm.C + 4 * q;
+  float best[2][2][4];
+  unsigned bi[2][2][4];
+  pool3s2_patch(pl.H, pl.W, a, b, [&](int h, int w) {
+    const float4 v = ldg4(xn + ((size_t)h * pl.W + w) * gm.C);
+    const float e[4] = {v.x, v.y, v.z, v.w};
+    float o[4];
+#pragma unroll
+    for (int s = 0; s < S::NSUB; ++s) {
+      float xi[GS], oi[GS];
+#pragma unroll
+      for (int c = 0; c < GS; ++c) xi[c] = e[s * GS + c];
+      apply_group<GS>(Wp[s], bp[s], xi, oi);
+#pragma unroll
+      for (int c = 0; c < GS; ++c) o[s * GS + c] = fmaxf(oi[c], 0.f);
+    }
+    return make_float4(o[0], o[1], o[2], o[3]);
+  }, best, bi);
+  pool3s2_store(y, idx, (((size_t)n * pl.OH + 2 * a) * pl.OW + 2 * b) * C4 + q, pl.OW, C4, best, bi);
+}
+
+template <int GS>
 __device__ __forceinline__ void bwd_accumulate(float* acc, const float (&dz)[GS], const float (&xi)[GS], const float* mu) {
 #pragma unroll
   for (int i = 0; i < GS; ++i) {
@@ -337,19 +409,21 @@
   }
 }
 
-template <int GS, int EPI, bool D2, bool DS>
+template <int GS, int EPI, bool D2, bool DS, bool POOL>
 __global__ void __launch_bounds__(kT, 2) cl_bwd_reduce_kernel(const float* __restrict__ x, const float* __restrict__ dout, const float* __restrict__ dout2,
                                                               const Geom gm, const float* __restrict__ save_mean,
                                                               const float* __restrict__ save_w, const float* __restrict__ gamma,
                                                               const float* __restrict__ beta, const uint8_t* __restrict__ mask,
                                                               float* __restrict__ dzout, float* __restrict__ partial,
                                                               const float* __restrict__ xds, const float* __restrict__ save_mean_d,
-                                                              size_t pstride) {
+                                                              size_t pstride, const ClPool pl) {
   using S = ClShape<GS>;
   constexpr int UNROLL = 4;
   constexpr bool MASK = (EPI & DWT_EPI_RESIDUAL) != 0;
   constexpr bool RELU = (EPI & DWT_EPI_RELU) != 0 && !MASK;
   static_assert(!DS || MASK, "the two-site tail is a residual epilogue");
+  static_assert(!POOL || (RELU && !DS), "the stem site's pool follows its ReLU");
+  constexpr bool ADD2 = D2 && !POOL;
   constexpr int NS = DS ? 2 : 1;
   __shared__ float sRed[kT * S::BWD];
   const ClThread t(gm);
@@ -379,15 +453,17 @@
     xp[0] = x + base;
     if constexpr (DS) xp[NS - 1] = xds + base;
     const float* gd = dout + base;
-    const float* gd2 = D2 ? dout2 + base : nullptr;
+    const float* gd2 = ADD2 ? dout2 + base : nullptr;
     float* zd = MASK ? dzout + base : nullptr;
     const uint8_t* md = mask + (size_t)d * rows * t.C4 + t.q;
-    constexpr int H = DS ? UNROLL / 2 : UNROLL;
+    constexpr int H = (DS || POOL) ? UNROLL / 2 : UNROLL;
     sweep_rows<UNROLL, true>(t, rows, [&](unsigned r0) {
+      PoolPos pp;
+      if constexpr (POOL) pp = PoolPos(pl, gm, r0);
 #pragma unroll
      for (int h = 0; h < UNROLL; h += H) {
       const unsigned r = r0 + h * t.rpi;
-      float4 v[NS][H], q[H], q2[D2 ? H : 1];
+      float4 v[NS][H], q[H], q2[ADD2 ? H : 1];
       unsigned mb[H];
 #pragma unroll
       for (int u = 0; u < H; ++u) {
@@ -395,18 +471,20 @@
         if (rr < rows) {
 #pragma unroll
           for (int k = 0; k < NS; ++k) v[k][u] = ldg4(xp[k] + (size_t)rr * gm.C);
-          q[u] = ldg4(gd + (size_t)rr * gm.C);
+          if constexpr (POOL) q[u] = pooled_grad<D2>(dout, dout2, pl, gm, d, pp, t.q);
+          else q[u] = ldg4(gd + (size_t)rr * gm.C);
           if constexpr (MASK) mb[u] = __ldg(md + (size_t)rr * t.C4);
-          if constexpr (D2) q2[u] = ldg4(gd2 + (size_t)rr * gm.C);
+          if constexpr (ADD2) q2[u] = ldg4(gd2 + (size_t)rr * gm.C);
         } else {
 #pragma unroll
           for (int k = 0; k < NS; ++k) v[k][u] = make_float4(mu[k][0], mu[k][1], mu[k][2], mu[k][3]);
           q[u] = make_float4(0.f, 0.f, 0.f, 0.f);
           if constexpr (MASK) mb[u] = 0u;
-          if constexpr (D2) q2[u] = make_float4(0.f, 0.f, 0.f, 0.f);
-        }
-      }
-      if constexpr (D2) {
+          if constexpr (ADD2) q2[u] = make_float4(0.f, 0.f, 0.f, 0.f);
+        }
+        if constexpr (POOL) pp.advance(pl, t.rpi);
+      }
+      if constexpr (ADD2) {
 #pragma unroll
         for (int u = 0; u < H; ++u) { q[u].x += q2[u].x; q[u].y += q2[u].y; q[u].z += q2[u].z; q[u].w += q2[u].w; }
       }
@@ -611,6 +689,58 @@
   }
 }
 
+template <int GS, bool D2>
+__global__ void __launch_bounds__(256) cl_pool_bwd_apply_kernel(const float* __restrict__ x, const float* __restrict__ dp,
+                                                                const float* __restrict__ dp2, float* __restrict__ dx, const Geom gm,
+                                                                const ClPool pl, const float* __restrict__ coef,
+                                                                const float* __restrict__ save_mean, const float* __restrict__ save_w,
+                                                                const float* __restrict__ gamma, const float* __restrict__ beta) {
+  using S = ClShape<GS>;
+  constexpr int EPI = DWT_EPI_AFFINE | DWT_EPI_RELU;
+  const int C4 = gm.C >> 2, H2 = pl.H >> 1;
+  const int n = blockIdx.y / H2, k = blockIdx.y - n * H2, d = n / gm.N;
+  const int i = blockIdx.x * blockDim.x + threadIdx.x;
+  pdl_wait();
+  if (i >= (pl.W >> 1) * C4) return;
+  const int j = i >> pl.c4shift, q = i & (C4 - 1);
+  float4 g[2][2];
+  pool3s2_patch_grad<D2>(dp, dp2, pl.idx, (((size_t)n * pl.OH + k) * pl.OW + j) * C4 + q, k, j, pl.OH, pl.OW, C4, g);
+  const size_t p00 = (((size_t)n * pl.H + 2 * k) * pl.W + 2 * j) * gm.C + 4 * q;
+  float4 v[2][2];
+#pragma unroll
+  for (int a = 0; a < 2; ++a)
+#pragma unroll
+    for (int b = 0; b < 2; ++b) v[a][b] = ldg4(x + p00 + ((size_t)a * pl.W + b) * gm.C);
+  float Wp[S::NSUB][S::NM], bp[S::NSUB][GS];
+  BwdCoef<GS> cf[S::NSUB];
+#pragma unroll
+  for (int s = 0; s < S::NSUB; ++s) {
+    const int gi = q * S::NSUB + s;
+    load_forward_map<GS, EPI>(save_w + ((size_t)d * gm.G + gi) * GS * GS, save_mean + (size_t)d * gm.C + gi * GS,
+                              gamma + gi * GS, beta + gi * GS, Wp[s], bp[s]);
+    cf[s].load(coef + ((size_t)d * gm.G + gi) * coef_stride(GS));
+  }
+#pragma unroll
+  for (int a = 0; a < 2; ++a)
+#pragma unroll
+    for (int b = 0; b < 2; ++b) {
+      const float e[4] = {v[a][b].x, v[a][b].y, v[a][b].z, v[a][b].w};
+      const float ge[4] = {g[a][b].x, g[a][b].y, g[a][b].z, g[a][b].w};
+      float o[4];
+#pragma unroll
+      for (int s = 0; s < S::NSUB; ++s) {
+        float xi[GS], dz[GS], oi[GS];
+#pragma unroll
+        for (int c = 0; c < GS; ++c) { xi[c] = e[s * GS + c]; dz[c] = ge[s * GS + c]; }
+        apply_group<GS>(Wp[s], bp[s], xi, oi);
+#pragma unroll
+        for (int c = 0; c < GS; ++c) dz[c] = oi[c] > 0.f ? dz[c] : 0.f;
+        cf[s].apply(dz, xi, o + s * GS);
+      }
+      *reinterpret_cast<float4*>(dx + p00 + ((size_t)a * pl.W + b) * gm.C) = make_float4(o[0], o[1], o[2], o[3]);
+    }
+}
+
 #define CL_GS(GS_, ...)                                  \
   switch (GS_) {                                         \
     case 1: { constexpr int kGS = 1; __VA_ARGS__; break; } \
@@ -690,15 +820,15 @@
 void cl_bwd_reduce(const float* x, const float* dout, const float* dout2, const Geom& gm, int nctas, int gz, int epi, const float* mean, const float* w,
                    const float* gamma, const float* beta, const uint8_t* mask, float* dz, float* partial, cudaStream_t st) {
   const float* nul = nullptr;
-  CL_GS(gm.GS, CL_D2(dout2, CL_EPI_BWD(epi, (cl_bwd_reduce_kernel<kGS, kEPI, kD2, false><<<cl_grid(gm, nctas, gz), kT, 0, st>>>(
-                                                x, dout, dout2, gm, mean, w, gamma, beta, mask, dz, partial, nul, nul, 0)))));
+  CL_GS(gm.GS, CL_D2(dout2, CL_EPI_BWD(epi, (cl_bwd_reduce_kernel<kGS, kEPI, kD2, false, false><<<cl_grid(gm, nctas, gz), kT, 0, st>>>(
+                                                x, dout, dout2, gm, mean, w, gamma, beta, mask, dz, partial, nul, nul, 0, ClPool{})))));
 }
 void cl_tail2_bwd_reduce(const float* x, const float* xd, const float* dout, const float* dout2, const Geom& gm, int nctas, int gz,
                          const float* mean, const float* mean_d, const uint8_t* mask, float* dz, float* partial, size_t pstride,
                          cudaStream_t st) {
   const float* nul = nullptr;
-  CL_GS(gm.GS, CL_D2(dout2, (cl_bwd_reduce_kernel<kGS, 7, kD2, true><<<cl_grid(gm, nctas, gz), kT, 0, st>>>(
-                                x, dout, dout2, gm, mean, nul, nul, nul, mask, dz, partial, xd, mean_d, pstride))));
+  CL_GS(gm.GS, CL_D2(dout2, (cl_bwd_reduce_kernel<kGS, 7, kD2, true, false><<<cl_grid(gm, nctas, gz), kT, 0, st>>>(
+                                x, dout, dout2, gm, mean, nul, nul, nul, mask, dz, partial, xd, mean_d, pstride, ClPool{}))));
 }
 void cl_bwd_finalize(const float* partial, int nrows, const Geom& gm, const BwdFin& fin, cudaStream_t st, const BwdFin* fin2, size_t pstride) {
   const dim3 b = fin_block(gm), g((gm.C / 4) / b.y, fin2 ? 2 : 1);
@@ -717,4 +847,37 @@
                          nul, nul, nul, nul, xd, dxd, coef_d)));
 }
 
-}
+inline int patch_threads(int items) {
+  for (int t = 256; t >= 64; t -= 32)
+    if (items % t == 0) return t;
+  return items >= 256 ? 256 : ((items + 31) / 32) * 32;
+}
+inline ClPool stem_pool(const Geom& gm, const uint8_t* idx, int H, int W) {
+  int sh = 0;
+  while ((4 << sh) < gm.C) ++sh;
+  return ClPool{idx, H, W, H / 2, W / 2, sh};
+}
+void cl_apply_pool(const float* x, float* y, uint8_t* idx, const Geom& gm, int H, int W, const float* mean, const float* w,
+                   const float* gamma, const float* beta, cudaStream_t st) {
+  const ClPool pl = stem_pool(gm, nullptr, H, W);
+  const int items = (pl.OW / 2) * (gm.C / 4), threads = patch_threads(items);
+  const dim3 grid((items + threads - 1) / threads, gm.D * gm.N * (pl.OH / 2));
+  CL_GS(gm.GS, (launch_k(cl_apply_pool_kernel<kGS>, grid, dim3(threads), st, use_pdl(), x, y, idx, gm, pl, mean, w, gamma, beta)));
+}
+void cl_pool_bwd_reduce(const float* x, const float* dp, const float* dp2, const uint8_t* idx, const Geom& gm, int H, int W, int nctas,
+                        int gz, const float* mean, const float* w, const float* gamma, const float* beta, float* partial, cudaStream_t st) {
+  const float* nul = nullptr;
+  const ClPool pl = stem_pool(gm, idx, H, W);
+  CL_GS(gm.GS, CL_D2(dp2, (cl_bwd_reduce_kernel<kGS, 3, kD2, false, true><<<cl_grid(gm, nctas, gz), kT, 0, st>>>(
+                              x, dp, dp2, gm, mean, w, gamma, beta, (const uint8_t*)nullptr, (float*)nullptr, partial, nul, nul, 0, pl))));
+}
+void cl_pool_bwd_apply(const float* x, const float* dp, const float* dp2, const uint8_t* idx, float* dx, const Geom& gm, int H, int W,
+                       const float* coef, const float* mean, const float* w, const float* gamma, const float* beta, cudaStream_t st) {
+  const ClPool pl = stem_pool(gm, idx, H, W);
+  const int items = (W / 2) * (gm.C / 4), threads = patch_threads(items);
+  const dim3 grid((items + threads - 1) / threads, gm.D * gm.N * (H / 2));
+  CL_GS(gm.GS, CL_D2(dp2, (launch_k(cl_pool_bwd_apply_kernel<kGS, kD2>, grid, dim3(threads), st, use_pdl(), x, dp, dp2, dx, gm, pl, coef,
+                                    mean, w, gamma, beta))));
+}
+
+}
diff --git a/dwt-domain-adaptation_b200/dwt_b200/csrc/norm_launch.h b/dwt-domain-adaptation_b200/dwt_b200/csrc/norm_launch.h
--- a/dwt-domain-adaptation_b200/dwt_b200/csrc/norm_launch.h
+++ b/dwt-domain-adaptation_b200/dwt_b200/csrc/norm_launch.h
@@ -76,6 +76,12 @@
                          cudaStream_t st);
 void cl_tail2_bwd_apply(const float* x, const float* xd, const float* dz, float* dx, float* dxd, const Geom& gm, int nctas, int gz,
                         const float* coef, const float* coef_d, cudaStream_t st);
+void cl_apply_pool(const float* x, float* y, uint8_t* idx, const Geom& gm, int H, int W, const float* mean, const float* w,
+                   const float* gamma, const float* beta, cudaStream_t st);
+void cl_pool_bwd_reduce(const float* x, const float* dp, const float* dp2, const uint8_t* idx, const Geom& gm, int H, int W, int nctas,
+                        int gz, const float* mean, const float* w, const float* gamma, const float* beta, float* partial, cudaStream_t st);
+void cl_pool_bwd_apply(const float* x, const float* dp, const float* dp2, const uint8_t* idx, float* dx, const Geom& gm, int H, int W,
+                       const float* coef, const float* mean, const float* w, const float* gamma, const float* beta, cudaStream_t st);
 
 void maxpool_fwd_launch(const float* x, float* y, uint8_t* idx, int N, int H, int W, int C, int OH, int OW, int k, int s, int p,
                         cudaStream_t st);
diff --git a/dwt-domain-adaptation_b200/dwt_b200/csrc/pool.cu b/dwt-domain-adaptation_b200/dwt_b200/csrc/pool.cu
--- a/dwt-domain-adaptation_b200/dwt_b200/csrc/pool.cu
+++ b/dwt-domain-adaptation_b200/dwt_b200/csrc/pool.cu
@@ -1,5 +1,6 @@
 #include "dwt_common.cuh"
 #include "norm_launch.h"
+#include "pool_3s2.cuh"
 
 namespace dwt {
 namespace {
@@ -13,8 +14,6 @@
   if constexpr (K > 0) { g.k = K; g.s = S; g.p = P; }
   return g;
 }
-
-__device__ __forceinline__ bool takes(float v, float best) { return (v > best) || (v != v); }
 
 template <int K, int S, int P, bool POW2>
 __global__ void __launch_bounds__(256) maxpool_fwd_kernel(const float* __restrict__ x, float* __restrict__ y,
@@ -100,58 +99,8 @@
   const float4* xn = reinterpret_cast<const float4*>(x) + (size_t)n * g.H * g.W * g.C4 + c4;
   float best[2][2][4];
   unsigned bi[2][2][4];
-#pragma unroll
-  for (int oa = 0; oa < 2; ++oa)
-#pragma unroll
-    for (int ob = 0; ob < 2; ++ob)
-#pragma unroll
-      for (int c = 0; c < 4; ++c) { best[oa][ob][c] = -INFINITY; bi[oa][ob][c] = 0u; }
-  const int h0 = 4 * a - 1, w0 = 4 * b - 1;
-#pragma unroll
-  for (int r = 0; r < 5; ++r) {
-    const int h = h0 + r;
-    if (h < 0 || h >= g.H) continue;
-    float4 row[5];
-    bool in[5];
-#pragma unroll
-    for (int cc = 0; cc < 5; ++cc) {
-      const int w = w0 + cc;
-      in[cc] = w >= 0 && w < g.W;
-      row[cc] = in[cc] ? __ldg(xn + ((size_t)h * g.W + w) * g.C4) : make_float4(0.f, 0.f, 0.f, 0.f);
-    }
-#pragma unroll
-    for (int oa = 0; oa < 2; ++oa) {
-      const int kh = r - 2 * oa;
-      if (kh < 0 || kh > 2) continue;
-#pragma unroll
-      for (int ob = 0; ob < 2; ++ob)
-#pragma unroll
-        for (int kw = 0; kw < 3; ++kw) {
-          const int cc = 2 * ob + kw;
-          if (!in[cc]) continue;
-          const float e[4] = {row[cc].x, row[cc].y, row[cc].z, row[cc].w};
-          const unsigned code = (unsigned)(kh * 3 + kw);
-#pragma unroll
-          for (int c = 0; c < 4; ++c)
-            if (takes(e[c], best[oa][ob][c])) { best[oa][ob][c] = e[c]; bi[oa][ob][c] = code; }
-        }
-    }
-  }
-#pragma unroll
-  for (int oa = 0; oa < 2; ++oa)
-#pragma unroll
-    for (int ob = 0; ob < 2; ++ob) {
-      const size_t o = (((size_t)n * g.OH + 2 * a + oa) * g.OW + 2 * b + ob) * g.C4 + c4;
-      reinterpret_cast<float4*>(y)[o] = make_float4(best[oa][ob][0], best[oa][ob][1], best[oa][ob][2], best[oa][ob][3]);
-      reinterpret_cast<uint32_t*>(idx)[o] = bi[oa][ob][0] | (bi[oa][ob][1] << 8) | (bi[oa][ob][2] << 16) | (bi[oa][ob][3] << 24);
-    }
-}
-
-__device__ __forceinline__ void take(float4& acc, const float4& gq, uint32_t m, unsigned code) {
-  if ((m & 0xFFu) == code) acc.x += gq.x;
-  if (((m >> 8) & 0xFFu) == code) acc.y += gq.y;
-  if (((m >> 16) & 0xFFu) == code) acc.z += gq.z;
-  if ((m >> 24) == code) acc.w += gq.w;
+  pool3s2_patch(g.H, g.W, a, b, [&](int h, int w) { return __ldg(xn + ((size_t)h * g.W + w) * g.C4); }, best, bi);
+  pool3s2_store(y, idx, (((size_t)n * g.OH + 2 * a) * g.OW + 2 * b) * g.C4 + c4, g.OW, g.C4, best, bi);
 }
 
 __global__ void __launch_bounds__(256) maxpool_bwd_3s2_kernel(const float* __restrict__ dy, const uint8_t* __restrict__ idx,
@@ -161,28 +110,12 @@
   const int i = blockIdx.x * blockDim.x + threadIdx.x;
   if (i >= W2 * g.C4) return;
   const int j = i >> g.c4shift, c4 = i & (g.C4 - 1);
-  const float4* dyn = reinterpret_cast<const float4*>(dy) + (size_t)n * g.OH * g.OW * g.C4;
-  const uint32_t* ixn = reinterpret_cast<const uint32_t*>(idx) + (size_t)n * g.OH * g.OW * g.C4;
-  uint32_t m[2][2];
-  float4 gq[2][2];
-#pragma unroll
-  for (int a = 0; a < 2; ++a)
-#pragma unroll
-    for (int b = 0; b < 2; ++b) {
-      const bool ok = (k + a < g.OH) && (j + b < g.OW);
-      const size_t o = ((size_t)(k + a) * g.OW + (j + b)) * g.C4 + c4;
-      m[a][b] = ok ? __ldg(ixn + o) : 0xFFFFFFFFu;
-      gq[a][b] = ok ? __ldg(dyn + o) : make_float4(0.f, 0.f, 0.f, 0.f);
-    }
-  float4 o00 = make_float4(0.f, 0.f, 0.f, 0.f), o01 = o00, o10 = o00, o11 = o00;
-  take(o00, gq[0][0], m[0][0], 4u);
-  take(o01, gq[0][0], m[0][0], 5u); take(o01, gq[0][1], m[0][1], 3u);
-  take(o10, gq[0][0], m[0][0], 7u); take(o10, gq[1][0], m[1][0], 1u);
-  take(o11, gq[0][0], m[0][0], 8u); take(o11, gq[0][1], m[0][1], 6u); take(o11, gq[1][0], m[1][0], 2u); take(o11, gq[1][1], m[1][1], 0u);
+  float4 o[2][2];
+  pool3s2_patch_grad<false>(dy, nullptr, idx, (((size_t)n * g.OH + k) * g.OW + j) * g.C4 + c4, k, j, g.OH, g.OW, g.C4, o);
   float4* r0 = reinterpret_cast<float4*>(dx) + (((size_t)n * g.H + 2 * k) * g.W + 2 * j) * g.C4 + c4;
   float4* r1 = r0 + (size_t)g.W * g.C4;
-  r0[0] = o00; r0[g.C4] = o01;
-  r1[0] = o10; r1[g.C4] = o11;
+  r0[0] = o[0][0]; r0[g.C4] = o[0][1];
+  r1[0] = o[1][0]; r1[g.C4] = o[1][1];
 }
 
 }
diff --git a/dwt-domain-adaptation_b200/dwt_b200/csrc/pool_3s2.cuh b/dwt-domain-adaptation_b200/dwt_b200/csrc/pool_3s2.cuh
--- /dev/null
+++ b/dwt-domain-adaptation_b200/dwt_b200/csrc/pool_3s2.cuh
@@ -0,0 +1,135 @@
+#pragma once
+#include "dwt_common.cuh"
+
+namespace dwt {
+namespace {
+
+__device__ __forceinline__ bool takes(float v, float best) { return (v > best) || (v != v); }
+
+template <class Load>
+__device__ __forceinline__ void pool3s2_patch(int H, int W, int a, int b, Load&& load, float (&best)[2][2][4],
+                                              unsigned (&bi)[2][2][4]) {
+#pragma unroll
+  for (int oa = 0; oa < 2; ++oa)
+#pragma unroll
+    for (int ob = 0; ob < 2; ++ob)
+#pragma unroll
+      for (int c = 0; c < 4; ++c) { best[oa][ob][c] = -INFINITY; bi[oa][ob][c] = 0u; }
+  const int h0 = 4 * a - 1, w0 = 4 * b - 1;
+#pragma unroll
+  for (int r = 0; r < 5; ++r) {
+    const int h = h0 + r;
+    if (h < 0 || h >= H) continue;
+    float4 row[5];
+    bool in[5];
+#pragma unroll
+    for (int cc = 0; cc < 5; ++cc) {
+      const int w = w0 + cc;
+      in[cc] = w >= 0 && w < W;
+      row[cc] = in[cc] ? load(h, w) : make_float4(0.f, 0.f, 0.f, 0.f);
+    }
+#pragma unroll
+    for (int oa = 0; oa < 2; ++oa) {
+      const int kh = r - 2 * oa;
+      if (kh < 0 || kh > 2) continue;
+#pragma unroll
+      for (int ob = 0; ob < 2; ++ob)
+#pragma unroll
+        for (int kw = 0; kw < 3; ++kw) {
+          const int cc = 2 * ob + kw;
+          if (!in[cc]) continue;
+          const float e[4] = {row[cc].x, row[cc].y, row[cc].z, row[cc].w};
+          const unsigned code = (unsigned)(kh * 3 + kw);
+#pragma unroll
+          for (int c = 0; c < 4; ++c)
+            if (takes(e[c], best[oa][ob][c])) { best[oa][ob][c] = e[c]; bi[oa][ob][c] = code; }
+        }
+    }
+  }
+}
+
+__device__ __forceinline__ void pool3s2_store(float* __restrict__ y, uint8_t* __restrict__ idx, size_t o, int OW, int C4,
+                                              const float (&best)[2][2][4], const unsigned (&bi)[2][2][4]) {
+#pragma unroll
+  for (int oa = 0; oa < 2; ++oa)
+#pragma unroll
+    for (int ob = 0; ob < 2; ++ob) {
+      const size_t oo = o + ((size_t)oa * OW + ob) * C4;
+      reinterpret_cast<float4*>(y)[oo] = make_float4(best[oa][ob][0], best[oa][ob][1], best[oa][ob][2], best[oa][ob][3]);
+      reinterpret_cast<uint32_t*>(idx)[oo] = bi[oa][ob][0] | (bi[oa][ob][1] << 8) | (bi[oa][ob][2] << 16) | (bi[oa][ob][3] << 24);
+    }
+}
+
+__device__ __forceinline__ void take(float4& acc, const float4& gq, uint32_t m, unsigned code) {
+  if ((m & 0xFFu) == code) acc.x += gq.x;
+  if (((m >> 8) & 0xFFu) == code) acc.y += gq.y;
+  if (((m >> 16) & 0xFFu) == code) acc.z += gq.z;
+  if ((m >> 24) == code) acc.w += gq.w;
+}
+
+template <bool D2>
+__device__ __forceinline__ float4 pool3s2_pixel_grad(const float* __restrict__ dy, const float* __restrict__ dy2,
+                                                     const uint8_t* __restrict__ idx, unsigned o, int h, int w, int OH, int OW,
+                                                     int C4) {
+  const bool hodd = (h & 1) != 0, wodd = (w & 1) != 0;
+  const bool h1 = hodd && (h >> 1) + 1 < OH, w1 = wodd && (w >> 1) + 1 < OW;
+  const unsigned kh = hodd ? 2u : 1u, kw = wodd ? 2u : 1u;
+  uint32_t m[2][2];
+  float4 g[2][2];
+#pragma unroll
+  for (int a = 0; a < 2; ++a)
+#pragma unroll
+    for (int b = 0; b < 2; ++b) {
+      const bool ok = (a == 0 || h1) && (b == 0 || w1);
+      const unsigned oo = o + (unsigned)(a * OW + b) * C4;
+      m[a][b] = ok ? __ldg(reinterpret_cast<const uint32_t*>(idx) + oo) : 0xFFFFFFFFu;
+      g[a][b] = ok ? __ldg(reinterpret_cast<const float4*>(dy) + oo) : make_float4(0.f, 0.f, 0.f, 0.f);
+      if constexpr (D2) {
+        if (ok) {
+          const float4 g2 = __ldg(reinterpret_cast<const float4*>(dy2) + oo);
+          g[a][b].x += g2.x; g[a][b].y += g2.y; g[a][b].z += g2.z; g[a][b].w += g2.w;
+        }
+      }
+    }
+  float4 acc = make_float4(0.f, 0.f, 0.f, 0.f);
+  take(acc, g[0][0], m[0][0], kh * 3 + kw);
+  take(acc, g[0][1], m[0][1], kh * 3);
+  take(acc, g[1][0], m[1][0], kw);
+  take(acc, g[1][1], m[1][1], 0u);
+  return acc;
+}
+
+template <bool D2>
+__device__ __forceinline__ void pool3s2_patch_grad(const float* __restrict__ dy, const float* __restrict__ dy2,
+                                                   const uint8_t* __restrict__ idx, size_t o, int k, int j, int OH, int OW,
+                                                   int C4, float4 (&out)[2][2]) {
+  uint32_t m[2][2];
+  float4 gq[2][2];
+#pragma unroll
+  for (int a = 0; a < 2; ++a)
+#pragma unroll
+    for (int b = 0; b < 2; ++b) {
+      const bool ok = (k + a < OH) && (j + b < OW);
+      const size_t oo = o + ((size_t)a * OW + b) * C4;
+      m[a][b] = ok ? __ldg(reinterpret_cast<const uint32_t*>(idx) + oo) : 0xFFFFFFFFu;
+      gq[a][b] = ok ? __ldg(reinterpret_cast<const float4*>(dy) + oo) : make_float4(0.f, 0.f, 0.f, 0.f);
+      if constexpr (D2) {
+        if (ok) {
+          const float4 g2 = __ldg(reinterpret_cast<const float4*>(dy2) + oo);
+          gq[a][b].x += g2.x; gq[a][b].y += g2.y; gq[a][b].z += g2.z; gq[a][b].w += g2.w;
+        }
+      }
+    }
+  float4& o00 = out[0][0];
+  float4& o01 = out[0][1];
+  float4& o10 = out[1][0];
+  float4& o11 = out[1][1];
+  o00 = o01 = o10 = o11 = make_float4(0.f, 0.f, 0.f, 0.f);
+  take(o00, gq[0][0], m[0][0], 4u);
+  take(o01, gq[0][0], m[0][0], 5u); take(o01, gq[0][1], m[0][1], 3u);
+  take(o10, gq[0][0], m[0][0], 7u); take(o10, gq[1][0], m[1][0], 1u);
+  take(o11, gq[0][0], m[0][0], 8u); take(o11, gq[0][1], m[0][1], 6u); take(o11, gq[1][0], m[1][0], 2u); take(o11, gq[1][1], m[1][1], 0u);
+}
+
+}
+}
diff --git a/dwt-domain-adaptation_b200/dwt_b200/functional.py b/dwt-domain-adaptation_b200/dwt_b200/functional.py
--- a/dwt-domain-adaptation_b200/dwt_b200/functional.py
+++ b/dwt-domain-adaptation_b200/dwt_b200/functional.py
@@ -1,4 +1,6 @@
 from __future__ import annotations
+
+import ctypes
 
 import torch
 
@@ -227,6 +229,84 @@
                                    [(r, float(e), float(m), bool(u)) for r, e, m, u in sites])
 
 
+class _SitePoolFunction(torch.autograd.Function):
+
+    @staticmethod
+    def forward(ctx, x, gamma, beta, kind, group_size, n_domains, site):
+        lib = nv.lib()
+        gs = group_size if kind == "whiten" else 1
+        if not (x.dim() == 4 and _dense(x, gs)[4] and x.shape[2] % 4 == 0 and x.shape[3] % 4 == 0):
+            raise ValueError("the fused site + max-pool takes a channels-last tensor with H and W multiples of 4 and a "
+                             "channels-last build")
+        if x.shape[0] % n_domains != 0:
+            raise ValueError(f"batch of {x.shape[0]} does not split into {n_domains} domains")
+        n_all, c, h, w = x.shape
+        n = n_all // n_domains
+        running, eps, momentum, update = site
+        dev = nv.require_cuda(x, gamma, beta, *[t for pair in running for t in pair])
+        for d, (rm_t, rv_t) in enumerate(running):
+            _check_param(f"running mean of domain {d}", rm_t, c)
+            _check_param(f"running second moment of domain {d}", rv_t, c * gs)
+        _check_param("gamma / weight", gamma, c)
+        _check_param("beta / bias", beta, c)
+        g_c, b_c = gamma.detach().reshape(-1).contiguous(), beta.detach().reshape(-1).contiguous()
+        save_mean = torch.empty(n_domains, c, dtype=torch.float32, device=dev)
+        save_w = torch.empty(n_domains, c // gs, gs, gs, dtype=torch.float32, device=dev)
+        rm = nv.ptr_array([pr[0] for pr in running]) if update else None
+        rv = nv.ptr_array([pr[1] for pr in running]) if update else None
+        c_site = nv.TailSite(x.data_ptr(), eps, momentum, int(update), rm, rv, g_c.data_ptr(), b_c.data_ptr(),
+                             save_mean.data_ptr(), save_w.data_ptr(), None, None, None)
+        y = torch.empty((n_all, c, h // 2, w // 2), dtype=torch.float32, device=dev, memory_format=torch.channels_last)
+        idx = torch.empty(y.numel(), dtype=torch.uint8, device=dev)
+        ws = nv.workspace(dev, n, c, h * w, gs, n_domains)
+        nv_kind = nv.KIND_WHITEN if kind == "whiten" else nv.KIND_BN
+        with torch.cuda.device(dev):
+            rc = lib.dwt_site_maxpool_fwd(nv_kind, ctypes.byref(c_site), nv.ptr(y), nv.ptr(idx), n, c, h, w, gs, n_domains,
+                                          3, 2, 1, nv.ptr(ws), ws.numel(), nv.stream_ptr(dev))
+        nv.check(rc)
+        nv.poll_status(dev)
+        if update:
+            seen = set()
+            for buf in (t for pair in running for t in pair):
+                if id(buf) not in seen:
+                    seen.add(id(buf))
+                    torch.autograd.graph.increment_version(buf)
+        ctx.save_for_backward(x, save_mean, save_w, g_c, b_c, idx)
+        ctx.cfg = (nv_kind, gs, n_domains, n, c, h, w, eps, gamma.shape, beta.shape)
+        return y
+
+    @staticmethod
+    def backward(ctx, dout):
+        lib = nv.lib()
+        x, save_mean, save_w, g_c, b_c, idx = ctx.saved_tensors
+        nv_kind, gs, n_domains, n, c, h, w, eps, gshape, bshape = ctx.cfg
+        dout2 = ctx.__dict__.pop("_dwt_extra_grad", None)
+        if dout2 is not None and not (dout2.shape == dout.shape and dout2.dtype == torch.float32
+                                      and dout2.is_contiguous(memory_format=torch.channels_last)):
+            dout, dout2 = dout + dout2, None
+        dout = dout.contiguous(memory_format=torch.channels_last)
+        dev = nv.require_cuda(dout)
+        dx = torch.empty_like(x)
+        grads = torch.empty(2, c, dtype=torch.float32, device=dev)
+        c_site = nv.TailSite(x.data_ptr(), eps, 0.0, 0, None, None, g_c.data_ptr(), b_c.data_ptr(), save_mean.data_ptr(),
+                             save_w.data_ptr(), dx.data_ptr(), grads[0].data_ptr(), grads[1].data_ptr())
+        ws = nv.workspace(dev, n, c, h * w, gs, n_domains)
+        with torch.cuda.device(dev):
+            rc = lib.dwt_site_maxpool_bwd(nv_kind, ctypes.byref(c_site), nv.ptr(dout), nv.ptr(dout2), nv.ptr(idx), n, c, h, w,
+                                          gs, n_domains, 3, 2, 1, nv.ptr(ws), ws.numel(), nv.stream_ptr(dev))
+        nv.check(rc)
+        return (dx, grads[0].view(gshape), grads[1].view(bshape)) + (None,) * 4
+
+
+def site_maxpool(x, gamma, beta, *, kind, group_size, n_domains, site):
+    running, eps, momentum, update = site
+    return _SitePoolFunction.apply(x, gamma, beta, kind, group_size, n_domains,
+                                   (running, float(eps), float(momentum), bool(update)))
+
+
+_FORK_PRODUCERS = (_NormFunction._backward_cls, _TailPairFunction._backward_cls, _SitePoolFunction._backward_cls)
+
+
 class _ForkForSum(torch.autograd.Function):
 
     @staticmethod
@@ -247,7 +327,7 @@
 
 def fork_for_sum(y):
     fn = getattr(y, "grad_fn", None)
-    if not torch.is_grad_enabled() or fn is None or not isinstance(fn, (_NormFunction._backward_cls, _TailPairFunction._backward_cls)):
+    if not torch.is_grad_enabled() or fn is None or not isinstance(fn, _FORK_PRODUCERS):
         return y, y
     return _ForkForSum.apply(y)
 
diff --git a/dwt-domain-adaptation_b200/dwt_b200/fused.py b/dwt-domain-adaptation_b200/dwt_b200/fused.py
--- a/dwt-domain-adaptation_b200/dwt_b200/fused.py
+++ b/dwt-domain-adaptation_b200/dwt_b200/fused.py
@@ -5,6 +5,7 @@
 
 from . import _native as nv
 from . import functional as F
+from . import pooling
 
 
 class DomainTripleNorm(nn.Module):
@@ -64,6 +65,19 @@
         return F.tail_pair(x, xd, gamma, beta, down_gamma, down_beta, kind=self.kind, group_size=self.group_size,
                            n_domains=self.n_domains, sites=(site_args, down_args))
 
+    def forward_with_maxpool(self, x, domain_modules, gamma, beta, pool, count_batches=True):
+        mods = list(domain_modules)
+        fuse = (self.kernel_epilogue and isinstance(pool, pooling.MaxPool2d)
+                and (pool.kernel_size, pool.stride, pool.padding) == (3, 2, 1)
+                and len(mods) == self.n_domains and x.dim() == 4 and x.shape[0] % self.n_domains == 0
+                and x.is_contiguous(memory_format=torch.channels_last) and not x.is_contiguous()
+                and x.shape[2] % 4 == 0 and x.shape[3] % 4 == 0 and x.shape[0] * (x.shape[2] // 2) <= 65535
+                and nv.channels_last_supported(x.shape[1], self.group_size))
+        if not fuse:
+            return pool(self(x, mods, gamma, beta, True, count_batches=count_batches))
+        return F.site_maxpool(x, gamma, beta, kind=self.kind, group_size=self.group_size, n_domains=self.n_domains,
+                              site=self._running_args(mods, count_batches))
+
     @staticmethod
     def _tensor_epilogue(y, gamma, beta, relu, residual):
         if residual is not None and not relu:
diff --git a/harness/resnet50_dwt.py b/harness/resnet50_dwt.py
--- a/harness/resnet50_dwt.py
+++ b/harness/resnet50_dwt.py
@@ -188,6 +188,15 @@
         c = self.conv1
         return torch.nn.functional.conv2d(xp, w, None, c.stride, c.padding, c.dilation, c.groups)
 
+    def _stem_site_pool(self, x):
+        fused = getattr(self, "_fused_1", None) if (self.training and not _REPLICATED[0]) else None
+        if fused is None:
+            return self.maxpool(self._site("1", x, relu=True))
+        names, gname, bname, whiten = self._sites["1"]
+        mods = [getattr(self, n).wh if whiten else getattr(self, n) for n in names]
+        return fused.forward_with_maxpool(x, mods, getattr(self, gname), getattr(self, bname), self.maxpool,
+                                          count_batches=not _BATCHED_COUNTERS[0])
+
     def _bump_counters(self):
         cs = getattr(self, "_bn_counters", None)
         if cs is None:
@@ -203,7 +212,7 @@
             self._bump_counters()
         _BATCHED_COUNTERS[0] = batched
         try:
-            x = self.maxpool(self._site("1", self._stem(x), relu=True))
+            x = self._stem_site_pool(self._stem(x))
             x = self.layer4(self.layer3(self.layer2(self.layer1(x))))
         finally:
             _BATCHED_COUNTERS[0] = False
diff --git a/include/dwt_b200.h b/include/dwt_b200.h
--- a/include/dwt_b200.h
+++ b/include/dwt_b200.h
@@ -8,7 +8,7 @@
 extern "C" {
 #endif
 
-#define DWT_B200_ABI_VERSION 6
+#define DWT_B200_ABI_VERSION 7
 #define DWT_MAX_DOMAINS 4
 #define DWT_MAX_GROUP_SIZE 64
 
@@ -88,6 +88,13 @@
                   const uint8_t *relu_mask, float *dz, int64_t N, int64_t C, int64_t HW, int group_size,
                   int n_domains, void *workspace, size_t workspace_bytes, dwt_stream_t stream);
 
+DWT_API int dwt_site_maxpool_fwd(int kind, const dwt_tail_site *site, float *y, uint8_t *argmax, int64_t N, int64_t C, int64_t H,
+                         int64_t W, int group_size, int n_domains, int kernel, int stride, int padding, void *workspace,
+                         size_t workspace_bytes, dwt_stream_t stream);
+DWT_API int dwt_site_maxpool_bwd(int kind, const dwt_tail_site *site, const float *dout, const float *dout2, const uint8_t *argmax,
+                         int64_t N, int64_t C, int64_t H, int64_t W, int group_size, int n_domains, int kernel, int stride,
+                         int padding, void *workspace, size_t workspace_bytes, dwt_stream_t stream);
+
 DWT_API int dwt_mec_fwd_bwd(const float *x, const float *y, int64_t N, int64_t K, float *loss, float *gx,
                     float *gy, dwt_stream_t stream);
 
```
